# alibaba-damo-academy/Inferix

Hardware: AMD Instinct MI355X
Metric: latent_frames_per_sec (higher is better)
Workload: dtype bf16; 1 GPU; Self-Forcing 480p bf16 (Wan2.1-T2V-1.3B causal DiT, 30 layers), block_size=3, 21 latent frames = 7 blocks x (4 denoise + 1 context) generator forwards, KV prefix 4680..32760 keys in the KV manager's cache (identity page map; page-table form: `streaming_steady`); `value` counts the generator calls (SURVEY 8d), the per-block VAE decode of config 2 is measured beside it under --full (`per_block_decod; batch=1, parallelism=single, layers=30, pair_forwards=True, pair_mode=streams

## Files before the change

### include/inferix_hip.h

```cpp
#ifndef INFERIX_HIP_H
#define INFERIX_HIP_H

#include <stdint.h>

#ifdef __cplusplus
extern "C" {
#endif

#define IFX_OK 0
#define IFX_EINVAL (-1)
#define IFX_ELAUNCH (-2)
#define IFX_EUNSUP (-3)

typedef uint16_t ifx_bf16;

#define IFX_ABI_MINOR 7
int ifx_version(void);
const char* ifx_last_error(void);
const char* ifx_arch(void);
int ifx_set_option(const char* key, int32_t value);
int ifx_get_option(const char* key, int32_t* value);
int32_t ifx_device_error(int32_t clear);

typedef struct {
  ifx_bf16* k;
  ifx_bf16* v;
  const int32_t* page_table;
  int32_t page_size;
  int32_t num_slots;
  int32_t kv_heads;
  int32_t head_dim;
  int32_t seg_split;
  int32_t seg_delta;
} ifx_kv_view;

int ifx_attn_fwd_paged(const ifx_bf16* q, ifx_bf16* out, float* lse, const ifx_kv_view* kv,
                       int32_t q_rows, int32_t heads, int32_t kv_start, int32_t kv_len, float scale,
                       void* stream);

int32_t ifx_attn_split_plan(int32_t q_rows, int32_t heads, int32_t kv_start, int32_t kv_len,
                            int64_t* workspace_bytes);
int ifx_attn_fwd_paged_split(const ifx_bf16* q, ifx_bf16* out, float* lse, const ifx_kv_view* kv,
                             int32_t q_rows, int32_t heads, int32_t kv_start, int32_t kv_len, float scale,
                             int32_t num_splits, void* workspace, int64_t workspace_bytes, void* stream);

int ifx_attn_fwd_paged_ld(const ifx_bf16* q, int32_t ldq, ifx_bf16* out, int32_t ldo, float* lse, const ifx_kv_view* kv,
                          int32_t q_rows, int32_t heads, int32_t kv_start, int32_t kv_len, float scale, int32_t num_splits,
                          void* workspace, int64_t workspace_bytes, void* stream);

int ifx_attn_fwd_dedup(const ifx_bf16* q, ifx_bf16* out, const ifx_kv_view* kv, int32_t q_rows, int32_t heads, int32_t kv_len,
                       int32_t last_key_multiplicity, float scale, void* stream);

int ifx_attn_fwd_ranges(const ifx_bf16* q, int32_t ldq, ifx_bf16* out, int32_t ldo, const ifx_kv_view* kv, int32_t q_rows,
                        int32_t heads, int32_t n_ranges, const int32_t* q_ranges, const int32_t* k_ranges, float scale,
                        void* stream);

int ifx_attn_fwd_partial(const ifx_bf16* q, const ifx_kv_view* kv, int32_t q_rows, int32_t heads, int32_t kv_start,
                         int32_t kv_len, float scale, int32_t num_splits, void* workspace, int64_t workspace_bytes,
                         int32_t slot_base, int32_t slot_cap, int32_t* slots_used, void* stream);
int ifx_attn_merge_partials(const void* workspace, int32_t slot_cap, int32_t slots_used, ifx_bf16* out, float* lse,
                            int32_t q_rows, int32_t heads, void* stream);

int ifx_lse_merge(ifx_bf16* out_a, float* lse_a, const ifx_bf16* out_b, const float* lse_b,
                  int32_t rows, int32_t heads, void* stream);

typedef struct {
  const double* freqs;
  int32_t max_pos;
  int32_t start_frame;
  int32_t height, width;
  int32_t hw_offset;
  int32_t hw_local;
  float q_scale;
  int32_t flags;
} ifx_rope_grid;

int ifx_rmsnorm_rope_kv_append(const ifx_bf16* qkv, int32_t qkv_row_stride, ifx_bf16* q_out,
                               const ifx_bf16* wq, const ifx_bf16* wk, const ifx_rope_grid* rope,
                               const ifx_kv_view* kv, int32_t local_start, int32_t rows,
                               int32_t dim, float eps, void* stream);

int ifx_rmsnorm(const ifx_bf16* x, int32_t x_row_stride, ifx_bf16* y, int32_t y_row_stride,
                const ifx_bf16* w, int32_t rows, int32_t dim, float eps, void* stream);

enum { IFX_LN_PLAIN = 0, IFX_LN_AFFINE = 1, IFX_LN_MODULATE = 2 };
int ifx_layernorm(const ifx_bf16* x, ifx_bf16* y, int32_t rows, int32_t dim, float eps, int32_t mode,
                  const ifx_bf16* gamma, const ifx_bf16* beta, const ifx_bf16* mod,
                  int32_t mod_slots, int32_t shift_slot, int32_t scale_slot, int32_t rows_per_group,
                  void* stream);

enum { IFX_EPI_BIAS = 0, IFX_EPI_GELU_TANH = 1, IFX_EPI_RESIDUAL = 2, IFX_EPI_GATE_RES = 3, IFX_EPI_GELU_ERF = 4 };
typedef struct {
  int32_t epilogue;
  const ifx_bf16* residual;
  int32_t ld_res;
  const ifx_bf16* mod;
  int32_t mod_slots;
  int32_t gate_slot;
  int32_t rows_per_group;
  ifx_bf16* y2;
  int32_t ldy2;
  int32_t split_col;
} ifx_epilogue;
int ifx_gemm_bf16(const ifx_bf16* x, int32_t ldx, const ifx_bf16* w, const ifx_bf16* bias,
                  ifx_bf16* y, int32_t ldy, int32_t M, int32_t N, int32_t K,
                  const ifx_epilogue* epi, void* stream);

int64_t ifx_gemm_workspace_bytes(int32_t M, int32_t N, int32_t K);
int ifx_gemm_bf16_ws(const ifx_bf16* x, int32_t ldx, const ifx_bf16* w, const ifx_bf16* bias, ifx_bf16* y, int32_t ldy,
                     int32_t M, int32_t N, int32_t K, const ifx_epilogue* epi, void* workspace, int64_t workspace_bytes,
                     void* stream);

enum { IFX_Q_FP8_E4M3 = 0, IFX_Q_INT8 = 1 };
int ifx_quant_per_token(const ifx_bf16* x, int32_t ldx, void* q, int32_t ldq, float* scale, int32_t rows,
                        int32_t K, int32_t format, void* stream);
int ifx_gemm_q8(const void* xq, int32_t ldx, const float* x_scale, const void* wq, const float* w_scale,
                const ifx_bf16* bias, ifx_bf16* y, int32_t ldy, int32_t M, int32_t N, int32_t K, int32_t format,
                const ifx_epilogue* epi, void* stream);
int64_t ifx_gemm_q8_workspace_bytes(int32_t M, int32_t N, int32_t K);
int ifx_gemm_q8_ws(const void* xq, int32_t ldx, const float* x_scale, const void* wq, const float* w_scale, const ifx_bf16* bias,
                   ifx_bf16* y, int32_t ldy, int32_t M, int32_t N, int32_t K, int32_t format, const ifx_epilogue* epi,
                   void* workspace, int64_t workspace_bytes, void* stream);
int ifx_layernorm_quant(const ifx_bf16* x, void* q, int32_t ldq, float* scale, int32_t rows, int32_t dim, float eps,
                        int32_t mode, const ifx_bf16* gamma, const ifx_bf16* beta, const ifx_bf16* mod, int32_t mod_slots,
                        int32_t shift_slot, int32_t scale_slot, int32_t rows_per_group, int32_t format, void* stream);

int ifx_gemm_q8_quant_out(const void* xq, int32_t ldx, const float* x_scale, const void* wq, const float* w_scale,
                          const ifx_bf16* bias, void* yq, int32_t ldyq, int32_t M, int32_t N, int32_t K, int32_t format,
                          const ifx_epilogue* epi, const float* out_divisor, int32_t via_bf16, void* stream);
int ifx_layernorm_quant_static(const ifx_bf16* x, void* q, int32_t ldq, const float* divisors, int32_t n_out, int32_t rows,
                               int32_t dim, float eps, int32_t mode, const ifx_bf16* gamma, const ifx_bf16* beta,
                               int32_t via_bf16, void* stream);

int ifx_quant_static(const ifx_bf16* x, int32_t ldx, void* q, int32_t ldq, const float* divisor, int32_t divisor_len,
                     float* row_scale, int32_t rows, int32_t K, int32_t format, int32_t via_bf16, void* stream);
int ifx_quant_per_tensor(const ifx_bf16* x, int32_t ldx, void* q, int32_t ldq, float* row_scale, void* amax_workspace,
                         int32_t rows, int32_t K, int32_t format, void* stream);

int ifx_kv_roll(const ifx_kv_view* kv, int32_t sink_tokens, int32_t evicted, int32_t rolled,
                ifx_bf16* scratch, void* stream);

int ifx_kv_scatter_shards(const ifx_bf16* gathered, int32_t world, int32_t frames, int32_t hw_local,
                          int32_t frame_tokens, int32_t local_start, const ifx_kv_view* kv, void* stream);

#define IFX_MAX_PEERS 8
#define IFX_PEER_HANDLE_BYTES 64
typedef struct {
  int32_t count;
  ifx_bf16* k[IFX_MAX_PEERS];
  ifx_bf16* v[IFX_MAX_PEERS];
} ifx_peer_caches;
typedef struct {
  int32_t count;
  int32_t* flags[IFX_MAX_PEERS];
} ifx_peer_flags;
int ifx_peer_alloc(int64_t bytes, int32_t fine_grained, void** ptr);
int ifx_peer_free(void* ptr);
int ifx_peer_export(const void* ptr, uint8_t* handle, int64_t* offset);
int ifx_peer_open(const uint8_t* handle, void** ptr);
int ifx_peer_close(void* ptr);
int ifx_rmsnorm_rope_kv_push(const ifx_bf16* kv_rows, int32_t kv_row_stride, const ifx_bf16* wk, const ifx_rope_grid* rope,
                             const ifx_peer_caches* peers, const ifx_kv_view* geometry, int32_t local_start, int32_t frame_tokens,
                             int32_t slot_hw_local, int32_t slot_hw_offset, int32_t rows, int32_t dim, float eps, void* stream);
int ifx_peer_signal(const ifx_peer_flags* peers, int32_t index, int32_t value, void* stream);
int ifx_peer_wait(const int32_t* flags, int32_t count, int32_t value, int32_t timeout_ms, int32_t* status, void* stream);

typedef struct {
  const ifx_bf16* x;
  int64_t in_frame_stride;
  const int32_t* in_slots;
  int32_t hs, ws, cin, upsample;
  const ifx_bf16* w;
  const ifx_bf16* bias;
  int32_t kt, ks;
  ifx_bf16* y;
  int64_t out_frame_stride;
  const int32_t* out_slots;
  int32_t cout, t_out;
  const ifx_bf16* residual;
  const void* zero_page;
  int32_t in_planar;
} ifx_conv3d_desc;
int ifx_conv3d_cl(const ifx_conv3d_desc* desc, void* stream);

#define IFX_NORM_SILU 1
#define IFX_NORM_OUT_PLANAR 2
int ifx_rmsnorm_cl(const ifx_bf16* x, const ifx_bf16* gamma, ifx_bf16* y, int64_t out_frame_stride,
                   const int32_t* out_slots, int32_t frames, int32_t frame_pixels, int32_t channels,
                   int32_t flags, void* stream);

int ifx_softmax_rows(const ifx_bf16* scores, ifx_bf16* probs, int32_t rows, int32_t cols, int32_t ld, float scale,
                     void* stream);

int ifx_t5_attention(const ifx_bf16* q, int32_t ldq, const ifx_bf16* k, int32_t ldk, const ifx_bf16* v, int32_t ldv,
                     ifx_bf16* out, int32_t ldo, const ifx_bf16* rel_bias, const int32_t* seq_lens, int32_t batch,
                     int32_t seq_len_padded, int32_t heads, void* stream);

int ifx_t5_gated_gelu(const ifx_bf16* gate_fc1, ifx_bf16* h, int32_t rows, int32_t ffn, void* stream);

typedef struct {
  const ifx_bf16* in;
  int32_t ld_in, rows, layout, q_heads, kv_heads, head_dim;
  const float* rope;
  const float *qn_w, *qn_b, *kn_w, *kn_b;
  const ifx_bf16 *xn_w, *xn_b;
  float eps;
  int32_t layernorm_1p;
  ifx_bf16* q_out;
  int32_t ld_q;
  ifx_bf16* qx_out;
  int32_t ld_qx;
  ifx_bf16* k_out;
  ifx_bf16* v_out;
  int32_t ld_kv, kv_head_stride;
  int32_t row0, split, row1;
  float q_scale;
  int32_t rope_half;
  int32_t q_group;
  int64_t q_group_stride;
} ifx_magi_head_prep_desc;
int ifx_magi_head_prep(const ifx_magi_head_prep_desc* desc, void* stream);

int ifx_magi_gate_norm_residual(const ifx_bf16* x, int32_t ldx, const ifx_bf16* residual, int32_t ld_res,
                                const int32_t* condition_map, const ifx_bf16* gate, int32_t ld_gate, const float* norm_w,
                                const float* norm_b, int32_t layernorm_1p, ifx_bf16* y, int32_t ldy, int32_t rows, int32_t dim,
                                float eps, void* stream);

enum { IFX_ACT_SILU = 0, IFX_ACT_TANH = 1 };
int ifx_act_rows(const ifx_bf16* x, ifx_bf16* y, int64_t n, int32_t mode, void* stream);
int ifx_kv_split_rows(const ifx_bf16* kv, ifx_bf16* k_cache, ifx_bf16* v_cache, int32_t rows, int32_t heads, int32_t row0,
                      int32_t split, int32_t row1, void* stream);

#ifdef __cplusplus
}
#endif
#endif
```

### inferix_amd/_hip.py

```python
from __future__ import annotations

import ctypes as C
import os
from typing import Optional

import torch

_HERE = os.path.dirname(os.path.abspath(__file__))
LIB_PATH = os.environ.get("IFX_HIP_LIB", os.path.join(_HERE, "libinferix_hip.so"))

IFX_LN_PLAIN, IFX_LN_AFFINE, IFX_LN_MODULATE = 0, 1, 2
IFX_EPI_BIAS, IFX_EPI_GELU_TANH, IFX_EPI_RESIDUAL, IFX_EPI_GATE_RES, IFX_EPI_GELU_ERF = 0, 1, 2, 3, 4
IFX_ACT_SILU, IFX_ACT_TANH = 0, 1
IFX_Q_FP8_E4M3, IFX_Q_INT8 = 0, 1


class HipLibraryMissing(RuntimeError):
    pass


class HipKernelError(RuntimeError):
    pass


class KvView(C.Structure):
    _fields_ = [("k", C.c_void_p), ("v", C.c_void_p), ("page_table", C.c_void_p),
                ("page_size", C.c_int32), ("num_slots", C.c_int32), ("kv_heads", C.c_int32),
                ("head_dim", C.c_int32), ("seg_split", C.c_int32), ("seg_delta", C.c_int32)]


class RopeGrid(C.Structure):
    _fields_ = [("freqs", C.c_void_p), ("max_pos", C.c_int32), ("start_frame", C.c_int32),
                ("height", C.c_int32), ("width", C.c_int32), ("hw_offset", C.c_int32),
                ("hw_local", C.c_int32), ("q_scale", C.c_float), ("flags", C.c_int32)]


class Conv3dDesc(C.Structure):
    _fields_ = [("x", C.c_void_p), ("in_frame_stride", C.c_int64), ("in_slots", C.POINTER(C.c_int32)),
                ("hs", C.c_int32), ("ws", C.c_int32), ("cin", C.c_int32), ("upsample", C.c_int32),
                ("w", C.c_void_p), ("bias", C.c_void_p), ("kt", C.c_int32), ("ks", C.c_int32),
                ("y", C.c_void_p), ("out_frame_stride", C.c_int64), ("out_slots", C.POINTER(C.c_int32)),
                ("cout", C.c_int32), ("t_out", C.c_int32), ("residual", C.c_void_p), ("zero_page", C.c_void_p),
                ("in_planar", C.c_int32)]


class Epilogue(C.Structure):
    _fields_ = [("epilogue", C.c_int32), ("residual", C.c_void_p), ("ld_res", C.c_int32),
                ("mod", C.c_void_p), ("mod_slots", C.c_int32), ("gate_slot", C.c_int32),
                ("rows_per_group", C.c_int32), ("y2", C.c_void_p), ("ldy2", C.c_int32), ("split_col", C.c_int32)]


class MagiHeadPrepDesc(C.Structure):
    _fields_ = [("inp", C.c_void_p), ("ld_in", C.c_int32), ("rows", C.c_int32), ("layout", C.c_int32),
                ("q_heads", C.c_int32), ("kv_heads", C.c_int32), ("head_dim", C.c_int32), ("rope", C.c_void_p),
                ("qn_w", C.c_void_p), ("qn_b", C.c_void_p), ("kn_w", C.c_void_p), ("kn_b", C.c_void_p),
                ("xn_w", C.c_void_p), ("xn_b", C.c_void_p), ("eps", C.c_float), ("layernorm_1p", C.c_int32),
                ("q_out", C.c_void_p), ("ld_q", C.c_int32), ("qx_out", C.c_void_p), ("ld_qx", C.c_int32),
                ("k_out", C.c_void_p), ("v_out", C.c_void_p), ("ld_kv", C.c_int32), ("kv_head_stride", C.c_int32),
                ("row0", C.c_int32), ("split", C.c_int32), ("row1", C.c_int32), ("q_scale", C.c_float), ("rope_half", C.c_int32),
                ("q_group", C.c_int32), ("q_group_stride", C.c_int64)]


IFX_MAX_PEERS, IFX_PEER_HANDLE_BYTES = 8, 64


class PeerCaches(C.Structure):
    _fields_ = [("count", C.c_int32), ("k", C.c_void_p * IFX_MAX_PEERS), ("v", C.c_void_p * IFX_MAX_PEERS)]


class PeerFlags(C.Structure):
    _fields_ = [("count", C.c_int32), ("flags", C.c_void_p * IFX_MAX_PEERS)]


_vp, _i32, _f32 = C.c_void_p, C.c_int32, C.c_float
SIGNATURES = {
    "ifx_version": (C.c_int, []),
    "ifx_last_error": (C.c_char_p, []),
    "ifx_arch": (C.c_char_p, []),
    "ifx_set_option": (C.c_int, [C.c_char_p, _i32]),
    "ifx_get_option": (C.c_int, [C.c_char_p, C.POINTER(_i32)]),
    "ifx_device_error": (_i32, [_i32]),
    "ifx_attn_fwd_paged": (C.c_int, [_vp, _vp, _vp, C.POINTER(KvView), _i32, _i32, _i32, _i32, _f32, _vp]),
    "ifx_attn_split_plan": (_i32, [_i32, _i32, _i32, _i32, C.POINTER(C.c_int64)]),
    "ifx_attn_fwd_paged_split": (C.c_int, [_vp, _vp, _vp, C.POINTER(KvView), _i32, _i32, _i32, _i32, _f32, _i32, _vp,
                                           C.c_int64, _vp]),
    "ifx_conv3d_cl": (C.c_int, [C.POINTER(Conv3dDesc), _vp]),
    "ifx_rmsnorm_cl": (C.c_int, [_vp, _vp, _vp, C.c_int64, C.POINTER(_i32), _i32, _i32, _i32, _i32, _vp]),
    "ifx_softmax_rows": (C.c_int, [_vp, _vp, _i32, _i32, _i32, _f32, _vp]),
    "ifx_t5_attention": (C.c_int, [_vp, _i32, _vp, _i32, _vp, _i32, _vp, _i32, _vp, _vp, _i32, _i32, _i32, _vp]),
    "ifx_t5_gated_gelu": (C.c_int, [_vp, _vp, _i32, _i32, _vp]),
    "ifx_kv_scatter_shards": (C.c_int, [_vp, _i32, _i32, _i32, _i32, _i32, C.POINTER(KvView), _vp]),
    "ifx_peer_alloc": (C.c_int, [C.c_int64, _i32, C.POINTER(C.c_void_p)]),
    "ifx_peer_free": (C.c_int, [_vp]),
    "ifx_peer_export": (C.c_int, [_vp, C.c_char_p, C.POINTER(C.c_int64)]),
    "ifx_peer_open": (C.c_int, [C.c_char_p, C.POINTER(C.c_void_p)]),
    "ifx_peer_close": (C.c_int, [_vp]),
    "ifx_rmsnorm_rope_kv_push": (C.c_int, [_vp, _i32, _vp, C.POINTER(RopeGrid), C.POINTER(PeerCaches), C.POINTER(KvView), _i32, _i32,
                                           _i32, _i32, _i32, _i32, _f32, _vp]),
    "ifx_peer_signal": (C.c_int, [C.POINTER(PeerFlags), _i32, _i32, _vp]),
    "ifx_peer_wait": (C.c_int, [_vp, _i32, _i32, _i32, _vp, _vp]),
    "ifx_attn_fwd_partial": (C.c_int, [_vp, C.POINTER(KvView), _i32, _i32, _i32, _i32, _f32, _i32, _vp, C.c_int64, _i32,
                                       _i32, C.POINTER(_i32), _vp]),
    "ifx_attn_merge_partials": (C.c_int, [_vp, _i32, _i32, _vp, _vp, _i32, _i32, _vp]),
    "ifx_lse_merge": (C.c_int, [_vp, _vp, _vp, _vp, _i32, _i32, _vp]),
    "ifx_rmsnorm_rope_kv_append": (C.c_int, [_vp, _i32, _vp, _vp, _vp, C.POINTER(RopeGrid), C.POINTER(KvView),
                                             _i32, _i32, _i32, _f32, _vp]),
    "ifx_rmsnorm": (C.c_int, [_vp, _i32, _vp, _i32, _vp, _i32, _i32, _f32, _vp]),
    "ifx_layernorm": (C.c_int, [_vp, _vp, _i32, _i32, _f32, _i32, _vp, _vp, _vp, _i32, _i32, _i32, _i32, _vp]),
    "ifx_gemm_bf16": (C.c_int, [_vp, _i32, _vp, _vp, _vp, _i32, _i32, _i32, _i32, C.POINTER(Epilogue), _vp]),
    "ifx_kv_roll": (C.c_int, [C.POINTER(KvView), _i32, _i32, _i32, _vp, _vp]),
    "ifx_quant_per_token": (C.c_int, [_vp, _i32, _vp, _i32, _vp, _i32, _i32, _i32, _vp]),
    "ifx_layernorm_quant": (C.c_int, [_vp, _vp, _i32, _vp, _i32, _i32, _f32, _i32, _vp, _vp, _vp, _i32, _i32, _i32, _i32, _i32, _vp]),
    "ifx_gemm_q8": (C.c_int, [_vp, _i32, _vp, _vp, _vp, _vp, _vp, _i32, _i32, _i32, _i32, _i32, C.POINTER(Epilogue), _vp]),
    "ifx_gemm_q8_ws": (C.c_int, [_vp, _i32, _vp, _vp, _vp, _vp, _vp, _i32, _i32, _i32, _i32, _i32, C.POINTER(Epilogue), _vp, C.c_int64, _vp]),
    "ifx_gemm_q8_workspace_bytes": (C.c_int64, [_i32, _i32, _i32]),
    "ifx_attn_fwd_paged_ld": (C.c_int, [_vp, _i32, _vp, _i32, _vp, C.POINTER(KvView), _i32, _i32, _i32, _i32, _f32, _i32, _vp,
                                        C.c_int64, _vp]),
    "ifx_gemm_q8_quant_out": (C.c_int, [_vp, _i32, _vp, _vp, _vp, _vp, _vp, _i32, _i32, _i32, _i32, _i32, C.POINTER(Epilogue), _vp, _i32, _vp]),
    "ifx_layernorm_quant_static": (C.c_int, [_vp, _vp, _i32, _vp, _i32, _i32, _i32, _f32, _i32, _vp, _vp, _i32, _vp]),
    "ifx_quant_static": (C.c_int, [_vp, _i32, _vp, _i32, _vp, _i32, _vp, _i32, _i32, _i32, _i32, _vp]),
    "ifx_quant_per_tensor": (C.c_int, [_vp, _i32, _vp, _i32, _vp, _vp, _i32, _i32, _i32, _vp]),
    "ifx_magi_head_prep": (C.c_int, [C.POINTER(MagiHeadPrepDesc), _vp]),
    "ifx_magi_gate_norm_residual": (C.c_int, [_vp, _i32, _vp, _i32, _vp, _vp, _i32, _vp, _vp, _i32, _vp, _i32, _i32, _i32, _f32,
                                              _vp]),
    "ifx_act_rows": (C.c_int, [_vp, _vp, C.c_int64, _i32, _vp]),
    "ifx_kv_split_rows": (C.c_int, [_vp, _vp, _vp, _i32, _i32, _i32, _i32, _i32, _vp]),
    "ifx_attn_fwd_dedup": (C.c_int, [_vp, _vp, C.POINTER(KvView), _i32, _i32, _i32, _i32, _f32, _vp]),
    "ifx_attn_fwd_ranges": (C.c_int, [_vp, _i32, _vp, _i32, C.POINTER(KvView), _i32, _i32, _i32, C.POINTER(_i32), C.POINTER(_i32), _f32, _vp]),
    "ifx_gemm_workspace_bytes": (C.c_int64, [_i32, _i32, _i32]),
    "ifx_gemm_bf16_ws": (C.c_int, [_vp, _i32, _vp, _vp, _vp, _i32, _i32, _i32, _i32, C.POINTER(Epilogue), _vp, C.c_int64, _vp]),
}

_lib: Optional[C.CDLL] = None
ABI_MINOR = 7


def load() -> C.CDLL:
    global _lib
    if _lib is not None:
        return _lib
    if not os.path.exists(LIB_PATH):
        raise HipLibraryMissing(
            f"{LIB_PATH} not found: build it with `python -c 'import __graft_entry__ as g; g.build()'` "
            "(hipcc --offload-arch=gfx950).  inferix_amd has no CPU or eager fallback.")
    lib = C.CDLL(LIB_PATH)
    for name, (res, args) in SIGNATURES.items():
        fn = getattr(lib, name)
        fn.restype = res
        fn.argtypes = args
    got = (lib.ifx_version() >> 8) & 255
    if got != ABI_MINOR:
        raise HipLibraryMissing(f"{LIB_PATH} has ABI minor {got}, these bindings are for {ABI_MINOR} (include/inferix_hip.h "
                                "IFX_ABI_MINOR): rebuild with __graft_entry__.build()")
    _lib = lib
    return lib


def check(rc: int, what: str) -> None:
    if rc != 0:
        msg = load().ifx_last_error().decode("utf-8", "replace")
        raise HipKernelError(f"{what} failed (code {rc}): {msg}")


def version() -> str:
    v = load().ifx_version()
    return f"{v >> 16}.{(v >> 8) & 255}.{v & 255}"
```

### inferix_amd/csrc/ifx_attn.hip

```cpp
#include <stdlib.h>
#include <type_traits>

#include "ifx_common.h"

namespace ifx {

constexpr int QT = 128;
constexpr int KT = 64;
constexpr int HD = 128;

struct AttnArgs {
  const unsigned short* q;
  unsigned short* out;
  float* lse;
  const unsigned short* k;
  const unsigned short* v;
  KvAddr ka;
  int q_rows, heads, kv_start, kv_len, q_tiles, per_xcd, total;
  int ldq, ldo;
  float last_key_bias;
  int kv_heads, q_per_kv;
  float scale, scale_log2;
};

typedef __attribute__((address_space(3))) void* attn_lds_ptr_t;
typedef const __attribute__((address_space(1))) void* attn_gbl_ptr_t;

__device__ __forceinline__ void attn_dma16(const unsigned short* src, unsigned lds) {
  asm volatile("s_mov_b32 m0, %0\n\ts_nop 0\n\tglobal_load_lds_dwordx4 %1, off" : : "s"(lds), "v"(src) : "memory");
}

__device__ __forceinline__ float max3f(float a, float b, float c) {
  float r;
  asm("v_max3_f32 %0, %1, %2, %3" : "=v"(r) : "v"(a), "v"(b), "v"(c));
  return r;
}
__device__ __forceinline__ float half_swap_max(float x) {
  float a = x, b = x, r;
  asm volatile("s_nop 1\n\tv_permlane32_swap_b32 %0, %1\n\ts_nop 1\n\tv_max_f32 %2, %0, %1"
               : "+v"(a), "+v"(b), "=v"(r));
  return r;
}

template <bool PAGED, bool SHORT>
__global__ __launch_bounds__(256, 2) void attn_fwd_kernel(AttnArgs A) {
  __shared__ __attribute__((aligned(16))) unsigned char smem[65536];
  const int tid = threadIdx.x, lane = tid & 63;
  const int wave = __builtin_amdgcn_readfirstlane(tid >> 6);
  const int hi = lane >> 5, l31 = lane & 31;

  const int xcd = blockIdx.x & 7, slot_i = blockIdx.x >> 3;
  const int wi = xcd * A.per_xcd + slot_i;
  if (slot_i >= A.per_xcd || wi >= A.total) return;
  const int head = wi / A.q_tiles, qt = wi - head * A.q_tiles;
  const int kv_stride = A.kv_heads * HD;
  const int kvh = head / A.q_per_kv;

  const int qrow = qt * QT + wave * 32 + l31;
  const int qrow_c = min(qrow, A.q_rows - 1);
  bf16x8 qf[8];
  {
    const unsigned short* qp = A.q + (size_t)qrow_c * A.ldq + head * HD + hi * 8;
#pragma unroll
    for (int ks = 0; ks < 8; ++ks) qf[ks] = *reinterpret_cast<const bf16x8*>(qp + ks * 16);
  }
  __builtin_amdgcn_s_waitcnt(0x0F70);

  const int d_row = lane >> 4, d_pc = lane & 15;
  int k_src_c[4], v_src_c[4], d_rowi[4];
#pragma unroll
  for (int r = 0; r < 4; ++r) {
    const int row = (r * 4 + wave) * 4 + d_row;
    d_rowi[r] = row;
    k_src_c[r] = (d_pc ^ (row & 15)) * 8;
    v_src_c[r] = ((((d_pc >> 2) ^ (row & 3)) << 2) | (d_pc & 3)) * 8;
  }
  const unsigned short* kbase = A.k + kvh * HD;
  const unsigned short* vbase = A.v + kvh * HD;
  const int last_key = A.kv_len - 1;
  const unsigned lds0 = (unsigned)(unsigned long long)(attn_lds_ptr_t)smem + wave * 1024;
  auto issue = [&](int t, int buf, auto clamp_tag) {
    constexpr bool CLAMP = decltype(clamp_tag)::value;
    const unsigned kb = lds0 + buf * 32768;
#pragma unroll
    for (int r = 0; r < 4; ++r) {
      int key = A.kv_start + t * KT + d_rowi[r];
      if (CLAMP) key = min(key, last_key);
      const size_t off = (size_t)(PAGED ? A.ka.slot(key) : key) * kv_stride;
      attn_dma16(kbase + off + k_src_c[r], kb + r * 4096);
      attn_dma16(vbase + off + v_src_c[r], kb + 16384 + r * 4096);
    }
  };

  f32x16 o[4];
#pragma unroll
  for (int d = 0; d < 4; ++d)
#pragma unroll
    for (int r = 0; r < 16; ++r) o[d][r] = 0.f;
  float m_run = -INFINITY, l_run = 0.f;
  const float c2 = A.scale_log2;

  const int kswz = l31 & 15;
  const int vi = lane & 15, vg1 = (lane >> 4) & 1;
  const int v_rowq = vi >> 2;
  const int v_in = (vg1 << 5) | ((vi & 3) << 3);

  const int nkeys = A.kv_len - A.kv_start;
  const int NT = (nkeys + KT - 1) / KT;

  auto tile = [&](int t, int buf, auto ragged_tag) {
    constexpr bool RAGGED = decltype(ragged_tag)::value;
    const unsigned char* kb = smem + buf * 32768;
    const unsigned char* vb = kb + 16384;
    bf16x8 kA[4], kB[4], vA[4], vB[4];
    auto ldK = [&](bf16x8(&f)[4], int b, int kh) {
      const unsigned char* krow = kb + (32 * b + l31) * 256;
#pragma unroll
      for (int k4 = 0; k4 < 4; ++k4)
        f[k4] = *reinterpret_cast<const bf16x8*>(krow + (((2 * (4 * kh + k4) + hi) ^ kswz) << 4));
    };
    auto mmaK = [&](f32x16& acc, bf16x8(&f)[4], int kh) {
#pragma unroll
      for (int k4 = 0; k4 < 4; ++k4) acc = __builtin_amdgcn_mfma_f32_32x32x16_bf16(f[k4], qf[4 * kh + k4], acc, 0, 0, 0);
    };
    auto ldV = [&](bf16x8(&f)[4], int b, int s2) {
      const unsigned char* vr0 = vb + (32 * b + 16 * s2 + 4 * hi + v_rowq) * 256 + v_in;
      const unsigned char* vr1 = vr0 + 8 * 256;
#pragma unroll
      for (int d = 0; d < 4; ++d) {
        const int ch = (d ^ v_rowq) << 6;
        const bf16x4 t0 = __builtin_amdgcn_ds_read_tr16_b64_v4bf16((bf16x4 __attribute__((address_space(3)))*)(vr0 + ch));
        const bf16x4 t1 = __builtin_amdgcn_ds_read_tr16_b64_v4bf16((bf16x4 __attribute__((address_space(3)))*)(vr1 + ch));
        f[d] = __builtin_shufflevector(t0, t1, 0, 1, 2, 3, 4, 5, 6, 7);
      }
    };
    auto mmaV = [&](bf16x8(&f)[4], const bf16x8& p) {
#pragma unroll
      for (int d = 0; d < 4; ++d) o[d] = __builtin_amdgcn_mfma_f32_32x32x16_bf16(f[d], p, o[d], 0, 0, 0);
    };
    auto block_max = [&](f32x16& sb) -> float {
      float mx = __builtin_fmaxf(sb[0], sb[1]);
      mx = max3f(mx, sb[2], m_run);
#pragma unroll
      for (int r = 3; r < 15; r += 2) mx = max3f(mx, sb[r], sb[r + 1]);
      mx = max3f(mx, sb[15], mx);
      return half_swap_max(mx);
    };
    auto exp_block = [&](f32x16& sb, bf16x8(&pb)[2]) -> float {
      typedef float f32x2 __attribute__((ext_vector_type(2)));
      const float mc = m_run * c2;
      const f32x2 c2v = {c2, c2}, mcv = {mc, mc};
      float a0 = 0.f, a1 = 0.f;
#pragma unroll
      for (int i = 0; i < 8; ++i) {
        const f32x2 sv = {sb[2 * i], sb[2 * i + 1]};
        const f32x2 e = sv * c2v - mcv;
        const float p0 = __builtin_amdgcn_exp2f(e[0]), p1 = __builtin_amdgcn_exp2f(e[1]);
        a0 += p0;
        a1 += p1;
        pb[i >> 2][(2 * i) & 7] = static_cast<__bf16>(p0);
        pb[i >> 2][(2 * i + 1) & 7] = static_cast<__bf16>(p1);
      }
      return a0 + a1;
    };
    auto softmax_block = [&](f32x16& sb, int b, bf16x8(&pb)[2]) -> float {
      if (RAGGED) {
        const int kidx = t * KT + 32 * b + 4 * hi;
#pragma unroll
        for (int r = 0; r < 16; ++r) {
          const int kk = kidx + (r & 3) + 8 * (r >> 2);
          if (kk >= nkeys) sb[r] = -INFINITY;
          else if (kk == nkeys - 1) sb[r] += A.last_key_bias;
        }
      }
      if (t == 0 && b == 0) m_run = block_max(sb);
      float ps = exp_block(sb, pb);
      float alpha = 1.0f;
      if (__any(!(ps < 1048576.f))) {
        const float m_new = block_max(sb);
        alpha = __builtin_amdgcn_exp2f((m_run - m_new) * c2);
        m_run = m_new;
        ps = exp_block(sb, pb);
        l_run *= alpha;
      }
      l_run += ps;
      return alpha;
    };
    auto rescale_o = [&](float alpha) {
      asm volatile("" : "+v"(alpha));
      if (__any(alpha != 1.0f)) {
        asm volatile("s_nop 15\n\ts_nop 7" ::: "memory");
#pragma unroll
        for (int d = 0; d < 4; ++d)
#pragma unroll
          for (int r = 0; r < 16; ++r) asm volatile("v_mul_f32 %0, %0, %1" : "+v"(o[d][r]) : "v"(alpha));
        asm volatile("s_nop 3" ::: "memory");
      }
    };

    f32x16 s0, s1;
    bf16x8 p0[2], p1[2];
    ldK(kA, 0, 0);
    ldK(kB, 0, 1);
    __builtin_amdgcn_sched_barrier(0);
#pragma unroll
    for (int r = 0; r < 16; ++r) s0[r] = 0.f;
    __builtin_amdgcn_s_setprio(1);
    mmaK(s0, kA, 0);
    ldK(kA, 1, 0);
    __builtin_amdgcn_sched_barrier(0);
    mmaK(s0, kB, 1);
    ldK(kB, 1, 1);
    __builtin_amdgcn_sched_barrier(0);
#pragma unroll
    for (int r = 0; r < 16; ++r) s1[r] = 0.f;
    mmaK(s1, kA, 0);
    ldV(vA, 0, 0);
    mmaK(s1, kB, 1);
    ldV(vB, 0, 1);
    const float a0 = softmax_block(s0, 0, p0);
#pragma unroll
    for (int i = 0; i < 8; ++i) {
      __builtin_amdgcn_sched_group_barrier(0x008, 1, 0);
      __builtin_amdgcn_sched_group_barrier(0x100, 2, 0);
      __builtin_amdgcn_sched_group_barrier(0x002, 10, 0);
    }
    __builtin_amdgcn_sched_barrier(0);
    rescale_o(a0);
    mmaV(vA, p0[0]);
    ldV(vA, 1, 0);
    mmaV(vB, p0[1]);
    ldV(vB, 1, 1);
    const float a1 = softmax_block(s1, 1, p1);
#pragma unroll
    for (int i = 0; i < 8; ++i) {
      __builtin_amdgcn_sched_group_barrier(0x008, 1, 1);
      __builtin_amdgcn_sched_group_barrier(0x100, 2, 1);
      __builtin_amdgcn_sched_group_barrier(0x002, 10, 1);
    }
    __builtin_amdgcn_sched_barrier(0);
    rescale_o(a1);
    mmaV(vA, p1[0]);
    mmaV(vB, p1[1]);
    __builtin_amdgcn_s_setprio(0);
  };

  issue(0, 0, std::true_type{});
  asm volatile("s_waitcnt vmcnt(0)" ::: "memory");
  __builtin_amdgcn_s_barrier();
  for (int t = 0; t < NT - 1; ++t) {
    const int buf = t & 1;
    if (t + 2 < NT) issue(t + 1, buf ^ 1, std::false_type{});
    else issue(t + 1, buf ^ 1, std::true_type{});
    tile(t, buf, std::false_type{});
    asm volatile("s_waitcnt vmcnt(0) lgkmcnt(0)" ::: "memory");
    __builtin_amdgcn_s_barrier();
  }
  if ((nkeys & (KT - 1)) || A.last_key_bias != 0.f) tile(NT - 1, (NT - 1) & 1, std::true_type{});
  else tile(NT - 1, (NT - 1) & 1, std::false_type{});

  const float l_tot = l_run + __shfl_xor(l_run, 32, 64);
  const float inv = 1.0f / l_tot;
  if (qrow < A.q_rows) {
    unsigned short* op = A.out + (size_t)qrow * A.ldo + head * HD + 4 * hi;
#pragma unroll
    for (int d = 0; d < 4; ++d)
#pragma unroll
      for (int g = 0; g < 4; ++g) {
        u16x4 w;
#pragma unroll
        for (int e = 0; e < 4; ++e) w[e] = f2bf(o[d][4 * g + e] * inv);
        *reinterpret_cast<u16x4*>(op + 32 * d + 8 * g) = w;
      }
    if (A.lse != nullptr && hi == 0) A.lse[(size_t)head * A.q_rows + qrow] = m_run * A.scale + __logf(l_tot);
  }
}

__global__ __launch_bounds__(256) void lse_merge_kernel(unsigned short* __restrict__ oa, float* __restrict__ la,
                                                        const unsigned short* __restrict__ ob,
                                                        const float* __restrict__ lb, int rows, int heads) {
  const size_t total = (size_t)rows * heads * 16;
  for (size_t i = (size_t)blockIdx.x * blockDim.x + threadIdx.x; i < total; i += (size_t)gridDim.x * blockDim.x) {
    const int c = (int)(i & 15);
    const size_t rh = i >> 4;
    const int h = (int)(rh % heads);
    const size_t r = rh / heads;
    const float a = la[(size_t)h * rows + r], b = lb[(size_t)h * rows + r];
    const float sg = 1.0f / (1.0f + __expf(a - b));
    u16x8 ua = *reinterpret_cast<const u16x8*>(oa + rh * HD + c * 8);
    const u16x8 ub = *reinterpret_cast<const u16x8*>(ob + rh * HD + c * 8);
#pragma unroll
    for (int e = 0; e < 8; ++e) {
      const float x = bf2f(ua[e]), y = bf2f(ub[e]);
      ua[e] = f2bf(x - sg * (x - y));
    }
    *reinterpret_cast<u16x8*>(oa + rh * HD + c * 8) = ua;
    if (c == 0) {
      const float mxv = fmaxf(a, b);
      la[(size_t)h * rows + r] = mxv + __logf(__expf(a - mxv) + __expf(b - mxv));
    }
  }
}

int launch_attn_pp(const unsigned short* q, unsigned short* out, float* lse, const ifx_kv_view* kv, int q_rows,
                   int heads, int kv_start, int kv_len, float scale, int splits, void* workspace, int groups,
                   hipStream_t stream, int slot_base = 0, int slot_cap = 0, int* slots_used = nullptr, int ldq = 0, int ldo = 0,
                   int n_ranges = 0, const int* q_ranges = nullptr, const int* k_ranges = nullptr);
int launch_attn_merge(const float* workspace, int slot_cap, int slots_used, unsigned short* out, float* lse, int q_rows,
                      int heads, hipStream_t stream, int ldo = 0);
size_t attn_pp_workspace_bytes(int q_rows, int heads, int splits);
int attn_pp_split_heuristic(int q_rows, int heads, int nkeys, int qt, int slots);
static int attn_groups(int variant, int q_rows, int heads = 0) {
  if (variant == 3 || variant == 4 || variant == 2 || variant == 5 || variant == 6 || variant == 7) return variant;
  if (variant == 0 && q_rows > 0) {
    const int t256 = (q_rows + 255) / 256, t128 = (q_rows + 127) / 128;
    const float u256 = (float)q_rows / (256.f * t256), u128 = (float)q_rows / (128.f * t128);
    if (u128 > 1.1f * u256) return 6;
    if (heads > 0 && t256 * heads > 256) {
      const float c5 = (float)((t256 * heads + 255) / 256);
      const float c6 = (float)((t128 * heads + 511) / 512) / 0.953f;
      if (c6 < 0.95f * c5) return 6;
    }
  }
  return 7;
}
static int attn_qt(int groups) { return groups == 3 ? 384 : (groups == 6 ? 128 : 256); }
static int attn_slots(int groups) { return groups == 6 ? 512 : 256; }

}

using namespace ifx;

static int attn_dispatch(const ifx_bf16* q, ifx_bf16* out, float* lse, const ifx_kv_view* kv, int32_t q_rows,
                         int32_t heads, int32_t kv_start, int32_t kv_len, float scale, int32_t splits, void* workspace,
                         int64_t workspace_bytes, void* stream, int32_t ldq = 0, int32_t ldo = 0, int32_t last_key_multiplicity = 1) {
  IFX_REQUIRE(q && out && kv && kv->k && kv->v, "ifx_attn_fwd_paged: null argument");
  if (ldq <= 0) ldq = heads * HD;
  if (ldo <= 0) ldo = heads * HD;
  IFX_REQUIRE(ldq >= heads * HD && ldo >= heads * HD && ldq % 8 == 0 && ldo % 8 == 0,
              "ifx_attn_fwd_paged: row strides (%d, %d) must be >= heads * 128 and multiples of 8", ldq, ldo);
  IFX_REQUIRE(kv->head_dim == HD, "ifx_attn_fwd_paged: head_dim %d not built (128 only)", kv->head_dim);
  IFX_REQUIRE(heads > 0 && kv->kv_heads > 0 && heads % kv->kv_heads == 0,
              "ifx_attn_fwd_paged: heads %d is not a multiple of kv_heads %d", heads, kv->kv_heads);
  IFX_REQUIRE(q_rows >= 0 && kv_start >= 0 && kv_len > kv_start && kv_len <= kv->num_slots,
              "ifx_attn_fwd_paged: key range [%d, %d) out of range (capacity %d)", kv_start, kv_len, kv->num_slots);
  if (kv->page_table) IFX_REQUIRE(kv->page_size > 0, "ifx_attn_fwd_paged: page_size must be > 0");
  if (q_rows == 0) return IFX_OK;
  const int variant = attn_variant();
  if (last_key_multiplicity > 1) {
    IFX_REQUIRE(splits <= 1 && kv_len - kv_start <= 1024 && lse == nullptr,
                "ifx_attn_fwd_dedup: the multiplicity form is built for short key ranges (<= 1024 keys), unsplit, without LSE");
  }
  if (splits > 1) {
    IFX_REQUIRE(workspace && workspace_bytes >= (int64_t)attn_pp_workspace_bytes(q_rows, heads, splits),
                "ifx_attn_fwd_paged_split: workspace of %lld B too small for %d splits (need %lld B)",
                (long long)workspace_bytes, splits, (long long)attn_pp_workspace_bytes(q_rows, heads, splits));
    return launch_attn_pp(q, out, lse, kv, q_rows, heads, kv_start, kv_len, scale, splits, workspace, attn_groups(variant, q_rows, heads),
                          (hipStream_t)stream, 0, 0, nullptr, ldq, ldo);
  }
  if (last_key_multiplicity <= 1 && (variant >= 2 || (variant == 0 && q_rows >= 1024 && kv_len - kv_start > 1024)))
    return launch_attn_pp(q, out, lse, kv, q_rows, heads, kv_start, kv_len, scale, 1, nullptr, attn_groups(variant, q_rows, heads),
                          (hipStream_t)stream, 0, 0, nullptr, ldq, ldo);
  AttnArgs a;
  a.q = q;
  a.out = out;
  a.lse = lse;
  a.k = kv->k;
  a.v = kv->v;
  a.ka = KvAddr{kv->page_table, kv->page_size, kv->page_table ? 0 : kv->seg_split, kv->page_table ? 0 : kv->seg_delta};
  a.q_rows = q_rows;
  a.heads = heads;
  a.ldq = ldq;
  a.ldo = ldo;
  a.kv_start = kv_start;
  a.kv_len = kv_len;
  a.kv_heads = kv->kv_heads;
  a.q_per_kv = heads / kv->kv_heads;
  a.q_tiles = (q_rows + QT - 1) / QT;
  a.total = a.q_tiles * heads;
  a.per_xcd = (a.total + 7) / 8;
  a.scale = scale > 0.f ? scale : 0.08838834764831845f;
  a.scale_log2 = a.scale * 1.4426950408889634f;
  a.last_key_bias = last_key_multiplicity > 1 ? logf((float)last_key_multiplicity) / a.scale : 0.f;

  const dim3 grid(a.per_xcd * 8), block(256);
  const bool short_kv = kv_len - kv_start <= 1024;
  if (kv->page_table || kv->seg_split > 0) {
    if (short_kv) hipLaunchKernelGGL((attn_fwd_kernel<true, true>), grid, block, 0, (hipStream_t)stream, a);
    else hipLaunchKernelGGL((attn_fwd_kernel<true, false>), grid, block, 0, (hipStream_t)stream, a);
  } else {
    if (short_kv) hipLaunchKernelGGL((attn_fwd_kernel<false, true>), grid, block, 0, (hipStream_t)stream, a);
    else hipLaunchKernelGGL((attn_fwd_kernel<false, false>), grid, block, 0, (hipStream_t)stream, a);
  }
  return check_launch("ifx_attn_fwd_paged");
}

extern "C" int ifx_attn_fwd_paged(const ifx_bf16* q, ifx_bf16* out, float* lse, const ifx_kv_view* kv,
                                  int32_t q_rows, int32_t heads, int32_t kv_start, int32_t kv_len, float scale,
                                  void* stream) {
  return attn_dispatch(q, out, lse, kv, q_rows, heads, kv_start, kv_len, scale, 1, nullptr, 0, stream);
}

extern "C" int ifx_attn_fwd_paged_ld(const ifx_bf16* q, int32_t ldq, ifx_bf16* out, int32_t ldo, float* lse, const ifx_kv_view* kv,
                                     int32_t q_rows, int32_t heads, int32_t kv_start, int32_t kv_len, float scale,
                                     int32_t num_splits, void* workspace, int64_t workspace_bytes, void* stream) {
  IFX_REQUIRE(num_splits >= 1 && num_splits <= 64, "ifx_attn_fwd_paged_ld: num_splits %d outside [1, 64]", num_splits);
  IFX_REQUIRE(ldq > 0 && ldo > 0, "ifx_attn_fwd_paged_ld: row strides must be given");
  return attn_dispatch(q, out, lse, kv, q_rows, heads, kv_start, kv_len, scale, num_splits, workspace, workspace_bytes, stream,
                       ldq, ldo);
}

extern "C" int ifx_attn_fwd_dedup(const ifx_bf16* q, ifx_bf16* out, const ifx_kv_view* kv, int32_t q_rows, int32_t heads,
                                  int32_t kv_len, int32_t last_key_multiplicity, float scale, void* stream) {
  IFX_REQUIRE(last_key_multiplicity >= 1, "ifx_attn_fwd_dedup: multiplicity %d", last_key_multiplicity);
  return attn_dispatch(q, out, nullptr, kv, q_rows, heads, 0, kv_len, scale, 1, nullptr, 0, stream, 0, 0, last_key_multiplicity);
}

extern "C" int ifx_attn_fwd_ranges(const ifx_bf16* q, int32_t ldq, ifx_bf16* out, int32_t ldo, const ifx_kv_view* kv, int32_t q_rows,
                                   int32_t heads, int32_t n_ranges, const int32_t* q_ranges, const int32_t* k_ranges, float scale,
                                   void* stream) {
  IFX_REQUIRE(q && out && kv && kv->k && kv->v && q_ranges && k_ranges, "ifx_attn_fwd_ranges: null argument");
  IFX_REQUIRE(kv->head_dim == HD, "ifx_attn_fwd_ranges: head_dim %d not built (128 only)", kv->head_dim);
  IFX_REQUIRE(heads > 0 && kv->kv_heads > 0 && heads % kv->kv_heads == 0, "ifx_attn_fwd_ranges: heads %d / kv_heads %d", heads,
              kv->kv_heads);
  IFX_REQUIRE(n_ranges >= 1 && n_ranges <= 8, "ifx_attn_fwd_ranges: 1..8 ranges per launch (got %d)", n_ranges);
  if (ldq <= 0) ldq = heads * HD;
  if (ldo <= 0) ldo = heads * HD;
  IFX_REQUIRE(ldq >= heads * HD && ldo >= heads * HD && ldq % 8 == 0 && ldo % 8 == 0, "ifx_attn_fwd_ranges: row strides (%d, %d)", ldq, ldo);
  if (kv->page_table) IFX_REQUIRE(kv->page_size > 0, "ifx_attn_fwd_ranges: page_size must be > 0");
  int kmin = 0x7fffffff, kmax = 0, rows = 0;
  for (int i = 0; i < n_ranges; ++i) {
    const int q0 = q_ranges[2 * i], q1 = q_ranges[2 * i + 1], k0 = k_ranges[2 * i], k1 = k_ranges[2 * i + 1];
    IFX_REQUIRE(q0 >= 0 && q1 > q0 && q1 <= q_rows, "ifx_attn_fwd_ranges: query range %d = [%d, %d) outside [0, %d)", i, q0, q1, q_rows);
    IFX_REQUIRE(k0 >= 0 && k1 > k0 && k1 <= kv->num_slots, "ifx_attn_fwd_ranges: key range %d = [%d, %d) out of range (capacity %d)",
                i, k0, k1, kv->num_slots);
    kmin = k0 < kmin ? k0 : kmin;
    kmax = k1 > kmax ? k1 : kmax;
    rows += q1 - q0;
  }
  const int groups = attn_groups(attn_variant(), rows / n_ranges, heads * n_ranges);
  return launch_attn_pp(q, out, nullptr, kv, q_rows, heads, kmin, kmax, scale, 1, nullptr, groups == 5 || groups == 6 || groups == 7 ? groups : 7,
                        (hipStream_t)stream, 0, 0, nullptr, ldq, ldo, n_ranges, q_ranges, k_ranges);
}

extern "C" int32_t ifx_attn_split_plan(int32_t q_rows, int32_t heads, int32_t kv_start, int32_t kv_len,
                                       int64_t* workspace_bytes) {
  int splits = 1;
  if (q_rows > 0 && heads > 0 && kv_len > kv_start)
    splits = attn_pp_split_heuristic(q_rows, heads, kv_len - kv_start, attn_qt(attn_groups(attn_variant(), q_rows, heads)),
                                     attn_slots(attn_groups(attn_variant(), q_rows, heads)));
  if (workspace_bytes) *workspace_bytes = (int64_t)attn_pp_workspace_bytes(q_rows, heads, splits);
  return splits;
}

extern "C" int ifx_attn_fwd_paged_split(const ifx_bf16* q, ifx_bf16* out, float* lse, const ifx_kv_view* kv,
                                        int32_t q_rows, int32_t heads, int32_t kv_start, int32_t kv_len, float scale,
                                        int32_t num_splits, void* workspace, int64_t workspace_bytes, void* stream) {
  IFX_REQUIRE(num_splits >= 1 && num_splits <= 64, "ifx_attn_fwd_paged_split: num_splits %d outside [1, 64]", num_splits);
  return attn_dispatch(q, out, lse, kv, q_rows, heads, kv_start, kv_len, scale, num_splits, workspace, workspace_bytes,
                       stream);
}

extern "C" int ifx_attn_fwd_partial(const ifx_bf16* q, const ifx_kv_view* kv, int32_t q_rows, int32_t heads,
                                    int32_t kv_start, int32_t kv_len, float scale, int32_t num_splits, void* workspace,
                                    int64_t workspace_bytes, int32_t slot_base, int32_t slot_cap, int32_t* slots_used,
                                    void* stream) {
  IFX_REQUIRE(q && kv && kv->k && kv->v && workspace, "ifx_attn_fwd_partial: null argument");
  IFX_REQUIRE(kv->head_dim == HD, "ifx_attn_fwd_partial: head_dim %d not built (128 only)", kv->head_dim);
  IFX_REQUIRE(heads > 0 && kv->kv_heads > 0 && heads % kv->kv_heads == 0,
              "ifx_attn_fwd_partial: heads %d is not a multiple of kv_heads %d", heads, kv->kv_heads);
  IFX_REQUIRE(q_rows > 0 && kv_start >= 0 && kv_len > kv_start && kv_len <= kv->num_slots,
              "ifx_attn_fwd_partial: key range [%d, %d) out of range (capacity %d)", kv_start, kv_len, kv->num_slots);
  IFX_REQUIRE(num_splits >= 1 && slot_base >= 0 && slot_cap >= 1 && slot_cap <= 128,
              "ifx_attn_fwd_partial: bad split / slot arguments (%d splits, base %d, cap %d)", num_splits, slot_base, slot_cap);
  IFX_REQUIRE(workspace_bytes >= (int64_t)slot_cap * q_rows * heads * 129 * (int64_t)sizeof(float),
              "ifx_attn_fwd_partial: workspace of %lld B too small for %d slots", (long long)workspace_bytes, slot_cap);
  if (kv->page_table) IFX_REQUIRE(kv->page_size > 0, "ifx_attn_fwd_partial: page_size must be > 0");
  return launch_attn_pp(q, nullptr, nullptr, kv, q_rows, heads, kv_start, kv_len, scale, num_splits, workspace,
                        attn_groups(attn_variant(), q_rows, heads), (hipStream_t)stream, slot_base, slot_cap, slots_used);
}

extern "C" int ifx_attn_merge_partials(const void* workspace, int32_t slot_cap, int32_t slots_used, ifx_bf16* out,
                                       float* lse, int32_t q_rows, int32_t heads, void* stream) {
  IFX_REQUIRE(workspace && out && q_rows > 0 && heads > 0 && slots_used >= 1 && slots_used <= slot_cap,
              "ifx_attn_merge_partials: bad arguments (%d of %d slots)", slots_used, slot_cap);
  return launch_attn_merge((const float*)workspace, slot_cap, slots_used, out, lse, q_rows, heads, (hipStream_t)stream);
}

extern "C" int ifx_lse_merge(ifx_bf16* out_a, float* lse_a, const ifx_bf16* out_b, const float* lse_b,
                             int32_t rows, int32_t heads, void* stream) {
  IFX_REQUIRE(out_a && lse_a && out_b && lse_b && rows >= 0 && heads > 0, "ifx_lse_merge: bad arguments");
  if (rows == 0) return IFX_OK;
  const size_t total = (size_t)rows * heads * 16;
  const int blocks = (int)((total + 255) / 256 < 2048 ? (total + 255) / 256 : 2048);
  hipLaunchKernelGGL(lse_merge_kernel, dim3(blocks), dim3(256), 0, (hipStream_t)stream, out_a, lse_a, out_b,
                     lse_b, rows, heads);
  return check_launch("ifx_lse_merge");
}
```

### inferix_amd/csrc/ifx_core.hip

```cpp
#include <stdarg.h>
#include <stdlib.h>
#include <string.h>

#include "ifx_common.h"

namespace ifx {
static thread_local char g_err[512] = "";

void set_error(const char* fmt, ...) {
  va_list ap;
  va_start(ap, fmt);
  vsnprintf(g_err, sizeof(g_err), fmt, ap);
  va_end(ap);
}

static int g_gemm_variant = -1, g_gemm_pp_variant = -1, g_attn_variant = -1, g_conv_variant = -1, g_spin_timeout_ms = -1, g_spin_fault = 0;
static thread_local int g_gemm_small_split = -1;
static int opt_or_env(int& slot, const char* env, int dflt = 0) {
  if (slot < 0) {
    const char* e = getenv(env);
    slot = e ? atoi(e) : dflt;
  }
  return slot;
}
int gemm_variant() { return opt_or_env(g_gemm_variant, "IFX_GEMM_VARIANT"); }
int gemm_pp_variant() { return opt_or_env(g_gemm_pp_variant, "IFX_GEMM_PP_VARIANT"); }
int attn_variant() { return opt_or_env(g_attn_variant, "IFX_ATTN_VARIANT"); }
int conv_variant() { return opt_or_env(g_conv_variant, "IFX_CONV_VARIANT"); }
static unsigned* g_attn_dbg = nullptr;
static bool g_attn_dbg_on = false;
unsigned* attn_debug_counter() { return g_attn_dbg_on ? g_attn_dbg : nullptr; }
int gemm_small_split() { return opt_or_env(g_gemm_small_split, "IFX_GEMM_SMALL_SPLIT"); }

static unsigned* g_dev_err = nullptr;
unsigned* device_error_word() {
  if (g_dev_err == nullptr) {
    void* p = nullptr;
    if (hipHostMalloc(&p, 64, hipHostMallocMapped | hipHostMallocPortable) == hipSuccess && p != nullptr) {
      memset(p, 0, 64);
      g_dev_err = (unsigned*)p;
    }
  }
  return g_dev_err;
}
long long spin_timeout_ticks() { return (long long)max(1, opt_or_env(g_spin_timeout_ms, "IFX_SPIN_TIMEOUT_MS", 2000)) * 100000LL; }
int spin_fault() { return g_spin_fault; }
static thread_local char g_err_dev[640] = "";

int check_launch(const char* what) {
  hipError_t e = hipGetLastError();
  if (e != hipSuccess) {
    set_error("%s: launch failed: %s", what, hipGetErrorString(e));
    return IFX_ELAUNCH;
  }
  return IFX_OK;
}
}

extern "C" int ifx_version(void) { return (0 << 16) | (IFX_ABI_MINOR << 8) | 0; }
extern "C" int32_t ifx_device_error(int32_t clear) {
  unsigned* w = ifx::g_dev_err;
  if (w == nullptr) return 0;
  const unsigned v = __atomic_load_n(w, __ATOMIC_ACQUIRE);
  if (v != 0 && clear) __atomic_store_n(w, 0u, __ATOMIC_RELEASE);
  return (int32_t)v;
}
extern "C" const char* ifx_last_error(void) {
  const unsigned v = (unsigned)ifx_device_error(1);
  if (v == 0) return ifx::g_err;
  const unsigned kind = v >> 24, detail = v & 0xffffffu;
  snprintf(ifx::g_err_dev, sizeof(ifx::g_err_dev),
           "device: a kernel gave up a wait (%s, flag %u) after the spin budget — the producing workgroup was not resident or did not "
           "finish; the results of that launch are invalid%s%s",
           kind == 1 ? "split-K / stream-K consumer of ifx_gemm_bf16_ws / ifx_gemm_q8_ws" : "unknown waiter", detail,
           ifx::g_err[0] ? "; last host error: " : "", ifx::g_err);
  return ifx::g_err_dev;
}
extern "C" const char* ifx_arch(void) { return "gfx950"; }
extern "C" int ifx_set_option(const char* key, int32_t value) {
  if (key && !strcmp(key, "gemm_variant") && value >= 0 && value <= 29) { ifx::g_gemm_variant = value; return IFX_OK; }
  if (key && !strcmp(key, "gemm_small_split") && (value == 0 || value == 1)) { ifx::g_gemm_small_split = value; return IFX_OK; }
  if (key && !strcmp(key, "attn_variant") && value >= 0 && value <= 7) { ifx::g_attn_variant = value; return IFX_OK; }
  if (key && !strcmp(key, "conv_variant") && value >= 0 && value <= 1) { ifx::g_conv_variant = value; return IFX_OK; }
  if (key && !strcmp(key, "gemm_pp_variant") && value >= 0 && value <= 1) { ifx::g_gemm_pp_variant = value; return IFX_OK; }
  if (key && !strcmp(key, "attn_debug_counters") && (value == 0 || value == 1)) {
    if (value == 1) {
      if (ifx::g_attn_dbg == nullptr && hipMalloc((void**)&ifx::g_attn_dbg, 64) != hipSuccess) {
        ifx::g_attn_dbg = nullptr;
        ifx::set_error("ifx_set_option: attn_debug_counters: hipMalloc failed");
        return IFX_ELAUNCH;
      }
      (void)hipDeviceSynchronize();
      (void)hipMemset(ifx::g_attn_dbg, 0, 64);
    }
    ifx::g_attn_dbg_on = value == 1;
    return IFX_OK;
  }
  if (key && !strcmp(key, "spin_timeout_ms") && value >= 1 && value <= 600000) { ifx::g_spin_timeout_ms = value; return IFX_OK; }
  if (key && !strcmp(key, "spin_fault") && (value == 0 || value == 1)) { ifx::g_spin_fault = value; return IFX_OK; }
  ifx::set_error("ifx_set_option: unknown key or value out of range: %s = %d", key ? key : "(null)", (int)value);
  return IFX_EINVAL;
}
extern "C" int ifx_get_option(const char* key, int32_t* value) {
  if (key == nullptr || value == nullptr) { ifx::set_error("ifx_get_option: null argument"); return IFX_EINVAL; }
  if (!strcmp(key, "gemm_variant")) { *value = ifx::gemm_variant(); return IFX_OK; }
  if (!strcmp(key, "gemm_small_split")) { *value = ifx::gemm_small_split(); return IFX_OK; }
  if (!strcmp(key, "attn_variant")) { *value = ifx::attn_variant(); return IFX_OK; }
  if (!strcmp(key, "conv_variant")) { *value = ifx::conv_variant(); return IFX_OK; }
  if (!strcmp(key, "gemm_pp_variant")) { *value = ifx::gemm_pp_variant(); return IFX_OK; }
  if (!strcmp(key, "attn_debug_counters")) { *value = ifx::g_attn_dbg_on ? 1 : 0; return IFX_OK; }
  if (!strcmp(key, "attn_rescale_count")) {
    unsigned v = 0;
    if (ifx::g_attn_dbg != nullptr) {
      (void)hipDeviceSynchronize();
      (void)hipMemcpy(&v, ifx::g_attn_dbg, sizeof(v), hipMemcpyDeviceToHost);
    }
    *value = (int32_t)(v & 0x7fffffffu);
    return IFX_OK;
  }
  if (!strcmp(key, "spin_timeout_ms")) { *value = (int32_t)(ifx::spin_timeout_ticks() / 100000LL); return IFX_OK; }
  if (!strcmp(key, "spin_fault")) { *value = ifx::spin_fault(); return IFX_OK; }
  ifx::set_error("ifx_get_option: unknown key: %s", key);
  return IFX_EINVAL;
}
```

### inferix_amd/csrc/ifx_norm.hip

```cpp
#include "ifx_rows.h"

namespace ifx {

template <int NCH, int QUANT = 0>
__global__ __launch_bounds__(256) void layernorm_kernel(
    const unsigned short* __restrict__ x, unsigned short* __restrict__ y, int rows, int dim, float eps,
    int mode, const unsigned short* __restrict__ gamma, const unsigned short* __restrict__ beta,
    const unsigned short* __restrict__ mod, int mod_slots, int shift_slot, int scale_slot,
    int rows_per_group, unsigned char* __restrict__ q, int ldq, float* __restrict__ qscale, int n_out, int via_bf16) {
  const int lane = threadIdx.x & 63;
  const int r = blockIdx.x * 4 + (threadIdx.x >> 6);
  if (r >= rows) return;
  u16x8 xr[NCH], pa[NCH], pb[NCH];
  load_chunks<NCH>(xr, x + (size_t)r * dim, dim, lane);
  {
    const unsigned short* pa_p = nullptr;
    const unsigned short* pb_p = nullptr;
    if (mode == IFX_LN_MODULATE) {
      const size_t g0 = (size_t)(r / rows_per_group) * mod_slots;
      pa_p = mod + (g0 + scale_slot) * dim;
      pb_p = mod + (g0 + shift_slot) * dim;
    } else if (mode == IFX_LN_AFFINE) {
      pa_p = gamma;
      pb_p = beta;
    }
    if (pa_p != nullptr) {
      load_chunks<NCH>(pa, pa_p, dim, lane);
      load_chunks<NCH>(pb, pb_p, dim, lane);
    } else {
#pragma unroll
      for (int c = 0; c < NCH; ++c) {
        pa[c] = u16x8{0, 0, 0, 0, 0, 0, 0, 0};
        pb[c] = u16x8{0, 0, 0, 0, 0, 0, 0, 0};
      }
    }
  }
  Row<NCH> row;
  row.from(xr, dim, lane);
  float mean, rstd;
  ln_stats(row, dim, eps, lane, mean, rstd);

  u16x8 qrow[QUANT != 0 ? NCH : 1];
  if (QUANT != 0) {
#pragma unroll
    for (int c = 0; c < NCH; ++c) qrow[c] = u16x8{0, 0, 0, 0, 0, 0, 0, 0};
  }
#pragma unroll
  for (int c = 0; c < NCH; ++c) {
    const int col = c * 512 + lane * 8;
    if (col >= dim) continue;
    u16x8 o;
    if (mode == IFX_LN_MODULATE) {
      const u16x8 sc = pa[c], sh = pb[c];
#pragma unroll
      for (int i = 0; i < 8; ++i) {
        float t = rbf((row.v[c][i] - mean) * rstd);
        float s1 = rbf(1.0f + bf2f(sc[i]));
        t = rbf(t * s1);
        o[i] = f2bf(t + bf2f(sh[i]));
      }
    } else if (mode == IFX_LN_AFFINE) {
      const u16x8 g = pa[c], b = pb[c];
#pragma unroll
      for (int i = 0; i < 8; ++i)
        o[i] = f2bf((row.v[c][i] - mean) * rstd * bf2f(g[i]) + bf2f(b[i]));
    } else {
#pragma unroll
      for (int i = 0; i < 8; ++i) o[i] = f2bf((row.v[c][i] - mean) * rstd);
    }
    if (QUANT == 0) *reinterpret_cast<u16x8*>(y + (size_t)r * dim + col) = o;
    else qrow[c] = o;
  }
  if constexpr (QUANT == 3) {
    const float* divs = qscale;
    for (int j = 0; j < n_out; ++j) {
#pragma unroll
      for (int c = 0; c < NCH; ++c) {
        const int col = c * 512 + lane * 8;
        if (col >= dim) continue;
        const f32x4 d0 = *reinterpret_cast<const f32x4*>(divs + (size_t)j * dim + col);
        const f32x4 d1 = *reinterpret_cast<const f32x4*>(divs + (size_t)j * dim + col + 4);
        float v[8];
#pragma unroll
        for (int i = 0; i < 8; ++i) v[i] = bf2f(qrow[c][i]);
        *reinterpret_cast<u32x2*>(q + (size_t)r * ldq + (size_t)j * dim + col) = div_clamp8<true>(v, d0, d1, via_bf16);
      }
    }
  } else if constexpr (QUANT != 0) {
    quant_row_dynamic<QUANT == 1, NCH>(qrow, q + (size_t)r * ldq, qscale + r, dim, lane);
  }
}

template <int NCH>
__global__ __launch_bounds__(256) void rmsnorm_kernel(const unsigned short* __restrict__ x, int ldx,
                                                      unsigned short* __restrict__ y, int ldy,
                                                      const unsigned short* __restrict__ w, int rows,
                                                      int dim, float eps) {
  const int lane = threadIdx.x & 63;
  const int r = blockIdx.x * 4 + (threadIdx.x >> 6);
  if (r >= rows) return;
  u16x8 xr[NCH], wv[NCH];
  load_chunks<NCH>(xr, x + (size_t)r * ldx, dim, lane);
  load_chunks<NCH>(wv, w, dim, lane);
  Row<NCH> row;
  row.from(xr, dim, lane);
  const float rs = 1.0f / sqrtf(wave_sum(row.sumsq()) / (float)dim + eps);
#pragma unroll
  for (int c = 0; c < NCH; ++c) {
    const int col = c * 512 + lane * 8;
    u16x8 o;
#pragma unroll
    for (int i = 0; i < 8; ++i) o[i] = f2bf(rbf(row.v[c][i] * rs) * bf2f(wv[c][i]));
    if (col < dim) *reinterpret_cast<u16x8*>(y + (size_t)r * ldy + col) = o;
  }
}

template <int NCH>
__global__ __launch_bounds__(256) void rmsnorm_rope_append_kernel(
    const unsigned short* __restrict__ qkv, int ld, unsigned short* __restrict__ q_out,
    const unsigned short* __restrict__ wq, const unsigned short* __restrict__ wk, RopeArgs ra, int has_rope,
    unsigned short* __restrict__ kc, unsigned short* __restrict__ vc, KvAddr ka, int local_start, int rows,
    int dim, int head_dim, float eps) {
  const int lane = threadIdx.x & 63;
  const int r = blockIdx.x * 4 + (threadIdx.x >> 6);
  if (r >= rows) return;
  const unsigned short* base = qkv + (size_t)r * ld;

  size_t slot_off = 0;
  if (kc != nullptr) slot_off = (size_t)ka.slot(local_start + r) * dim;
  const RopeToken tk(ra, has_rope, r, head_dim, lane);

  const bool has_kv = kc != nullptr;
  const bool copy_v = vc != nullptr;
  u16x8 qraw[NCH], kraw[NCH], vraw[NCH], wqv[NCH], wkv[NCH];
  load_chunks<NCH>(qraw, base, dim, lane);
  load_chunks<NCH>(wqv, wq, dim, lane);
  if (has_kv) {
    load_chunks<NCH>(kraw, base + dim, dim, lane);
    if (copy_v) load_chunks<NCH>(vraw, base + 2 * dim, dim, lane);
    load_chunks<NCH>(wkv, wk, dim, lane);
  }
  if (has_kv && copy_v) {
#pragma unroll
    for (int c = 0; c < NCH; ++c) {
      const int col = c * 512 + lane * 8;
      if (col < dim) *reinterpret_cast<u16x8*>(vc + slot_off + col) = vraw[c];
    }
  }
  Row<NCH> row;
  rmsnorm_rope_row<NCH>(row, qraw, wqv, tk, ra, has_rope, ra.q_scale, dim, head_dim, eps, lane,
                        [&](int, int col, const u16x8& o) { *reinterpret_cast<u16x8*>(q_out + (size_t)r * dim + col) = o; });
  if (!has_kv) return;
  rmsnorm_rope_row<NCH>(row, kraw, wkv, tk, ra, has_rope, 1.0f, dim, head_dim, eps, lane,
                        [&](int, int col, const u16x8& o) { *reinterpret_cast<u16x8*>(kc + slot_off + col) = o; });
}

__global__ __launch_bounds__(256) void kv_copy_rows_kernel(const unsigned short* __restrict__ src,
                                                           unsigned short* __restrict__ dst, KvAddr ka,
                                                           int src_tok0, int dst_tok0, int ntok, int row_elems,
                                                           int src_is_paged, int dst_is_paged) {
  const int chunks = row_elems / 8;
  const size_t total = (size_t)ntok * chunks;
  for (size_t i = (size_t)blockIdx.x * blockDim.x + threadIdx.x; i < total; i += (size_t)gridDim.x * blockDim.x) {
    const int t = (int)(i / chunks), c = (int)(i - (size_t)t * chunks);
    const size_t s = (size_t)(src_is_paged ? ka.slot(src_tok0 + t) : (src_tok0 + t)) * row_elems + c * 8;
    const size_t d = (size_t)(dst_is_paged ? ka.slot(dst_tok0 + t) : (dst_tok0 + t)) * row_elems + c * 8;
    *reinterpret_cast<u16x8*>(dst + d) = *reinterpret_cast<const u16x8*>(src + s);
  }
}

__global__ __launch_bounds__(256) void kv_scatter_shards_kernel(const unsigned short* __restrict__ gathered,
                                                                unsigned short* __restrict__ kc,
                                                                unsigned short* __restrict__ vc, KvAddr ka, int world,
                                                                int frames, int hw_local, int frame_tokens,
                                                                int local_start, int row_elems) {
  const int n_local = frames * hw_local;
  const int chunks = row_elems / 8;
  const size_t total = (size_t)world * n_local * chunks;
  for (size_t i = (size_t)blockIdx.x * blockDim.x + threadIdx.x; i < total; i += (size_t)gridDim.x * blockDim.x) {
    const int row = (int)(i / chunks), c = (int)(i - (size_t)row * chunks);
    const int r = row / n_local, j = row - r * n_local;
    const int f = j / hw_local, w = j - f * hw_local;
    const int tok = local_start + f * frame_tokens + r * hw_local + w;
    const size_t d = (size_t)ka.slot(tok) * row_elems + c * 8;
    const unsigned short* ks = gathered + ((size_t)(2 * r) * n_local + j) * row_elems + c * 8;
    *reinterpret_cast<u16x8*>(kc + d) = *reinterpret_cast<const u16x8*>(ks);
    *reinterpret_cast<u16x8*>(vc + d) = *reinterpret_cast<const u16x8*>(ks + (size_t)n_local * row_elems);
  }
}

template <typename F>
static int dispatch_norm(int dim, F&& f) {
  return dispatch_nch<1, 2, 3, 4, 6, 8, 10>(dim, "row kernels support dim <= 5120 (got %d)", f);
}

}

using namespace ifx;

extern "C" int ifx_layernorm(const ifx_bf16* x, ifx_bf16* y, int32_t rows, int32_t dim, float eps, int32_t mode,
                             const ifx_bf16* gamma, const ifx_bf16* beta, const ifx_bf16* mod, int32_t mod_slots,
                             int32_t shift_slot, int32_t scale_slot, int32_t rows_per_group, void* stream) {
  IFX_REQUIRE(x && y && rows >= 0 && dim > 0 && dim % 8 == 0, "ifx_layernorm: bad x/y/rows/dim(%d)", dim);
  if (const int rc = check_ln_mode("ifx_layernorm", mode, gamma, beta, mod, mod_slots, shift_slot, scale_slot, rows_per_group))
    return rc;
  if (rows == 0) return IFX_OK;
  return dispatch_norm(dim, [&](auto nch) {
    return launch_rows("ifx_layernorm", layernorm_kernel<decltype(nch)::value, 0>, rows, stream, x, y, rows, dim, eps, mode, gamma, beta,
                       mod, mod_slots, shift_slot, scale_slot, rows_per_group > 0 ? rows_per_group : 1, (unsigned char*)nullptr, 0,
                       (float*)nullptr, 0, 0);
  });
}

extern "C" int ifx_layernorm_quant(const ifx_bf16* x, void* q, int32_t ldq, float* scale, int32_t rows, int32_t dim, float eps,
                                   int32_t mode, const ifx_bf16* gamma, const ifx_bf16* beta, const ifx_bf16* mod,
                                   int32_t mod_slots, int32_t shift_slot, int32_t scale_slot, int32_t rows_per_group,
                                   int32_t format, void* stream) {
  IFX_REQUIRE(x && q && scale && rows >= 0 && dim > 0 && dim % 8 == 0 && ldq >= dim && ldq % 8 == 0,
              "ifx_layernorm_quant: bad x/q/scale/rows/dim(%d)/ldq(%d)", dim, ldq);
  IFX_REQUIRE(format == IFX_Q_FP8_E4M3 || format == IFX_Q_INT8, "ifx_layernorm_quant: unknown format %d", format);
  if (const int rc = check_ln_mode("ifx_layernorm_quant", mode, gamma, beta, mod, mod_slots, shift_slot, scale_slot, rows_per_group))
    return rc;
  if (rows == 0) return IFX_OK;
  return dispatch_norm(dim, [&](auto nch) {
    return dispatch_q8_format(format, [&](auto fp8) {
      return launch_rows("ifx_layernorm_quant", layernorm_kernel<decltype(nch)::value, decltype(fp8)::value ? 1 : 2>, rows, stream, x,
                         (unsigned short*)nullptr, rows, dim, eps, mode, gamma, beta, mod, mod_slots, shift_slot, scale_slot,
                         rows_per_group > 0 ? rows_per_group : 1, (unsigned char*)q, ldq, scale, 0, 0);
    });
  });
}

extern "C" int ifx_layernorm_quant_static(const ifx_bf16* x, void* q, int32_t ldq, const float* divisors, int32_t n_out, int32_t rows,
                                          int32_t dim, float eps, int32_t mode, const ifx_bf16* gamma, const ifx_bf16* beta,
                                          int32_t via_bf16, void* stream) {
  IFX_REQUIRE(x && q && divisors && rows >= 0 && dim > 0 && dim % 8 == 0 && n_out >= 1 && n_out <= 8 && ldq >= n_out * dim && ldq % 8 == 0,
              "ifx_layernorm_quant_static: bad x/q/divisors/rows/dim(%d)/n_out(%d)/ldq(%d)", dim, n_out, ldq);
  IFX_REQUIRE(mode == IFX_LN_PLAIN || mode == IFX_LN_AFFINE, "ifx_layernorm_quant_static: mode %d (plain or affine)", mode);
  if (mode == IFX_LN_AFFINE) IFX_REQUIRE(gamma && beta, "ifx_layernorm_quant_static: affine mode needs gamma/beta");
  if (rows == 0) return IFX_OK;
  return dispatch_norm(dim, [&](auto nch) {
    return launch_rows("ifx_layernorm_quant_static", layernorm_kernel<decltype(nch)::value, 3>, rows, stream, x, (unsigned short*)nullptr,
                       rows, dim, eps, mode, gamma, beta, (const unsigned short*)nullptr, 0, 0, 0, 1, (unsigned char*)q, ldq,
                       const_cast<float*>(divisors), n_out, via_bf16);
  });
}

extern "C" int ifx_rmsnorm(const ifx_bf16* x, int32_t ldx, ifx_bf16* y, int32_t ldy, const ifx_bf16* w,
                           int32_t rows, int32_t dim, float eps, void* stream) {
  IFX_REQUIRE(x && y && w && rows >= 0 && dim > 0 && dim % 8 == 0 && ldx % 8 == 0 && ldy % 8 == 0,
              "ifx_rmsnorm: bad arguments (dim %d)", dim);
  IFX_REQUIRE(ldx >= dim && ldy >= dim, "ifx_rmsnorm: row strides ldx (%d) and ldy (%d) must be >= dim (%d)", ldx, ldy, dim);
  if (rows == 0) return IFX_OK;
  return dispatch_norm(dim, [&](auto nch) {
    return launch_rows("ifx_rmsnorm", rmsnorm_kernel<decltype(nch)::value>, rows, stream, x, ldx, y, ldy, w, rows, dim, eps);
  });
}

extern "C" int ifx_rmsnorm_rope_kv_append(const ifx_bf16* qkv, int32_t ld, ifx_bf16* q_out, const ifx_bf16* wq,
                                          const ifx_bf16* wk, const ifx_rope_grid* rope, const ifx_kv_view* kv,
                                          int32_t local_start, int32_t rows, int32_t dim, float eps,
                                          void* stream) {
  IFX_REQUIRE(qkv && q_out && wq && rows >= 0 && dim > 0 && dim % 8 == 0 && ld % 8 == 0,
              "ifx_rmsnorm_rope_kv_append: bad arguments");
  int head_dim = 128;
  KvAddr ka{nullptr, 1};
  unsigned short *kc = nullptr, *vc = nullptr;
  if (kv) {
    IFX_REQUIRE(wk && kv->k && kv->v && kv->kv_heads * kv->head_dim == dim,
                "ifx_rmsnorm_rope_kv_append: kv view (heads %d x head_dim %d) does not match dim %d",
                kv->kv_heads, kv->head_dim, dim);
    IFX_REQUIRE(local_start >= 0 && local_start + rows <= kv->num_slots,
                "ifx_rmsnorm_rope_kv_append: append [%d, %d) exceeds cache capacity %d", local_start,
                local_start + rows, kv->num_slots);
    if (const int rc = check_writer_view("ifx_rmsnorm_rope_kv_append", kv)) return rc;
    head_dim = kv->head_dim;
    kc = kv->k;
    vc = kv->v;
    ka = KvAddr{kv->page_table, kv->page_size};
  }
  RopeArgs ra{};
  if (const int rc = resolve_rope("ifx_rmsnorm_rope_kv_append", rope, head_dim, dim, rows, &ra)) return rc;
  if (rope) {
    IFX_REQUIRE(rope->q_scale >= 0.f && rope->q_scale == rope->q_scale, "ifx_rmsnorm_rope_kv_append: q_scale must be >= 0 (0 = 1)");
    ra.q_scale = rope->q_scale > 0.f ? rope->q_scale : 1.0f;
    if (rope->flags & 1) {
      IFX_REQUIRE(kv != nullptr, "ifx_rmsnorm_rope_kv_append: flags bit 0 (V in place) needs a cache view");
      vc = nullptr;
    }
  }
  {
    const int cols = kc == nullptr ? 1 : (vc == nullptr ? 2 : 3);
    IFX_REQUIRE(ld >= cols * dim, "ifx_rmsnorm_rope_kv_append: qkv_row_stride (ld %d) must cover the %d x dim (%d) columns read", ld, cols,
                dim);
  }
  if (rows == 0) return IFX_OK;
  return dispatch_norm(dim, [&](auto nch) {
    return launch_rows("ifx_rmsnorm_rope_kv_append", rmsnorm_rope_append_kernel<decltype(nch)::value>, rows, stream, qkv, ld, q_out, wq,
                       wk, ra, rope ? 1 : 0, kc, vc, ka, local_start, rows, dim, head_dim, eps);
  });
}

struct PeerDest {
  unsigned short* k[IFX_MAX_PEERS];
  unsigned short* v[IFX_MAX_PEERS];
  int n;
};

template <int NCH>
__global__ __launch_bounds__(256) void rmsnorm_rope_kv_push_kernel(
    const unsigned short* __restrict__ kv, int ld, const unsigned short* __restrict__ wk, RopeArgs ra, int has_rope, PeerDest pd,
    KvAddr ka, int local_start, int frame_tokens, int slot_hw_local, int slot_hw_offset, int rows, int dim, int head_dim, float eps) {
  const int lane = threadIdx.x & 63;
  const int r = blockIdx.x * 4 + (threadIdx.x >> 6);
  if (r >= rows) return;
  const unsigned short* base = kv + (size_t)r * ld;
  const int sf = r / slot_hw_local;
  const size_t slot_off = (size_t)ka.slot(local_start + sf * frame_tokens + slot_hw_offset + (r - sf * slot_hw_local)) * dim;
  const RopeToken tk(ra, has_rope, r, head_dim, lane);
  u16x8 kraw[NCH], vraw[NCH], wkv[NCH];
  load_chunks<NCH>(kraw, base, dim, lane);
  load_chunks<NCH>(vraw, base + dim, dim, lane);
  load_chunks<NCH>(wkv, wk, dim, lane);
  Row<NCH> row;
  rmsnorm_rope_row<NCH>(row, kraw, wkv, tk, ra, has_rope, 1.0f, dim, head_dim, eps, lane, [&](int c, int col, const u16x8& o) {
    for (int p = 0; p < pd.n; ++p) {
      *reinterpret_cast<u16x8*>(pd.k[p] + slot_off + col) = o;
      *reinterpret_cast<u16x8*>(pd.v[p] + slot_off + col) = vraw[c];
    }
  });
}

extern "C" int ifx_rmsnorm_rope_kv_push(const ifx_bf16* kv_rows, int32_t ld, const ifx_bf16* wk, const ifx_rope_grid* rope,
                                        const ifx_peer_caches* peers, const ifx_kv_view* geometry, int32_t local_start,
                                        int32_t frame_tokens, int32_t slot_hw_local, int32_t slot_hw_offset, int32_t rows, int32_t dim,
                                        float eps, void* stream) {
  IFX_REQUIRE(kv_rows && wk && peers && geometry && rows >= 0 && dim > 0 && dim % 8 == 0 && ld % 8 == 0 && ld >= 2 * dim,
              "ifx_rmsnorm_rope_kv_push: bad arguments");
  IFX_REQUIRE(peers->count >= 1 && peers->count <= IFX_MAX_PEERS, "ifx_rmsnorm_rope_kv_push: %d destinations (1..%d)", peers->count,
              IFX_MAX_PEERS);
  IFX_REQUIRE(geometry->kv_heads * geometry->head_dim == dim, "ifx_rmsnorm_rope_kv_push: cache rows (heads %d x head_dim %d) != dim %d",
              geometry->kv_heads, geometry->head_dim, dim);
  IFX_REQUIRE(slot_hw_local > 0 && frame_tokens >= slot_hw_local && slot_hw_offset >= 0 && slot_hw_offset + slot_hw_local <= frame_tokens,
              "ifx_rmsnorm_rope_kv_push: bad shard geometry (frame %d tokens, shard [%d, %d))", frame_tokens, slot_hw_offset,
              slot_hw_offset + slot_hw_local);
  if (rows == 0) return IFX_OK;
  const int last_f = (rows - 1) / slot_hw_local;
  const int last_token = local_start + last_f * frame_tokens + slot_hw_offset + (rows - 1 - last_f * slot_hw_local);
  IFX_REQUIRE(local_start >= 0 && last_token < geometry->num_slots, "ifx_rmsnorm_rope_kv_push: token %d exceeds the cache capacity %d",
              last_token, geometry->num_slots);
  if (geometry->page_table) IFX_REQUIRE(geometry->page_size > 0, "ifx_rmsnorm_rope_kv_push: page_size must be > 0");
  PeerDest pd{};
  pd.n = peers->count;
  for (int p = 0; p < pd.n; ++p) {
    IFX_REQUIRE(peers->k[p] && peers->v[p], "ifx_rmsnorm_rope_kv_push: destination %d is null", p);
    pd.k[p] = peers->k[p];
    pd.v[p] = peers->v[p];
  }
  const int head_dim = geometry->head_dim;
  RopeArgs ra{};
  if (const int rc = resolve_rope("ifx_rmsnorm_rope_kv_push", rope, head_dim, dim, rows, &ra)) return rc;
  const KvAddr ka{geometry->page_table, geometry->page_size, geometry->page_table ? 0 : geometry->seg_split,
                  geometry->page_table ? 0 : geometry->seg_delta};
  return dispatch_norm(dim, [&](auto nch) {
    return launch_rows("ifx_rmsnorm_rope_kv_push", rmsnorm_rope_kv_push_kernel<decltype(nch)::value>, rows, stream, kv_rows, ld, wk, ra,
                       rope ? 1 : 0, pd, ka, local_start, frame_tokens, slot_hw_local, slot_hw_offset, rows, dim, head_dim, eps);
  });
}

extern "C" int ifx_kv_roll(const ifx_kv_view* kv, int32_t sink_tokens, int32_t evicted, int32_t rolled,
                           ifx_bf16* scratch, void* stream) {
  IFX_REQUIRE(kv && kv->k && kv->v && scratch, "ifx_kv_roll: null argument");
  IFX_REQUIRE(sink_tokens >= 0 && evicted >= 0 && rolled >= 0 &&
                  sink_tokens + evicted + rolled <= kv->num_slots,
              "ifx_kv_roll: span out of range");
  if (const int rc = check_writer_view("ifx_kv_roll", kv)) return rc;
  if (rolled == 0 || evicted == 0) return IFX_OK;
  const int row_elems = kv->kv_heads * kv->head_dim;
  KvAddr ka{kv->page_table, kv->page_size};
  const int blocks = 1024;
  for (int which = 0; which < 2; ++which) {
    unsigned short* c = which == 0 ? kv->k : kv->v;
    hipLaunchKernelGGL(kv_copy_rows_kernel, dim3(blocks), dim3(256), 0, (hipStream_t)stream, c, scratch, ka,
                       sink_tokens + evicted, 0, rolled, row_elems, 1, 0);
    hipLaunchKernelGGL(kv_copy_rows_kernel, dim3(blocks), dim3(256), 0, (hipStream_t)stream, scratch, c, ka, 0,
                       sink_tokens, rolled, row_elems, 0, 1);
  }
  return check_launch("ifx_kv_roll");
}

extern "C" int ifx_kv_scatter_shards(const ifx_bf16* gathered, int32_t world, int32_t frames, int32_t hw_local,
                                     int32_t frame_tokens, int32_t local_start, const ifx_kv_view* kv, void* stream) {
  IFX_REQUIRE(gathered && kv && kv->k && kv->v, "ifx_kv_scatter_shards: null argument");
  IFX_REQUIRE(world > 0 && frames > 0 && hw_local > 0 && world * hw_local <= frame_tokens && local_start >= 0,
              "ifx_kv_scatter_shards: bad shard geometry (world %d, frames %d, hw_local %d, frame_tokens %d)", world,
              frames, hw_local, frame_tokens);
  IFX_REQUIRE(local_start + (frames - 1) * frame_tokens + world * hw_local <= kv->num_slots,
              "ifx_kv_scatter_shards: tokens [%d, %d) exceed the cache capacity %d", local_start,
              local_start + (frames - 1) * frame_tokens + world * hw_local, kv->num_slots);
  if (const int rc = check_writer_view("ifx_kv_scatter_shards", kv)) return rc;
  const int row_elems = kv->kv_heads * kv->head_dim;
  IFX_REQUIRE(row_elems % 8 == 0, "ifx_kv_scatter_shards: row of %d elements is not 16-byte granular", row_elems);
  const size_t total = (size_t)world * frames * hw_local * (row_elems / 8);
  const int blocks = (int)((total + 255) / 256 < 4096 ? (total + 255) / 256 : 4096);
  hipLaunchKernelGGL(kv_scatter_shards_kernel, dim3(blocks), dim3(256), 0, (hipStream_t)stream, gathered, kv->k, kv->v,
                     KvAddr{kv->page_table, kv->page_size}, world, frames, hw_local, frame_tokens, local_start, row_elems);
  return check_launch("ifx_kv_scatter_shards");
}
```

### inferix_amd/csrc/ifx_rows.h

```cpp
#pragma once
#include <type_traits>

#include "ifx_common.h"

namespace ifx {

template <int NCH>
__device__ __forceinline__ void load_chunks(u16x8 (&u)[NCH], const unsigned short* p, int dim, int lane) {
#pragma unroll
  for (int c = 0; c < NCH; ++c) {
    const int col = c * 512 + lane * 8;
    u[c] = *reinterpret_cast<const u16x8*>(p + (col < dim ? col : 0));
  }
}

template <int NCH>
struct Row {
  float v[NCH][8];
  __device__ __forceinline__ void from(const u16x8 (&u)[NCH], int dim, int lane) {
#pragma unroll
    for (int c = 0; c < NCH; ++c) {
      const bool ok = c * 512 + lane * 8 < dim;
#pragma unroll
      for (int i = 0; i < 8; ++i) v[c][i] = ok ? bf2f(u[c][i]) : 0.f;
    }
  }
  __device__ __forceinline__ float sum() const {
    float s = 0.f;
#pragma unroll
    for (int c = 0; c < NCH; ++c)
#pragma unroll
      for (int i = 0; i < 8; ++i) s += v[c][i];
    return s;
  }
  __device__ __forceinline__ float sumsq() const {
    float s = 0.f;
#pragma unroll
    for (int c = 0; c < NCH; ++c)
#pragma unroll
      for (int i = 0; i < 8; ++i) s += v[c][i] * v[c][i];
    return s;
  }
};

template <int NCH>
__device__ __forceinline__ void ln_stats(const Row<NCH>& row, int dim, float eps, int lane, float& mean, float& rstd) {
  const float inv_n = 1.0f / (float)dim;
  mean = wave_sum(row.sum()) * inv_n;
  float ss = 0.f;
#pragma unroll
  for (int c = 0; c < NCH; ++c) {
    if (c * 512 + lane * 8 < dim) {
#pragma unroll
      for (int i = 0; i < 8; ++i) {
        const float d = row.v[c][i] - mean;
        ss += d * d;
      }
    }
  }
  rstd = 1.0f / sqrtf(wave_sum(ss) * inv_n + eps);
}

template <bool FP8>
__device__ __forceinline__ u32x2 pack8(const float (&v)[8]) {
  if (FP8) {
    unsigned w0 = 0, w1 = 0;
    w0 = __builtin_amdgcn_cvt_pk_fp8_f32(v[0], v[1], w0, false);
    w0 = __builtin_amdgcn_cvt_pk_fp8_f32(v[2], v[3], w0, true);
    w1 = __builtin_amdgcn_cvt_pk_fp8_f32(v[4], v[5], w1, false);
    w1 = __builtin_amdgcn_cvt_pk_fp8_f32(v[6], v[7], w1, true);
    return u32x2{w0, w1};
  }
  unsigned w[2] = {0, 0};
#pragma unroll
  for (int i = 0; i < 8; ++i) w[i >> 2] |= ((unsigned)(int)rintf(v[i]) & 0xffu) << (8 * (i & 3));
  return u32x2{w[0], w[1]};
}

template <bool FP8, int NCH>
__device__ __forceinline__ void quant_row_dynamic(const u16x8 (&u)[NCH], unsigned char* qr, float* scale, int dim, int lane) {
  constexpr float QMAX = FP8 ? 448.0f : 127.0f;
  float amax = 0.f;
#pragma unroll
  for (int c = 0; c < NCH; ++c)
#pragma unroll
    for (int i = 0; i < 8; ++i) amax = fmaxf(amax, fabsf(bf2f(u[c][i])));
  amax = wave_max(amax);
  const float s = amax > 0.f ? amax / QMAX : 1.0f;
  if (lane == 0) *scale = s;
  const RowDivisor rdiv(s);
  auto emit = [&](auto fastc) {
#pragma unroll
    for (int c = 0; c < NCH; ++c) {
      const int col = c * 512 + lane * 8;
      float v[8];
#pragma unroll
      for (int i = 0; i < 8; ++i) v[i] = fminf(fmaxf(rdiv.template div<decltype(fastc)::value>(bf2f(u[c][i])), -QMAX), QMAX);
      const u32x2 pk = pack8<FP8>(v);
      if (col < dim) *reinterpret_cast<u32x2*>(qr + col) = pk;
    }
  };
  if (rdiv.fast()) emit(std::true_type{});
  else emit(std::false_type{});
}

template <bool FP8>
__device__ __forceinline__ u32x2 div_clamp8(const float (&x)[8], const f32x4 d0, const f32x4 d1, int via_bf16) {
  constexpr float QMAX = FP8 ? 448.0f : 127.0f;
  float v[8];
#pragma unroll
  for (int i = 0; i < 8; ++i) {
    const float t = fminf(fmaxf(x[i] / (i < 4 ? d0[i] : d1[i - 4]), -QMAX), QMAX);
    v[i] = via_bf16 ? rbf(t) : t;
  }
  return pack8<FP8>(v);
}

struct RopeArgs {
  const double* freqs;
  int max_pos, start_frame, height, width, hw_offset, hw_local;
  float q_scale = 1.0f;
};

__device__ __forceinline__ void rope4(float (&t)[8], int jp0, const RopeArgs& ra, int half, int n_t,
                                      int n_h, int pos_t, int pos_h, int pos_w) {
#pragma unroll
  for (int p = 0; p < 4; ++p) {
    const int j = jp0 + p;
    const int pos = (j < n_t) ? pos_t : ((j < n_t + n_h) ? pos_h : pos_w);
    const double2 cs = *reinterpret_cast<const double2*>(ra.freqs + ((size_t)pos * half + j) * 2);
    const double a = (double)t[2 * p], b = (double)t[2 * p + 1];
    const double re = __dmul_rn(a, cs.x) - __dmul_rn(b, cs.y);
    const double im = __dmul_rn(a, cs.y) + __dmul_rn(b, cs.x);
    t[2 * p] = (float)re;
    t[2 * p + 1] = (float)im;
  }
}

__device__ __forceinline__ void rope4_cs(float (&t)[8], const double2 (&cs)[4]) {
#pragma unroll
  for (int p = 0; p < 4; ++p) {
    const double a = (double)t[2 * p], b = (double)t[2 * p + 1];
    const double re = __dmul_rn(a, cs[p].x) - __dmul_rn(b, cs[p].y);
    const double im = __dmul_rn(a, cs[p].y) + __dmul_rn(b, cs[p].x);
    t[2 * p] = (float)re;
    t[2 * p + 1] = (float)im;
  }
}

struct RopeToken {
  int pos_t = 0, pos_h = 0, pos_w = 0;
  int half, n_t, n_h;
  bool shared_cs;
  double2 cs4[4];
  __device__ __forceinline__ RopeToken(const RopeArgs& ra, int has_rope, int r, int head_dim, int lane)
      : half(head_dim >> 1), n_t(half - 2 * (half / 3)), n_h(half / 3), shared_cs(has_rope && (512 % head_dim) == 0) {
    if (has_rope) {
      const int f = r / ra.hw_local;
      const int p = ra.hw_offset + (r - f * ra.hw_local);
      pos_t = ra.start_frame + f;
      pos_h = p / ra.width;
      pos_w = p - pos_h * ra.width;
    }
    if (shared_cs) {
      const int jp0 = ((lane * 8) % head_dim) >> 1;
#pragma unroll
      for (int p = 0; p < 4; ++p) {
        const int j = jp0 + p;
        const int pos = (j < n_t) ? pos_t : ((j < n_t + n_h) ? pos_h : pos_w);
        cs4[p] = *reinterpret_cast<const double2*>(ra.freqs + ((size_t)pos * half + j) * 2);
      }
    }
  }
};

template <int NCH, typename Put>
__device__ __forceinline__ void rmsnorm_rope_row(Row<NCH>& row, const u16x8 (&raw)[NCH], const u16x8 (&wv)[NCH], const RopeToken& tk,
                                                 const RopeArgs& ra, int has_rope, float out_scale, int dim, int head_dim, float eps,
                                                 int lane, Put&& put) {
  row.from(raw, dim, lane);
  const float rs = 1.0f / sqrtf(wave_sum(row.sumsq()) / (float)dim + eps);
#pragma unroll
  for (int c = 0; c < NCH; ++c) {
    const int col = c * 512 + lane * 8;
    float t[8];
#pragma unroll
    for (int i = 0; i < 8; ++i) t[i] = rbf(rbf(row.v[c][i] * rs) * bf2f(wv[c][i]));
    if (tk.shared_cs) rope4_cs(t, tk.cs4);
    else if (has_rope && col < dim) rope4(t, (col % head_dim) >> 1, ra, tk.half, tk.n_t, tk.n_h, tk.pos_t, tk.pos_h, tk.pos_w);
    u16x8 o;
#pragma unroll
    for (int i = 0; i < 8; ++i) o[i] = f2bf(t[i] * out_scale);
    if (col < dim) put(c, col, o);
  }
}

template <int N, int... WIDER, typename F>
static int dispatch_nch(int dim, const char* too_wide, F&& f) {
  if (N == 0 || (dim + 511) / 512 <= N) return f(std::integral_constant<int, N>{});
  if constexpr (sizeof...(WIDER) > 0) return dispatch_nch<WIDER...>(dim, too_wide, f);
  set_error(too_wide, dim);
  return IFX_EUNSUP;
}

template <typename K, typename... A>
static int launch_rows(const char* who, K kernel, int rows, void* stream, A... args) {
  hipLaunchKernelGGL(kernel, dim3((rows + 3) / 4), dim3(256), 0, (hipStream_t)stream, args...);
  return check_launch(who);
}

template <typename F>
static int dispatch_q8_format(int format, F&& f) {
  return format == IFX_Q_FP8_E4M3 ? f(std::true_type{}) : f(std::false_type{});
}

static int check_ln_mode(const char* who, int mode, const void* gamma, const void* beta, const void* mod, int mod_slots,
                         int shift_slot, int scale_slot, int rows_per_group) {
  IFX_REQUIRE(mode >= IFX_LN_PLAIN && mode <= IFX_LN_MODULATE, "%s: bad mode %d", who, mode);
  if (mode == IFX_LN_AFFINE) IFX_REQUIRE(gamma && beta, "%s: affine mode needs gamma/beta", who);
  if (mode == IFX_LN_MODULATE)
    IFX_REQUIRE(mod && rows_per_group > 0 && mod_slots > 0 && shift_slot >= 0 && shift_slot < mod_slots &&
                    scale_slot >= 0 && scale_slot < mod_slots,
                "%s: modulate mode needs mod/slots/rows_per_group", who);
  return IFX_OK;
}

static int resolve_rope(const char* who, const ifx_rope_grid* rope, int head_dim, int dim, int rows, RopeArgs* ra) {
  if (rope == nullptr) return IFX_OK;
  IFX_REQUIRE(rope->freqs && rope->hw_local > 0 && rope->width > 0 && rope->height > 0, "%s: bad rope grid", who);
  IFX_REQUIRE(head_dim % 16 == 0 && dim % head_dim == 0, "%s: head_dim %d", who, head_dim);
  IFX_REQUIRE(rope->hw_offset >= 0 && (long long)rope->hw_offset + rope->hw_local <= (long long)rope->height * rope->width,
              "%s: rope hw_offset %d + hw_local %d outside the %d x %d grid", who, rope->hw_offset, rope->hw_local, rope->height,
              rope->width);
  const int frames = (rows + rope->hw_local - 1) / rope->hw_local;
  IFX_REQUIRE(rope->start_frame + frames <= rope->max_pos && rope->height <= rope->max_pos && rope->width <= rope->max_pos,
              "%s: positions exceed rope table (%d)", who, rope->max_pos);
  *ra = RopeArgs{rope->freqs, rope->max_pos, rope->start_frame, rope->height, rope->width, rope->hw_offset, rope->hw_local};
  return IFX_OK;
}

static int check_writer_view(const char* who, const ifx_kv_view* kv) {
  if (kv->page_table) IFX_REQUIRE(kv->page_size > 0, "%s: page_size must be > 0", who);
  else IFX_REQUIRE(kv->seg_split <= 0, "%s: kv view with a two-segment map (seg_split %d) and no page table: the map is for readers",
                   who, kv->seg_split);
  return IFX_OK;
}

}
```

### inferix_amd/hip_ops.py

```python
from __future__ import annotations

import ctypes as C
import threading
from dataclasses import dataclass
from typing import Sequence, Optional, Tuple

import torch

from . import _hip

BF16 = torch.bfloat16
F32 = torch.float32


class KernelTimer:

    def __init__(self, names=("attn_self",)):
        self.names = set(names)
        self.records = []

    def wants(self, name: str) -> bool:
        return name in self.names

    def summary(self):
        torch.cuda.synchronize()
        out = {}
        for name, s, e, fl, by in self.records:
            d = out.setdefault(name, dict(launches=0, ms=0.0, flops=0.0, bytes=0.0))
            d["launches"] += 1
            d["ms"] += s.elapsed_time(e)
            d["flops"] += fl
            d["bytes"] += by
        return out


_timer: Optional[KernelTimer] = None


def set_kernel_timer(t: Optional[KernelTimer]) -> None:
    global _timer
    _timer = t


class _Timing:
    def __init__(self, name, flops, nbytes):
        self.name, self.flops, self.nbytes = name, flops, nbytes

    def __enter__(self):
        self.s = torch.cuda.Event(enable_timing=True)
        self.e = torch.cuda.Event(enable_timing=True)
        self.s.record()

    def __exit__(self, *a):
        self.e.record()
        _timer.records.append((self.name, self.s, self.e, self.flops, self.nbytes))


class _NotTimed:
    __slots__ = ()

    def __enter__(self):
        return None

    def __exit__(self, *a):
        return False


_NOT_TIMED = _NotTimed()


def _timed(name, flops=0.0, nbytes=0.0):
    if _timer is None or name not in _timer.names:
        return _NOT_TIMED
    return _Timing(name, flops, nbytes)


_raw_stream = torch._C._cuda_getCurrentRawStream
_cur_device = torch._C._cuda_getDevice


def _stream() -> int:
    return _raw_stream(_cur_device())


def _dev(t: torch.Tensor, name: str, dtype=BF16) -> int:
    if not t.is_cuda:
        raise _hip.HipKernelError(f"{name}: tensor is on {t.device}; inferix_amd ops run on the GPU only")
    if t.dtype != dtype:
        raise TypeError(f"{name}: expected {dtype}, got {t.dtype}")
    if t.dim() and t.stride(-1) != 1:
        raise ValueError(f"{name}: innermost dimension must be contiguous")
    return t.data_ptr()


def _rows2d(t: torch.Tensor, name: str) -> Tuple[int, int, int]:
    if t.dim() == 1:
        return 1, t.shape[0], t.shape[0]
    if t.dim() > 2:
        if t.is_contiguous():
            t = t.flatten(0, -2)
        else:
            try:
                t = t.view(-1, t.shape[-1])
            except RuntimeError as e:
                raise ValueError(f"{name}: tensor of shape {tuple(t.shape)} / strides {t.stride()} is not a matrix of "
                                 "uniformly strided rows; make it contiguous first") from e
    return t.shape[0], t.shape[1], t.stride(0)


@dataclass
class KvCacheView:
    k: torch.Tensor
    v: torch.Tensor
    page_table: Optional[torch.Tensor] = None
    page_size: int = 1
    seg_split: int = 0
    seg_delta: int = 0

    def struct(self) -> _hip.KvView:
        key = (self.k.data_ptr(), self.v.data_ptr(), None if self.page_table is None else self.page_table.data_ptr(), self.page_size,
               self.seg_split, self.seg_delta)
        memo = self.__dict__.get("_memo")
        if memo is not None and memo[0] == key:
            return memo[1]
        assert self.k.shape == self.v.shape and self.k.dim() == 3 and self.k.is_contiguous() and self.v.is_contiguous()
        pt = 0
        if self.page_table is not None:
            pt = _dev(self.page_table, "page_table", torch.int32)
        assert not (self.seg_split and self.page_table is not None), "a view has a page table or a two-segment map, not both"
        st = _hip.KvView(_dev(self.k, "kv.k"), _dev(self.v, "kv.v"), pt, int(self.page_size),
                         self.k.shape[0], self.k.shape[1], self.k.shape[2], int(self.seg_split), int(self.seg_delta))
        self.__dict__["_memo"] = (key, st)
        return st

    @staticmethod
    def from_manager_tensor(t: torch.Tensor, page_table=None, page_size=1) -> "KvCacheView":
        assert t.dim() == 5 and t.shape[0] == 2 and t.is_contiguous()
        return KvCacheView(t[0].flatten(0, 1), t[1].flatten(0, 1), page_table, page_size)


@dataclass
class RopeGridSpec:
    freqs: torch.Tensor
    start_frame: int
    height: int
    width: int
    hw_offset: int = 0
    hw_local: Optional[int] = None
    q_scale: float = 0.0

    def struct(self) -> _hip.RopeGrid:
        hl = self.hw_local if self.hw_local is not None else self.height * self.width
        return _hip.RopeGrid(_dev(self.freqs, "rope.freqs", torch.float64), self.freqs.shape[0],
                             int(self.start_frame), int(self.height), int(self.width), int(self.hw_offset), int(hl),
                             float(self.q_scale))


def attn_q_prescale(head_dim: int) -> Tuple[float, float]:
    return (head_dim ** -0.5) * 1.4426950408889634, 0.6931471805599453


def _ln_mode(rows: int, dim: int, gamma, beta, mod, shift_slot: int, scale_slot: int, rows_per_group: Optional[int]):
    if mod is not None:
        assert mod.dim() == 3 and mod.shape[-1] == dim and mod.is_contiguous() and rows_per_group
        assert rows <= mod.shape[0] * rows_per_group
        return _hip.IFX_LN_MODULATE, (None, None, _dev(mod, "mod"), mod.shape[1], shift_slot, scale_slot, rows_per_group)
    if gamma is not None:
        return _hip.IFX_LN_AFFINE, (_dev(gamma, "gamma"), _dev(beta, "beta"), None, 0, 0, 0, 1)
    return _hip.IFX_LN_PLAIN, (None, None, None, 0, 0, 0, 1)


def layernorm(x: torch.Tensor, eps: float, *, gamma=None, beta=None, mod=None, shift_slot=0, scale_slot=1,
              rows_per_group: Optional[int] = None, out: Optional[torch.Tensor] = None) -> torch.Tensor:
    lib = _hip.load()
    rows, dim, ld = _rows2d(x, "x")
    assert ld == dim, "x rows must be dense"
    out = torch.empty_like(x) if out is None else out
    mode, args = _ln_mode(rows, dim, gamma, beta, mod, shift_slot, scale_slot, rows_per_group)
    with _timed("layernorm", 0.0, 4.0 * rows * dim):
        _hip.check(lib.ifx_layernorm(_dev(x, "x"), _dev(out, "out"), rows, dim, eps, mode, *args, _stream()),
                   "ifx_layernorm")
    return out


def layernorm_quant(x: torch.Tensor, eps: float, fmt: int, *, gamma=None, beta=None, mod=None, shift_slot=0, scale_slot=1,
                    rows_per_group: Optional[int] = None, q: Optional[torch.Tensor] = None,
                    scale: Optional[torch.Tensor] = None) -> Tuple[torch.Tensor, torch.Tensor]:
    lib = _hip.load()
    rows, dim, ld = _rows2d(x, "x")
    assert ld == dim, "x rows must be dense"
    q = torch.empty(rows, dim, dtype=torch.uint8, device=x.device) if q is None else q
    scale = torch.empty(rows, dtype=torch.float32, device=x.device) if scale is None else scale
    mode, args = _ln_mode(rows, dim, gamma, beta, mod, shift_slot, scale_slot, rows_per_group)
    with _timed("layernorm", 0.0, 3.0 * rows * dim):
        _hip.check(lib.ifx_layernorm_quant(_dev(x, "x"), _dev(q, "q", torch.uint8), q.stride(0), _dev(scale, "scale", torch.float32),
                                           rows, dim, eps, mode, *args, int(fmt), _stream()), "ifx_layernorm_quant")
    return q, scale


def rmsnorm(x: torch.Tensor, w: torch.Tensor, eps: float, out: Optional[torch.Tensor] = None) -> torch.Tensor:
    lib = _hip.load()
    rows, dim, ldx = _rows2d(x, "x")
    out = torch.empty(x.shape, dtype=x.dtype, device=x.device) if out is None else out
    _, _, ldy = _rows2d(out, "out")
    _hip.check(lib.ifx_rmsnorm(_dev(x, "x"), ldx, _dev(out, "out"), ldy, _dev(w, "w"), rows, dim, eps, _stream()),
               "ifx_rmsnorm")
    return out


def rmsnorm_rope_kv_append(qkv: torch.Tensor, wq: torch.Tensor, wk: Optional[torch.Tensor], eps: float,
                           rope: Optional[RopeGridSpec], kv: Optional[KvCacheView], local_start: int,
                           dim: int, q_out: Optional[torch.Tensor] = None, v_in_place: bool = False) -> torch.Tensor:
    lib = _hip.load()
    rows, _, ld = _rows2d(qkv, "qkv")
    q_out = torch.empty(rows, dim, dtype=BF16, device=qkv.device) if q_out is None else q_out
    rs = rope.struct() if rope is not None else None
    if v_in_place:
        assert rs is not None and kv is not None, "v_in_place needs a rope grid (it carries the flag) and a cache view"
        rs.flags = 1
    ks = kv.struct() if kv is not None else None
    nb = 2.0 * rows * dim * ((4 if v_in_place else 6) if kv is not None else 2)
    with _timed("rmsnorm_rope_append", 0.0, nb):
        _hip.check(lib.ifx_rmsnorm_rope_kv_append(
            _dev(qkv, "qkv"), ld, _dev(q_out, "q_out"), _dev(wq, "wq"), _dev(wk, "wk") if wk is not None else None,
            C.byref(rs) if rs is not None else None, C.byref(ks) if ks is not None else None,
            int(local_start), rows, dim, eps, _stream()), "ifx_rmsnorm_rope_kv_append")
    return q_out


_OPTIONS: dict = {}


def get_option(key: str) -> int:
    v = C.c_int32(0)
    _hip.check(_hip.load().ifx_get_option(key.encode(), C.byref(v)), "ifx_get_option")
    _OPTIONS[key] = int(v.value)
    if key == "gemm_small_split":
        _TLS.small_split = int(v.value)
    return int(v.value)


_TLS = threading.local()


def _small_split() -> int:
    v = getattr(_TLS, "small_split", None)
    return get_option("gemm_small_split") if v is None else v


def device_error(clear: bool = True) -> int:
    return int(_hip.load().ifx_device_error(1 if clear else 0))


def check_device(what: str = "", sync: bool = False) -> None:
    if sync and torch.cuda.is_available():
        torch.cuda.current_stream().synchronize()
    if device_error(clear=False):
        _GEMM_WS.clear()
        msg = _hip.load().ifx_last_error().decode("utf-8", "replace")
        raise _hip.HipKernelError(f"{what + ': ' if what else ''}{msg}")


def set_option(key: str, value: int) -> None:
    _hip.check(_hip.load().ifx_set_option(key.encode(), int(value)), "ifx_set_option")
    _OPTIONS[key] = int(value)
    if key == "gemm_small_split":
        _TLS.small_split = int(value)
    if key == "attn_variant":
        _SPLIT_PLAN.clear()
    if key == "gemm_variant":
        _GEMM_WS_NEED.clear()


class option_scope:

    def __init__(self, key: str, value: int):
        self.key, self.value, self.prev = key, int(value), 0

    def __enter__(self):
        self.prev = get_option(self.key)
        if self.prev != self.value:
            set_option(self.key, self.value)
        return self

    def __exit__(self, *exc):
        if self.prev != self.value:
            set_option(self.key, self.prev)
        return False


_ATTN_WS: dict = {}
_SPLIT_PLAN: dict = {}


def _split_plan(rows: int, heads: int, kv_start: int, kv_len: int) -> Tuple[int, int]:
    key = (rows, heads, kv_len - kv_start)
    plan = _SPLIT_PLAN.get(key)
    if plan is None:
        need = C.c_int64(0)
        plan = (int(_hip.load().ifx_attn_split_plan(rows, heads, int(kv_start), int(kv_len), C.byref(need))), int(need.value))
        _SPLIT_PLAN[key] = plan
    return plan


def _attn_workspace(dev: torch.device, nbytes: int) -> torch.Tensor:
    key = (dev.index, _stream())
    ws = _ATTN_WS.get(key)
    if ws is None or ws.numel() * 4 < nbytes:
        ws = torch.empty((nbytes + 3) // 4, dtype=torch.float32, device=dev)
        _ATTN_WS[key] = ws
    return ws


def attention(q: torch.Tensor, kv: KvCacheView, kv_len: int, scale: float = 0.0,
              out: Optional[torch.Tensor] = None, return_lse: bool = False, tag: str = "attn", kv_start: int = 0,
              splits: Optional[int] = None):
    lib = _hip.load()
    assert q.dim() == 3 and q.is_contiguous()
    rows, heads, hd = q.shape
    out = torch.empty_like(q) if out is None else out
    lse = torch.empty(heads, rows, dtype=torch.float32, device=q.device) if return_lse else None
    ks = kv.struct()
    d = heads * hd
    nk = kv_len - kv_start
    if splits is None:
        splits, ws_bytes = _split_plan(rows, heads, kv_start, kv_len)
    else:
        ws_bytes = splits * rows * heads * (hd + 1) * 4 if splits > 1 else 0
    lse_p = _dev(lse, "lse", torch.float32) if lse is not None else None
    with _timed(tag, 4.0 * rows * nk * d, 2.0 * (2 * rows * d + 2 * nk * d)):
        if splits > 1:
            ws = _attn_workspace(q.device, ws_bytes)
            _hip.check(lib.ifx_attn_fwd_paged_split(_dev(q, "q"), _dev(out, "out"), lse_p, C.byref(ks), rows, heads,
                                                    int(kv_start), int(kv_len), float(scale), int(splits),
                                                    ws.data_ptr(), ws.numel() * 4, _stream()),
                       "ifx_attn_fwd_paged_split")
        else:
            _hip.check(lib.ifx_attn_fwd_paged(_dev(q, "q"), _dev(out, "out"), lse_p, C.byref(ks), rows, heads,
                                              int(kv_start), int(kv_len), float(scale), _stream()),
                       "ifx_attn_fwd_paged")
    return (out, lse) if return_lse else out


def attention_split_plan(rows: int, heads: int, nkeys: int) -> int:
    return _split_plan(rows, heads, 0, nkeys)[0]


def attention_partial(q: torch.Tensor, kv: KvCacheView, kv_len: int, kv_start: int, splits: int, workspace: torch.Tensor,
                      slot_base: int, slot_cap: int, scale: float = 0.0, tag: str = "attn") -> int:
    rows, heads, hd = q.shape
    ks = kv.struct()
    used = C.c_int32(0)
    nk = kv_len - kv_start
    with _timed(tag, 4.0 * rows * nk * heads * hd, 2.0 * (2 * rows * heads * hd + 2 * nk * heads * hd)):
        _hip.check(_hip.load().ifx_attn_fwd_partial(_dev(q, "q"), C.byref(ks), rows, heads, int(kv_start), int(kv_len),
                                                    float(scale), int(splits), workspace.data_ptr(), workspace.numel() * 4,
                                                    int(slot_base), int(slot_cap), C.byref(used), _stream()),
                   "ifx_attn_fwd_partial")
    return int(used.value)


def attention_merge(workspace: torch.Tensor, slot_cap: int, slots_used: int, out: torch.Tensor,
                    lse: Optional[torch.Tensor] = None) -> None:
    rows, heads, _ = out.shape
    _hip.check(_hip.load().ifx_attn_merge_partials(workspace.data_ptr(), int(slot_cap), int(slots_used), _dev(out, "out"),
                                                   _dev(lse, "lse", torch.float32) if lse is not None else None, rows, heads,
                                                   _stream()), "ifx_attn_merge_partials")


def attention_workspace(q: torch.Tensor, slot_cap: int) -> torch.Tensor:
    rows, heads, hd = q.shape
    return _attn_workspace(q.device, slot_cap * rows * heads * (hd + 1) * 4)


def kv_scatter_shards(gathered: torch.Tensor, world: int, frames: int, hw_local: int, frame_tokens: int,
                      local_start: int, kv: KvCacheView) -> None:
    assert gathered.is_contiguous() and gathered.numel() == world * 2 * frames * hw_local * kv.k.shape[-2] * kv.k.shape[-1]
    ks = kv.struct()
    with _timed("kv_scatter", 0.0, 2.0 * gathered.numel() * 2):
        _hip.check(_hip.load().ifx_kv_scatter_shards(_dev(gathered, "gathered"), world, frames, hw_local, frame_tokens,
                                                     int(local_start), C.byref(ks), _stream()), "ifx_kv_scatter_shards")


class PeerBuffer:

    def __init__(self, nbytes: int, fine_grained: bool = False):
        p = C.c_void_p()
        _hip.check(_hip.load().ifx_peer_alloc(int(nbytes), 1 if fine_grained else 0, C.byref(p)), "ifx_peer_alloc")
        self.ptr, self.nbytes = int(p.value), int(nbytes)

    def free(self) -> None:
        if self.ptr:
            _hip.check(_hip.load().ifx_peer_free(self.ptr), "ifx_peer_free")
            self.ptr = 0

    def tensor(self, dtype: torch.dtype, shape) -> torch.Tensor:
        typestr = {torch.int32: "<i4", torch.bfloat16: "<u2", torch.uint8: "|u1", torch.float32: "<f4"}[dtype]
        holder = type("_Cai", (), {"__cuda_array_interface__": {"shape": tuple(shape), "typestr": typestr, "data": (self.ptr, False),
                                                                 "version": 2}, "_keep": self})()
        t = torch.as_tensor(holder, device="cuda")
        return t.view(torch.bfloat16) if dtype == torch.bfloat16 else t


def peer_export(ptr: int) -> Tuple[bytes, int]:
    h = C.create_string_buffer(_hip.IFX_PEER_HANDLE_BYTES)
    off = C.c_int64()
    _hip.check(_hip.load().ifx_peer_export(int(ptr), h, C.byref(off)), "ifx_peer_export")
    return h.raw, int(off.value)


def peer_open(handle: bytes) -> int:
    p = C.c_void_p()
    _hip.check(_hip.load().ifx_peer_open(C.create_string_buffer(handle, _hip.IFX_PEER_HANDLE_BYTES), C.byref(p)), "ifx_peer_open")
    return int(p.value)


def peer_close(ptr: int) -> None:
    _hip.check(_hip.load().ifx_peer_close(int(ptr)), "ifx_peer_close")


def rmsnorm_rope_kv_push(kv_rows: torch.Tensor, wk: torch.Tensor, eps: float, rope: Optional[RopeGridSpec], dest_k: Sequence[int],
                         dest_v: Sequence[int], geometry: KvCacheView, local_start: int, frame_tokens: int, slot_hw_local: int,
                         slot_hw_offset: int, dim: int) -> None:
    rows, cols, ld = _rows2d(kv_rows, "kv_rows")
    assert cols >= 2 * dim and len(dest_k) == len(dest_v) and 1 <= len(dest_k) <= _hip.IFX_MAX_PEERS
    pc = _hip.PeerCaches()
    pc.count = len(dest_k)
    for i, (a, b) in enumerate(zip(dest_k, dest_v)):
        pc.k[i], pc.v[i] = int(a), int(b)
    rs = rope.struct() if rope is not None else None
    gs = geometry.struct()
    with _timed("kv_push", 0.0, 2.0 * rows * dim * 2 * (1 + len(dest_k))):
        _hip.check(_hip.load().ifx_rmsnorm_rope_kv_push(
            _dev(kv_rows, "kv_rows"), ld, _dev(wk, "wk"), C.byref(rs) if rs is not None else None, C.byref(pc), C.byref(gs),
            int(local_start), int(frame_tokens), int(slot_hw_local), int(slot_hw_offset), rows, dim, eps, _stream()),
            "ifx_rmsnorm_rope_kv_push")


def peer_signal(flag_blocks: Sequence[int], index: int, value: int) -> None:
    pf = _hip.PeerFlags()
    pf.count = len(flag_blocks)
    for i, a in enumerate(flag_blocks):
        pf.flags[i] = int(a)
    _hip.check(_hip.load().ifx_peer_signal(C.byref(pf), int(index), int(value), _stream()), "ifx_peer_signal")


def peer_wait(flags_ptr: int, count: int, value: int, timeout_ms: int, status: Optional[torch.Tensor]) -> None:
    _hip.check(_hip.load().ifx_peer_wait(int(flags_ptr), int(count), int(value), int(timeout_ms),
                                         _dev(status, "status", torch.int32) if status is not None else None, _stream()), "ifx_peer_wait")


def lse_merge(out_a: torch.Tensor, lse_a: torch.Tensor, out_b: torch.Tensor, lse_b: torch.Tensor) -> None:
    lib = _hip.load()
    rows, heads, _ = out_a.shape
    _hip.check(lib.ifx_lse_merge(_dev(out_a, "out_a"), _dev(lse_a, "lse_a", torch.float32), _dev(out_b, "out_b"),
                                 _dev(lse_b, "lse_b", torch.float32), rows, heads, _stream()), "ifx_lse_merge")


def _epilogue(epilogue: int, M: int, N: int, residual: Optional[torch.Tensor] = None, mod: Optional[torch.Tensor] = None,
              gate_slot: int = 0, rows_per_group: int = 1) -> _hip.Epilogue:
    epi = _hip.Epilogue(epilogue, None, 0, None, 1, 0, 1)
    if residual is not None:
        _, _, ldr = _rows2d(residual, "residual")
        epi.residual, epi.ld_res = _dev(residual, "residual"), ldr
    if mod is not None:
        assert mod.dim() == 3 and mod.shape[-1] == N and mod.is_contiguous()
        assert rows_per_group > 0 and M <= mod.shape[0] * rows_per_group, "mod table does not cover every output row"
        epi.mod, epi.mod_slots, epi.gate_slot, epi.rows_per_group = _dev(mod, "mod"), mod.shape[1], gate_slot, rows_per_group
    return epi


def linear(x: torch.Tensor, w: torch.Tensor, bias: Optional[torch.Tensor], *, epilogue: int = _hip.IFX_EPI_BIAS,
           residual: Optional[torch.Tensor] = None, mod: Optional[torch.Tensor] = None, gate_slot: int = 0,
           rows_per_group: int = 1, out: Optional[torch.Tensor] = None, out2: Optional[torch.Tensor] = None,
           split_col: int = 0) -> torch.Tensor:
    lib = _hip.load()
    M, K, ldx = _rows2d(x, "x")
    N = w.shape[0]
    assert w.shape[1] == K and w.is_contiguous()
    if out is None:
        out = torch.empty(*x.shape[:-1], N, dtype=BF16, device=x.device)
    _, _, ldy = _rows2d(out, "out")
    epi = _epilogue(epilogue, M, N, residual, mod, gate_slot, rows_per_group)
    if out2 is not None:
        r2, c2, ld2 = _rows2d(out2, "out2")
        assert r2 == M and c2 == N - split_col and 0 < split_col < N, (out2.shape, M, N, split_col)
        epi.y2, epi.ldy2, epi.split_col = _dev(out2, "out2"), ld2, int(split_col)
    wkey = (M, N, K, _small_split())
    need = _GEMM_WS_NEED.get(wkey) if out2 is None else 0
    if need is None:
        need = _GEMM_WS_NEED[wkey] = int(lib.ifx_gemm_workspace_bytes(M, N, K))
    with _timed("gemm", 2.0 * M * N * K, 2.0 * (M * K + N * K + M * N * (2 if residual is not None else 1))):
        if need:
            ws = _gemm_workspace(x.device, need)
            _hip.check(lib.ifx_gemm_bf16_ws(_dev(x, "x"), ldx, _dev(w, "w"), _dev(bias, "bias") if bias is not None else None,
                                            _dev(out, "out"), ldy, M, N, K, C.byref(epi), ws.data_ptr(), ws.numel(), _stream()),
                       "ifx_gemm_bf16_ws")
        else:
            _hip.check(lib.ifx_gemm_bf16(_dev(x, "x"), ldx, _dev(w, "w"), _dev(bias, "bias") if bias is not None else None,
                                         _dev(out, "out"), ldy, M, N, K, C.byref(epi), _stream()), "ifx_gemm_bf16")
    return out


_GEMM_WS_NEED: dict = {}
_GEMM_WS: dict = {}


def _gemm_workspace(dev: torch.device, nbytes: int) -> torch.Tensor:
    key = (dev.index, _stream())
    ws = _GEMM_WS.get(key)
    if ws is None or ws.numel() < nbytes:
        ws = torch.zeros(nbytes, dtype=torch.uint8, device=dev)
        _GEMM_WS[key] = ws
    return ws


def quant_per_token(x: torch.Tensor, fmt: int, q: Optional[torch.Tensor] = None,
                    scale: Optional[torch.Tensor] = None) -> Tuple[torch.Tensor, torch.Tensor]:
    lib = _hip.load()
    rows, K, ldx = _rows2d(x, "x")
    q = torch.empty(rows, K, dtype=torch.uint8, device=x.device) if q is None else q
    scale = torch.empty(rows, dtype=torch.float32, device=x.device) if scale is None else scale
    with _timed("quant_per_token", 0.0, 3.0 * rows * K):
        _hip.check(lib.ifx_quant_per_token(_dev(x, "x"), ldx, _dev(q, "q", torch.uint8), q.stride(0),
                                           _dev(scale, "scale", torch.float32), rows, K, fmt, _stream()),
                   "ifx_quant_per_token")
    return q, scale


def linear_q8(xq: torch.Tensor, x_scale: torch.Tensor, wq: torch.Tensor, w_scale: torch.Tensor,
              bias: Optional[torch.Tensor], fmt: int, *, epilogue: int = _hip.IFX_EPI_BIAS,
              residual: Optional[torch.Tensor] = None, mod: Optional[torch.Tensor] = None, gate_slot: int = 0,
              rows_per_group: int = 1, out: Optional[torch.Tensor] = None) -> torch.Tensor:
    lib = _hip.load()
    M, K = xq.shape
    N = wq.shape[0]
    assert wq.shape[1] == K and wq.is_contiguous() and xq.stride(1) == 1
    out = torch.empty(M, N, dtype=BF16, device=xq.device) if out is None else out
    _, _, ldy = _rows2d(out, "out")
    epi = _epilogue(epilogue, M, N, residual, mod, gate_slot, rows_per_group)
    wkey = ("q8", M, N, K, _small_split())
    need = _GEMM_WS_NEED.get(wkey)
    if need is None:
        need = _GEMM_WS_NEED[wkey] = int(lib.ifx_gemm_q8_workspace_bytes(M, N, K))
    with _timed("gemm_q8", 2.0 * M * N * K, 1.0 * (M * K + N * K) + 2.0 * M * N):
        if need:
            ws = _gemm_workspace(xq.device, need)
            _hip.check(lib.ifx_gemm_q8_ws(_dev(xq, "xq", torch.uint8), xq.stride(0), _dev(x_scale, "x_scale", torch.float32),
                                          _dev(wq, "wq", torch.uint8), _dev(w_scale, "w_scale", torch.float32),
                                          _dev(bias, "bias") if bias is not None else None, _dev(out, "out"), ldy, M, N, K,
                                          fmt, C.byref(epi), ws.data_ptr(), ws.numel(), _stream()), "ifx_gemm_q8_ws")
        else:
            _hip.check(lib.ifx_gemm_q8(_dev(xq, "xq", torch.uint8), xq.stride(0), _dev(x_scale, "x_scale", torch.float32),
                                       _dev(wq, "wq", torch.uint8), _dev(w_scale, "w_scale", torch.float32),
                                       _dev(bias, "bias") if bias is not None else None, _dev(out, "out"), ldy, M, N, K,
                                       fmt, C.byref(epi), _stream()), "ifx_gemm_q8")
    return out


def linear_q8_quant_out(xq: torch.Tensor, x_scale: torch.Tensor, wq: torch.Tensor, w_scale: torch.Tensor, fmt: int, out_divisor: torch.Tensor,
                        *, epilogue: int = _hip.IFX_EPI_GELU_ERF, via_bf16: bool = True, out: Optional[torch.Tensor] = None) -> torch.Tensor:
    M, K = xq.shape
    N = wq.shape[0]
    assert wq.shape[1] == K and wq.is_contiguous() and xq.stride(1) == 1 and out_divisor.numel() == N
    out = torch.empty(M, N, dtype=torch.uint8, device=xq.device) if out is None else out
    epi = _epilogue(epilogue, M, N)
    with _timed("gemm_q8", 2.0 * M * N * K, 1.0 * (M * K + N * K) + 1.0 * M * N):
        _hip.check(_hip.load().ifx_gemm_q8_quant_out(_dev(xq, "xq", torch.uint8), xq.stride(0), _dev(x_scale, "x_scale", F32),
                                                     _dev(wq, "wq", torch.uint8), _dev(w_scale, "w_scale", F32), None,
                                                     _dev(out, "out", torch.uint8), out.stride(0), M, N, K, int(fmt), C.byref(epi),
                                                     _dev(out_divisor, "out_divisor", F32), 1 if via_bf16 else 0, _stream()),
                   "ifx_gemm_q8_quant_out")
    return out


def layernorm_quant_static(x: torch.Tensor, eps: float, divisors: torch.Tensor, gamma: Optional[torch.Tensor] = None,
                           beta: Optional[torch.Tensor] = None, via_bf16: bool = True) -> torch.Tensor:
    rows, dim, ldx = _rows2d(x, "x")
    assert ldx == dim, "layernorm_quant_static: dense rows"
    n_out = divisors.shape[0]
    assert divisors.shape == (n_out, dim) and divisors.is_contiguous()
    q = torch.empty(rows, n_out, dim, dtype=torch.uint8, device=x.device)
    mode = _hip.IFX_LN_AFFINE if gamma is not None else _hip.IFX_LN_PLAIN
    with _timed("layernorm", 0.0, (2.0 + n_out) * rows * dim):
        _hip.check(_hip.load().ifx_layernorm_quant_static(_dev(x, "x"), _dev(q, "q", torch.uint8), n_out * dim, _dev(divisors, "divisors", F32),
                                                          n_out, rows, dim, float(eps), mode, _dev(gamma, "gamma") if gamma is not None else None,
                                                          _dev(beta, "beta") if beta is not None else None, 1 if via_bf16 else 0, _stream()),
                   "ifx_layernorm_quant_static")
    return q


def kv_roll(kv: KvCacheView, sink_tokens: int, evicted: int, rolled: int, scratch: torch.Tensor) -> None:
    lib = _hip.load()
    ks = kv.struct()
    assert scratch.numel() >= rolled * kv.k.shape[1] * kv.k.shape[2]
    _hip.check(lib.ifx_kv_roll(C.byref(ks), sink_tokens, evicted, rolled, _dev(scratch, "scratch"), _stream()),
               "ifx_kv_roll")


_ZERO_PAGE = {}


def _zero_page(dev: torch.device) -> torch.Tensor:
    z = _ZERO_PAGE.get(dev)
    if z is None:
        z = _ZERO_PAGE[dev] = torch.zeros(256, dtype=torch.uint8, device=dev)
    return z


def _slots(v) -> "C.Array":
    return (C.c_int32 * len(v))(*[int(i) for i in v])


def to_planar(x: torch.Tensor) -> torch.Tensor:
    t, h, w, c = x.shape
    return x.view(t, h, w, c // 32, 32).permute(0, 3, 1, 2, 4).contiguous()


def conv3d_cl(x: torch.Tensor, in_slots, w: torch.Tensor, bias: Optional[torch.Tensor], *, kt: int, ks: int,
              y: torch.Tensor, out_slots, upsample: bool = False, residual: Optional[torch.Tensor] = None) -> torch.Tensor:
    t_out = len(out_slots)
    assert len(in_slots) == t_out + kt - 1, (len(in_slots), t_out, kt)
    in_planar = x.dim() == 5
    if in_planar:
        _, planes, hs, ws, c32 = x.shape
        assert c32 == 32
        cin = planes * 32
    else:
        _, hs, ws, cin = x.shape
    taps, cc, cout, c32 = w.shape
    assert taps == kt * ks * ks and c32 == 32 and cc * 32 == cin and x.is_contiguous() and y.is_contiguous() and w.is_contiguous()
    ho, wo = (hs * 2, ws * 2) if upsample else (hs, ws)
    assert tuple(y.shape[1:]) == (ho, wo, cout), (tuple(y.shape), ho, wo, cout)
    assert max(out_slots) < y.shape[0] and max(in_slots) < x.shape[0]
    if residual is not None:
        assert residual.is_contiguous() and tuple(residual.shape) == (t_out, ho, wo, cout)
    ins, outs = _slots(in_slots), _slots(out_slots)
    d = _hip.Conv3dDesc(_dev(x, "x"), hs * ws * cin, ins, hs, ws, cin, 1 if upsample else 0, _dev(w, "w"),
                        _dev(bias, "bias") if bias is not None else None, kt, ks, _dev(y, "y"), ho * wo * cout, outs, cout,
                        t_out, _dev(residual, "residual") if residual is not None else None,
                        _zero_page(x.device).data_ptr(), 1 if in_planar else 0)
    flops = 2.0 * t_out * ho * wo * cout * cin * taps
    with _timed("conv3d", flops, 0.0):
        _hip.check(_hip.load().ifx_conv3d_cl(C.byref(d), _stream()), "ifx_conv3d_cl")
    return y


def rmsnorm_cl(x: torch.Tensor, gamma: torch.Tensor, y: torch.Tensor, out_slots, silu: bool) -> torch.Tensor:
    frames, h, w_, c = x.shape
    out_planar = y.dim() == 5
    assert x.is_contiguous() and y.is_contiguous() and len(out_slots) == frames
    assert tuple(y.shape[1:]) == ((c // 32, h, w_, 32) if out_planar else (h, w_, c)), (tuple(y.shape), tuple(x.shape))
    assert gamma.numel() == c and max(out_slots) < y.shape[0]
    with _timed("rmsnorm_cl", 0.0, 4.0 * x.numel()):
        _hip.check(_hip.load().ifx_rmsnorm_cl(_dev(x, "x"), _dev(gamma, "gamma"), _dev(y, "y"), h * w_ * c, _slots(out_slots),
                                              frames, h * w_, c, (1 if silu else 0) | (2 if out_planar else 0), _stream()), "ifx_rmsnorm_cl")
    return y


def softmax_rows(scores: torch.Tensor, scale: float, out: Optional[torch.Tensor] = None) -> torch.Tensor:
    rows, cols = scores.shape
    ld = scores.stride(0)
    out = torch.empty_like(scores) if out is None else out
    assert scores.stride(1) == 1 and out.stride() == scores.stride()
    _hip.check(_hip.load().ifx_softmax_rows(_dev(scores, "scores"), _dev(out, "probs"), rows, cols, ld, float(scale),
                                            _stream()), "ifx_softmax_rows")
    return out


def t5_attention(q: torch.Tensor, k: torch.Tensor, v: torch.Tensor, rel_bias: torch.Tensor, seq_lens: torch.Tensor,
                 batch: int, heads: int, out: Optional[torch.Tensor] = None) -> torch.Tensor:
    rows = q.shape[0]
    L = rows // batch
    assert rows == batch * L and q.shape[1] == heads * 64 and k.shape == q.shape and v.shape == q.shape
    assert tuple(rel_bias.shape) == (heads, 2 * L - 1) and rel_bias.is_contiguous()
    assert seq_lens.dtype == torch.int32 and seq_lens.is_cuda and seq_lens.numel() == batch
    out = torch.empty(rows, heads * 64, dtype=BF16, device=q.device) if out is None else out
    with _timed("attn_t5", 4.0 * batch * heads * L * L * 64, 0.0):
        _hip.check(_hip.load().ifx_t5_attention(_dev(q, "q"), q.stride(0), _dev(k, "k"), k.stride(0), _dev(v, "v"), v.stride(0),
                                                _dev(out, "out"), out.stride(0), _dev(rel_bias, "rel_bias"),
                                                seq_lens.data_ptr(), batch, L, heads, _stream()), "ifx_t5_attention")
    return out


def t5_gated_gelu(gate_fc1: torch.Tensor, out: Optional[torch.Tensor] = None) -> torch.Tensor:
    rows, two_ffn = gate_fc1.shape
    ffn = two_ffn // 2
    assert gate_fc1.is_contiguous()
    out = torch.empty(rows, ffn, dtype=BF16, device=gate_fc1.device) if out is None else out
    _hip.check(_hip.load().ifx_t5_gated_gelu(_dev(gate_fc1, "gate_fc1"), _dev(out, "h"), rows, ffn, _stream()),
               "ifx_t5_gated_gelu")
    return out


def attention_ld(q: torch.Tensor, kv: KvCacheView, kv_len: int, out: torch.Tensor, heads: int, kv_start: int = 0,
                 scale: float = 0.0, tag: str = "attn") -> torch.Tensor:
    lib = _hip.load()
    rows = q.shape[0]
    assert q.dim() == 2 and out.dim() == 2 and out.shape[0] == rows and q.stride(1) == 1 and out.stride(1) == 1
    assert q.shape[1] >= heads * 128 and out.shape[1] >= heads * 128
    ks = kv.struct()
    nk = kv_len - kv_start
    splits, ws_bytes = _split_plan(rows, heads, kv_start, kv_len)
    ws = _attn_workspace(q.device, ws_bytes) if splits > 1 else None
    d = heads * 128
    with _timed(tag, 4.0 * rows * nk * d, 2.0 * (2 * rows * d + 2 * nk * kv.k.shape[1] * 128)):
        _hip.check(lib.ifx_attn_fwd_paged_ld(_dev(q, "q"), q.stride(0), _dev(out, "out"), out.stride(0), None, C.byref(ks), rows,
                                             heads, int(kv_start), int(kv_len), float(scale), int(splits),
                                             ws.data_ptr() if ws is not None else None,
                                             ws.numel() * 4 if ws is not None else 0, _stream()), "ifx_attn_fwd_paged_ld")
    return out


def magi_head_prep(mixed: torch.Tensor, *, layout: int, q_heads: int, kv_heads: int, eps: float, layernorm_1p: bool,
                   k_out: torch.Tensor, v_out: torch.Tensor, kv_head_stride: int, ld_kv: int, row0: int = 0,
                   split: Optional[int] = None, row1: int = 0, rope: Optional[torch.Tensor] = None, qn=None, kn=None, xn=None,
                   q_out: Optional[torch.Tensor] = None, qx_out: Optional[torch.Tensor] = None, q_scale: float = 0.0,
                   q_group: int = 0) -> None:
    rows = mixed.shape[0]
    assert mixed.dim() == 2 and mixed.stride(1) == 1
    d = _hip.MagiHeadPrepDesc()
    d.inp, d.ld_in, d.rows, d.layout = _dev(mixed, "mixed"), mixed.stride(0), rows, layout
    d.q_heads, d.kv_heads, d.head_dim = q_heads, kv_heads, 128
    d.eps, d.layernorm_1p = float(eps), 1 if layernorm_1p else 0
    if layout == 0:
        assert rope is not None and rope.is_contiguous() and rope.dim() == 2 and rope.shape[0] == rows
        assert rope.shape[1] % 16 == 0 and rope.shape[1] <= 128, "rope rows are (sin | cos) of at most 64 pairs, a multiple of 8 each"
        d.rope = _dev(rope, "rope", F32)
        d.rope_half = rope.shape[1] // 2
        d.qn_w, d.qn_b = _dev(qn[0], "q_layernorm.weight", F32), _dev(qn[1], "q_layernorm.bias", F32)
        d.kn_w, d.kn_b = _dev(kn[0], "k_layernorm.weight", F32), _dev(kn[1], "k_layernorm.bias", F32)
        if q_group > 0:
            assert q_out.dim() == 3 and q_out.is_contiguous() and q_out.shape == (q_heads // q_group, rows, q_group * 128), q_out.shape
            d.q_out, d.ld_q, d.q_group, d.q_group_stride = _dev(q_out, "q_out"), q_group * 128, int(q_group), rows * q_group * 128
        else:
            d.q_out, d.ld_q = _dev(q_out, "q_out"), q_out.stride(0)
            assert q_out.shape[0] >= rows
        d.qx_out, d.ld_qx = _dev(qx_out, "qx_out"), qx_out.stride(0)
        assert qx_out.shape[0] >= rows
    d.xn_w, d.xn_b = _dev(xn[0], "layernorm_xattn.weight"), _dev(xn[1], "layernorm_xattn.bias")
    d.k_out, d.v_out, d.ld_kv, d.kv_head_stride = _dev(k_out, "k_out"), _dev(v_out, "v_out"), int(ld_kv), int(kv_head_stride)
    d.row0, d.split, d.row1 = int(row0), int(rows if split is None else split), int(row1)
    d.q_scale = float(q_scale)
    n_heads = (2 * q_heads + 2 * kv_heads) if layout == 0 else 2 * kv_heads
    with _timed("magi_head_prep", 0.0, 4.0 * rows * n_heads * 128):
        _hip.check(_hip.load().ifx_magi_head_prep(C.byref(d), _stream()), "ifx_magi_head_prep")


def kv_split_rows(kv: torch.Tensor, k_cache: torch.Tensor, v_cache: torch.Tensor, row0: int, split: int, row1: int) -> None:
    n, heads, hd2 = kv.shape
    assert hd2 == 256 and kv.is_contiguous() and k_cache.is_contiguous() and v_cache.is_contiguous()
    assert k_cache.shape[1:] == (heads, 128) and v_cache.shape == k_cache.shape
    assert 0 <= split <= n and row0 + split <= k_cache.shape[0] and row1 + (n - split) <= k_cache.shape[0]
    _hip.check(_hip.load().ifx_kv_split_rows(_dev(kv, "kv"), _dev(k_cache, "k_cache"), _dev(v_cache, "v_cache"), n, heads, int(row0),
                                             int(split), int(row1), _stream()), "ifx_kv_split_rows")


def magi_gate_norm_residual(x: torch.Tensor, residual: torch.Tensor, condition_map: torch.Tensor, gate: torch.Tensor,
                            norm_w: torch.Tensor, norm_b: torch.Tensor, eps: float, layernorm_1p: bool,
                            out: Optional[torch.Tensor] = None) -> torch.Tensor:
    rows, dim, ldx = _rows2d(x, "x")
    _, _, ldr = _rows2d(residual, "residual")
    out = torch.empty(rows, dim, dtype=BF16, device=x.device) if out is None else out
    _, _, ldy = _rows2d(out, "out")
    assert gate.dim() == 2 and gate.shape[1] == dim and gate.stride(1) == 1
    assert condition_map.dtype == torch.int32 and condition_map.is_cuda and condition_map.numel() == rows and condition_map.is_contiguous()
    with _timed("magi_gate_norm", 0.0, 6.0 * rows * dim):
        _hip.check(_hip.load().ifx_magi_gate_norm_residual(
            _dev(x, "x"), ldx, _dev(residual, "residual"), ldr, condition_map.data_ptr(), _dev(gate, "gate"), gate.stride(0),
            _dev(norm_w, "norm_w", F32), _dev(norm_b, "norm_b", F32), 1 if layernorm_1p else 0, _dev(out, "out"), ldy, rows, dim,
            float(eps), _stream()), "ifx_magi_gate_norm_residual")
    return out


def act_rows(x: torch.Tensor, mode: int, out: Optional[torch.Tensor] = None) -> torch.Tensor:
    assert x.is_contiguous()
    out = torch.empty_like(x) if out is None else out
    _hip.check(_hip.load().ifx_act_rows(_dev(x, "x"), _dev(out, "out"), x.numel(), int(mode), _stream()), "ifx_act_rows")
    return out


def quant_static(x: torch.Tensor, divisor: torch.Tensor, fmt: int, via_bf16: bool, q: Optional[torch.Tensor] = None,
                 row_scale: Optional[torch.Tensor] = None) -> torch.Tensor:
    rows, K, ldx = _rows2d(x, "x")
    q = torch.empty(rows, K, dtype=torch.uint8, device=x.device) if q is None else q
    divisor = divisor.reshape(-1)
    with _timed("quant_static", 0.0, 3.0 * rows * K):
        _hip.check(_hip.load().ifx_quant_static(_dev(x, "x"), ldx, _dev(q, "q", torch.uint8), q.stride(0), _dev(divisor, "divisor", F32),
                                                divisor.numel(), _dev(row_scale, "row_scale", F32) if row_scale is not None else None,
                                                rows, K, int(fmt), 1 if via_bf16 else 0, _stream()), "ifx_quant_static")
    return q


_AMAX_WS: dict = {}


def quant_per_tensor(x: torch.Tensor, fmt: int, q: Optional[torch.Tensor] = None,
                     scale: Optional[torch.Tensor] = None) -> Tuple[torch.Tensor, torch.Tensor]:
    rows, K, ldx = _rows2d(x, "x")
    q = torch.empty(rows, K, dtype=torch.uint8, device=x.device) if q is None else q
    scale = torch.empty(rows, dtype=F32, device=x.device) if scale is None else scale
    key = (x.device.index, _stream())
    ws = _AMAX_WS.get(key)
    if ws is None:
        ws = _AMAX_WS[key] = torch.zeros(1, dtype=torch.int32, device=x.device)
    _hip.check(_hip.load().ifx_quant_per_tensor(_dev(x, "x"), ldx, _dev(q, "q", torch.uint8), q.stride(0), _dev(scale, "scale", F32),
                                                ws.data_ptr(), rows, K, int(fmt), _stream()), "ifx_quant_per_tensor")
    return q, scale


def attention_ranges(q: torch.Tensor, kv: KvCacheView, q_ranges, k_ranges, out: torch.Tensor, heads: int, scale: float = 0.0,
                     tag: str = "attn") -> torch.Tensor:
    n = len(q_ranges)
    assert 1 <= n <= 8 and len(k_ranges) == n and q.dim() == 2 and out.dim() == 2 and q.stride(1) == 1 and out.stride(1) == 1
    rows = q.shape[0]
    qa = (C.c_int32 * (2 * n))(*[int(v) for r in q_ranges for v in r])
    ka = (C.c_int32 * (2 * n))(*[int(v) for r in k_ranges for v in r])
    ks = kv.struct()
    d = heads * 128
    flops = sum(4.0 * (qe - qs) * (ke - kb) * d for (qs, qe), (kb, ke) in zip(q_ranges, k_ranges))
    with _timed(tag, flops, 0.0):
        _hip.check(_hip.load().ifx_attn_fwd_ranges(_dev(q, "q"), q.stride(0), _dev(out, "out"), out.stride(0), C.byref(ks), rows, heads,
                                                   n, qa, ka, float(scale), _stream()), "ifx_attn_fwd_ranges")
    return out


def attention_dedup(q: torch.Tensor, kv: KvCacheView, kv_len: int, last_key_multiplicity: int, out: Optional[torch.Tensor] = None,
                    scale: float = 0.0, tag: str = "attn") -> torch.Tensor:
    assert q.dim() == 3 and q.is_contiguous()
    rows, heads, hd = q.shape
    out = torch.empty_like(q) if out is None else out
    ks = kv.struct()
    nk = kv_len - 1 + last_key_multiplicity
    with _timed(tag, 4.0 * rows * nk * heads * hd, 0.0):
        _hip.check(_hip.load().ifx_attn_fwd_dedup(_dev(q, "q"), _dev(out, "out"), C.byref(ks), rows, heads, int(kv_len),
                                                  int(last_key_multiplicity), float(scale), _stream()), "ifx_attn_fwd_dedup")
    return out
```

### inferix_amd/wan/causal_model.py

```python
from __future__ import annotations

import math
import os
from dataclasses import dataclass
from typing import Dict, List, Optional, Sequence, Tuple

import torch
import torch.nn.functional as F

from .. import _hip, hip_ops as ops
from ..kvcache_manager import KVCacheManager, KVCacheRequest
from ..kvcache_manager.model import SelfForcingKVCacheManagerFactory
from . import components as C

BF16 = torch.bfloat16


class ParallelConfig:

    def __init__(self, ulysses_size=1, ring_size=1, local_rank=0, rank=0, world_size=1,
                 ring_strategy="pass-kv", attn_backend=None):
        from ..attention import collect_supported_attn
        ulysses_size, ring_size, world_size = int(ulysses_size), int(ring_size), int(world_size)
        if ulysses_size < 1 or ring_size < 1:
            raise ValueError(f"ulysses_size={ulysses_size} / ring_size={ring_size}: degrees must be >= 1")
        if ulysses_size * ring_size not in (1, world_size):
            raise ValueError(f"ulysses_size={ulysses_size} x ring_size={ring_size} != world_size={world_size}: the sequence-parallel "
                             "degree is ulysses_size * ring_size and must equal the number of ranks")
        self.ulysses_size, self.ring_size = ulysses_size, ring_size
        self.local_rank, self.rank, self.world_size = local_rank, rank, world_size
        self.ring_strategy = ring_strategy
        supported = collect_supported_attn()
        if attn_backend is None:
            attn_backend = "HipPagedFA"
        if attn_backend not in supported:
            raise ValueError(f"Specified attention backend '{attn_backend}' is not available. "
                             f"Available backends: {list(supported)}")
        self.attn_backend = attn_backend


@dataclass
class KVIndexStep:
    local_start: int
    local_end: int
    global_end: int
    evicted: int
    rolled: int
    sink_tokens: int


def kv_index_update(global_end: int, local_end: int, current_start: int, num_new: int, cache_size: int,
                    local_attn_size: int, sink_tokens: int) -> KVIndexStep:
    current_end = current_start + num_new
    evicted = rolled = 0
    if local_attn_size != -1 and current_end > global_end and num_new + local_end > cache_size:
        evicted = num_new + local_end - cache_size
        rolled = local_end - evicted - sink_tokens
    new_local_end = local_end + current_end - global_end - evicted
    return KVIndexStep(new_local_end - num_new, new_local_end, current_end, evicted, rolled, sink_tokens)


class _Block:

    def __init__(self, layer_idx: int, num_heads: int, head_dim: int, enable_kv_offload: bool):
        self.layer_idx = layer_idx
        self.kv_cache_manager = SelfForcingKVCacheManagerFactory.create_manager(
            layer_idx, num_heads, head_dim, enable_kv_offload=enable_kv_offload)
        self.w: Dict[str, torch.Tensor] = {}
        self.cross_meta = {"is_init": False}

    @property
    def is_cross_attn_init(self) -> bool:
        return self.cross_meta["is_init"]

    @is_cross_attn_init.setter
    def is_cross_attn_init(self, v: bool) -> None:
        self.cross_meta["is_init"] = bool(v)


class HipCausalWanModel(torch.nn.Module):
    def __init__(self, model_type="t2v", patch_size=(1, 2, 2), text_len=512, in_dim=16, dim=2048, ffn_dim=8192,
                 freq_dim=256, text_dim=4096, out_dim=16, num_heads=16, num_layers=32, local_attn_size=-1,
                 sink_size=0, qk_norm=True, cross_attn_norm=True, eps=1e-6, enable_kv_offload=False,
                 parallel_config: Optional[ParallelConfig] = None, device="cuda"):
        super().__init__()
        if model_type != "t2v":
            raise NotImplementedError("HipCausalWanModel: only the t2v cross-attention path is built")
        if not (qk_norm and cross_attn_norm):
            raise NotImplementedError("HipCausalWanModel: qk_norm and cross_attn_norm are always on (Wan2.1 config)")
        if dim % num_heads or dim // num_heads != 128:
            raise NotImplementedError("HipCausalWanModel: kernels are built for head_dim 128")
        _hip.load()
        self.model_type, self.patch_size, self.text_len = model_type, tuple(patch_size), text_len
        self.in_dim, self.dim, self.ffn_dim, self.freq_dim = in_dim, dim, ffn_dim, freq_dim
        self.text_dim, self.out_dim, self.num_heads, self.num_layers = text_dim, out_dim, num_heads, num_layers
        self.head_dim = dim // num_heads
        self.local_attn_size, self.sink_size, self.eps = local_attn_size, sink_size, eps
        self.qk_norm, self.cross_attn_norm = qk_norm, cross_attn_norm
        self.enable_kv_offload = enable_kv_offload
        self.parallel_config = parallel_config if parallel_config is not None else ParallelConfig()
        pc = self.parallel_config
        u, r = int(getattr(pc, "ulysses_size", 1)), int(getattr(pc, "ring_size", 1))
        if u * r not in (1, int(getattr(pc, "world_size", 1))):
            raise ValueError(f"CausalWanModel: ulysses_size={u} x ring_size={r} must equal world_size={getattr(pc, 'world_size', 1)} "
                             "(both degrees map onto the one sequence-parallel exchange; see ParallelConfig)")
        self.num_frame_per_block = 1
        self.independent_first_frame = False
        self.device_ = torch.device(device)
        self.blocks: List[_Block] = [_Block(i, num_heads, self.head_dim, enable_kv_offload) for i in range(num_layers)]
        self.g: Dict[str, torch.Tensor] = {}
        self.mod_all: Optional[torch.Tensor] = None
        self.freqs = C.rope_table(self.head_dim).to(self.device_)
        self._scratch: Dict[Tuple, torch.Tensor] = {}
        self.cross_dedup = True
        self._cross_dedup: Dict[str, Tuple[int, int]] = {}
        self._roll_scratch: Optional[torch.Tensor] = None
        self.v_direct = os.environ.get("IFX_V_DIRECT", "1") != "0"
        self._temb_cache: Dict[Tuple, Tuple] = {}
        self.index_trace: Optional[list] = None
        self._chain = 0
        self._pair_stream: Optional[torch.cuda.Stream] = None
        self.cp = None
        self.q_prescale = self.head_dim == 128

    def parameters(self, recurse: bool = True):
        for t in self.g.values():
            yield t
        for b in self.blocks:
            for t in b.w.values():
                if isinstance(t, torch.Tensor):
                    yield t

    def state_dict_keys(self) -> List[str]:
        keys = ["patch_embedding.weight", "patch_embedding.bias"]
        for n in ("text_embedding.0", "text_embedding.2", "time_embedding.0", "time_embedding.2", "time_projection.1"):
            keys += [n + ".weight", n + ".bias"]
        for i in range(self.num_layers):
            p = f"blocks.{i}."
            keys += [p + "modulation", p + "norm3.weight", p + "norm3.bias"]
            for a in ("self_attn", "cross_attn"):
                for n in ("q", "k", "v", "o"):
                    keys += [p + f"{a}.{n}.weight", p + f"{a}.{n}.bias"]
                keys += [p + f"{a}.norm_q.weight", p + f"{a}.norm_k.weight"]
            keys += [p + "ffn.0.weight", p + "ffn.0.bias", p + "ffn.2.weight", p + "ffn.2.bias"]
        keys += ["head.modulation", "head.head.weight", "head.head.bias"]
        return keys

    def load_state_dict(self, sd: Dict[str, torch.Tensor], strict: bool = True, assign: bool = False):
        missing = [k for k in self.state_dict_keys() if k not in sd]
        if missing and strict:
            raise KeyError(f"missing keys in state_dict: {missing[:5]}{'...' if len(missing) > 5 else ''}")
        dev = self.device_

        def t(name):
            return sd[name].detach().to(device=dev, dtype=BF16).contiguous()

        g = self.g
        g["patch_w"] = t("patch_embedding.weight").flatten(1).contiguous()
        g["patch_b"] = t("patch_embedding.bias")
        for short, n in (("text0", "text_embedding.0"), ("text2", "text_embedding.2"), ("time0", "time_embedding.0"),
                         ("time2", "time_embedding.2"), ("tproj", "time_projection.1"), ("head", "head.head")):
            g[short + "_w"], g[short + "_b"] = t(n + ".weight"), t(n + ".bias")
        g["head_mod"] = t("head.modulation")
        mods = []
        for i, blk in enumerate(self.blocks):
            p = f"blocks.{i}."
            w = blk.w
            w["qkv_w"] = torch.cat([t(p + f"self_attn.{n}.weight") for n in "qkv"], dim=0).contiguous()
            w["qkv_b"] = torch.cat([t(p + f"self_attn.{n}.bias") for n in "qkv"], dim=0).contiguous()
            w["nq"], w["nk"] = t(p + "self_attn.norm_q.weight"), t(p + "self_attn.norm_k.weight")
            w["o_w"], w["o_b"] = t(p + "self_attn.o.weight"), t(p + "self_attn.o.bias")
            w["n3_w"], w["n3_b"] = t(p + "norm3.weight"), t(p + "norm3.bias")
            for n in "qkvo":
                w[f"c{n}_w"], w[f"c{n}_b"] = t(p + f"cross_attn.{n}.weight"), t(p + f"cross_attn.{n}.bias")
            w["cnq"], w["cnk"] = t(p + "cross_attn.norm_q.weight"), t(p + "cross_attn.norm_k.weight")
            w["f0_w"], w["f0_b"] = t(p + "ffn.0.weight"), t(p + "ffn.0.bias")
            w["f2_w"], w["f2_b"] = t(p + "ffn.2.weight"), t(p + "ffn.2.bias")
            mods.append(t(p + "modulation"))
        self.mod_all = torch.stack(mods, dim=0).contiguous()
        self._temb_cache.clear()
        return self

    def _buf(self, name: str, *shape) -> torch.Tensor:
        key = (self._chain, name, shape)
        b = self._scratch.get(key)
        if b is None:
            b = torch.empty(*shape, dtype=BF16, device=self.device_)
            self._scratch[key] = b
        return b

    @staticmethod
    def _meta_int(v) -> int:
        return int(v.item()) if isinstance(v, torch.Tensor) else int(v)

    @staticmethod
    def _meta_set(meta: dict, key: str, value: int) -> None:
        cur = meta.get(key)
        if isinstance(cur, torch.Tensor):
            cur.fill_(value)
        else:
            meta[key] = value

    def _kv_view(self, mgr: KVCacheManager, req: KVCacheRequest, name: str) -> ops.KvCacheView:
        t = mgr.get_raw(req, name)
        pt = mgr.page_table(req, name) if hasattr(mgr, "page_table") else None
        caches = getattr(mgr, "request_to_kv_caches", {}).get(getattr(req, "request_id", None))
        store = getattr(caches, "views", None)
        key = (t.data_ptr(), None if pt is None else (pt.device.data_ptr(), pt.page_size))
        if store is not None:
            hit = store.get(name)
            if hit is not None and hit[0] == key:
                return hit[1]
        if not t.is_cuda:
            raise _hip.HipKernelError(
                f"KV cache '{name}' lives on {t.device}: the HIP path reads pages in place from HBM "
                "(create the model with enable_kv_offload=False)")
        if pt is not None:
            v = ops.KvCacheView.from_manager_tensor(t, pt.device, pt.page_size)
        else:
            v = ops.KvCacheView.from_manager_tensor(t)
        if store is not None:
            store[name] = (key, v)
        return v

    def _evict(self, mgr, req, name: str, view: ops.KvCacheView, step: KVIndexStep) -> None:
        pt = mgr.page_table(req, name) if hasattr(mgr, "page_table") else None
        if pt is not None and step.sink_tokens % pt.page_size == 0 and step.evicted % pt.page_size == 0 \
                and step.rolled % pt.page_size == 0:
            mgr.rotate_pages(req, name, step.sink_tokens // pt.page_size, step.evicted // pt.page_size,
                             step.rolled // pt.page_size)
            return
        need = step.rolled * self.dim
        if self._chain:
            ops.kv_roll(view, step.sink_tokens, step.evicted, step.rolled, self._buf("roll", need))
            return
        if self._roll_scratch is None or self._roll_scratch.numel() < need:
            self._roll_scratch = torch.empty(need, dtype=BF16, device=self.device_)
        ops.kv_roll(view, step.sink_tokens, step.evicted, step.rolled, self._roll_scratch)

    def _q8_scratch(self, rows: int, cols: int, device):
        c = self._chain
        xq = self._scratch.get((c, "xq", rows, cols))
        if xq is None:
            xq = torch.empty(rows, cols, dtype=torch.uint8, device=device)
            self._scratch[(c, "xq", rows, cols)] = xq
            self._scratch[(c, "xs", rows)] = torch.empty(rows, dtype=torch.float32, device=device)
        return xq, self._scratch[(c, "xs", rows)]

    def _lin(self, w: Dict[str, torch.Tensor], key: str, x: torch.Tensor, **kw) -> torch.Tensor:
        if key + "_q" in w:
            fmt = w[key + "_fmt"]
            xq, xs = self._q8_scratch(x.shape[0], x.shape[1], x.device)
            if w.get(key + "_act") == "per_tensor":
                ops.quant_per_tensor(x, fmt, q=xq, scale=xs)
            else:
                ops.quant_per_token(x, fmt, q=xq, scale=xs)
            return ops.linear_q8(xq, xs, w[key + "_q"], w[key + "_s"], w[key + "_b"], fmt, **kw)
        return ops.linear(x, w[key + "_w"], w[key + "_b"], **kw)

    def _norm_lin(self, w: Dict[str, torch.Tensor], key: str, x: torch.Tensor, h: torch.Tensor, norm_kw: dict, **kw) -> torch.Tensor:
        if key + "_q" in w:
            fmt = w[key + "_fmt"]
            xq, xs = self._q8_scratch(x.shape[0], x.shape[1], x.device)
            if w.get(key + "_act") == "per_tensor":
                ops.layernorm(x, self.eps, out=h, **norm_kw)
                ops.quant_per_tensor(h, fmt, q=xq, scale=xs)
            else:
                ops.layernorm_quant(x, self.eps, fmt, q=xq, scale=xs, **norm_kw)
            return ops.linear_q8(xq, xs, w[key + "_q"], w[key + "_s"], w[key + "_b"], fmt, **kw)
        ops.layernorm(x, self.eps, out=h, **norm_kw)
        return ops.linear(h, w[key + "_w"], w[key + "_b"], **kw)

    def _run_block(self, l: int, xact: torch.Tensor, El: torch.Tensor, st: dict, meta: dict, cmeta: dict,
                   kv_cache_manager, kv_cache_requests) -> None:
        blk = self.blocks[l]
        w = blk.w
        d, H, hd = self.dim, self.num_heads, self.head_dim
        B, N, rows_per_group, rope = st["B"], st["N"], st["rows_per_group"], st["rope"]
        sink_tokens, current_start, ctx = st["sink_tokens"], st["current_start"], st["ctx"]
        h = self._buf("h", B * N, d)
        qkv = self._buf("qkv", B * N, 3 * d)
        qb = self._buf("q", B * N, d)
        ab = self._buf("a", B * N, d)
        ub = self._buf("u", B * N, self.ffn_dim)
        explicit0 = st.get("explicit_slots")
        samples = st.get("samples")
        if samples is None:
            samples = [dict(req=req, rope=rope, current_start=current_start, explicit=explicit0, ctx_index=b)
                       for b, req in enumerate(kv_cache_requests)]
        lockstep = bool(st.get("lockstep"))
        explicit_any = any(smp["explicit"] is not None for smp in samples)
        if not explicit_any:
            g_end, l_end = self._meta_int(meta["global_end_index"]), self._meta_int(meta["local_end_index"])
        else:
            g_end = l_end = 0
        steps_done: List[KVIndexStep] = []

        def index_state(smp=None):
            if lockstep and smp is not None and smp.get("fwd", 0) > 0:
                prev = [stp for stp, s0 in zip(steps_done, samples) if s0.get("fwd", 0) == smp["fwd"] - 1]
                if prev:
                    return prev[-1].global_end, prev[-1].local_end
            return g_end, l_end
        step = None
        kv_first = self.cp is not None and self.cp.kv_first and "qkv_q" not in w
        if kv_first:
            ops.layernorm(xact, self.eps, out=h, mod=El, shift_slot=0, scale_slot=1, rows_per_group=rows_per_group)
            kvp = self._buf("kvp", B * N, 2 * d)
            ops.linear(h, w["qkv_w"][d:], w["qkv_b"][d:], out=kvp)
            name = blk.kv_cache_manager.self_name
            pending = []
            for b, smp in enumerate(samples):
                ge, le = index_state(smp)
                pst = self.cp.begin(self, l, self._kv_view(kv_cache_manager, smp["req"], name), kvp[b * N:(b + 1) * N], w, smp["rope"],
                                    smp["current_start"], ge, le, sink_tokens, kv_cache_manager, smp["req"], name)
                pending.append(pst)
                steps_done.append(pst["step"])
            qraw = self._buf("qraw", B * N, d)
            ops.linear(h, w["qkv_w"][:d], w["qkv_b"][:d], out=qraw)
            for b, pst in enumerate(pending):
                ops.rmsnorm_rope_kv_append(qraw[b * N:(b + 1) * N], w["nq"], None, self.eps, samples[b]["rope"], None, 0, d,
                                           q_out=qb[b * N:(b + 1) * N])
                step = self.cp.finish(self, pst, qb[b * N:(b + 1) * N], ab[b * N:(b + 1) * N])
        planned: List[Tuple[KVIndexStep, ops.KvCacheView]] = []
        v_direct = None

        def plan(smp):
            name = blk.kv_cache_manager.self_name
            view = self._kv_view(kv_cache_manager, smp["req"], name)
            ge, le = index_state(smp)
            if smp["explicit"] is not None:
                step = KVIndexStep(smp["explicit"][0], smp["explicit"][1], smp["explicit"][1], 0, 0, 0)
            else:
                step = kv_index_update(ge, le, smp["current_start"], N, view.k.shape[0], self.local_attn_size, sink_tokens)
            if step.local_start < 0 or step.local_end > view.k.shape[0]:
                raise _hip.HipKernelError(f"KV cache overflow: slots [{step.local_start}, {step.local_end}) of "
                                          f"{view.k.shape[0]} (layer {l})")
            if step.evicted:
                self._evict(kv_cache_manager, smp["req"], name, view, step)
                view = self._kv_view(kv_cache_manager, smp["req"], name)
            steps_done.append(step)
            return step, view
        if not kv_first and self.cp is None and not lockstep:
            planned = [plan(smp) for smp in samples]
            step0, view0 = planned[0]
            if (self.v_direct and len(samples) == 1 and B * N >= 2048 and "qkv_q" not in w and view0.page_table is None
                    and not view0.seg_split and d % 256 == 0 and ops.get_option("gemm_variant") in (0, 22, 23, 24, 25)):
                v_direct = view0.v.view(view0.v.shape[0], d)[step0.local_start:step0.local_start + N]
        if not kv_first:
            extra = dict(out2=v_direct, split_col=2 * d) if v_direct is not None else {}
            self._norm_lin(w, "qkv", xact, h, dict(mod=El, shift_slot=0, scale_slot=1, rows_per_group=rows_per_group), out=qkv, **extra)
        for b, smp in enumerate(() if kv_first else samples):
            req, rope_b = smp["req"], smp["rope"]
            name = blk.kv_cache_manager.self_name
            if self.cp is not None:
                view = self._kv_view(kv_cache_manager, req, name)
                ge, le = index_state(smp)
                step = self.cp.self_attention(self, l, b, view, qkv[b * N:(b + 1) * N], qb[b * N:(b + 1) * N],
                                              ab[b * N:(b + 1) * N], w, rope_b, smp["current_start"], ge, le,
                                              sink_tokens, kv_cache_manager, req, name)
                steps_done.append(step)
                continue
            step, view = planned[b] if planned else plan(smp)
            ops.rmsnorm_rope_kv_append(qkv[b * N:(b + 1) * N], w["nq"], w["nk"], self.eps, rope_b, view,
                                       step.local_start, d, q_out=qb[b * N:(b + 1) * N], v_in_place=v_direct is not None)
            ops.attention(qb[b * N:(b + 1) * N].view(N, H, hd), view, step.local_end, scale=st.get("attn_scale", 0.0),
                          out=ab[b * N:(b + 1) * N].view(N, H, hd), tag="attn_self")
        if not explicit_any:
            self._meta_set(meta, "global_end_index", step.global_end)
            self._meta_set(meta, "local_end_index", step.local_end)
        if self.index_trace is not None and l == 0:
            for smp, stp in zip(samples, steps_done if steps_done else [step] * len(samples)):
                if smp["ctx_index"] == 0:
                    self.index_trace.append((int(smp["current_start"]), int(stp.global_end), int(stp.local_end)))
        self._lin(w, "o", ab, epilogue=_hip.IFX_EPI_GATE_RES, residual=xact, mod=El, gate_slot=2,
                  rows_per_group=rows_per_group, out=xact)
        self._norm_lin(w, "cq", xact, h, dict(gamma=w["n3_w"], beta=w["n3_b"]), out=qb)
        ops.rmsnorm(qb, w["cnq"], self.eps, out=qb)
        b = 0
        while b < len(samples):
            req = samples[b]["req"]
            nb = 1
            while b + nb < len(samples) and samples[b + nb]["req"] is req:
                nb += 1
            cview = self._kv_view(kv_cache_manager, req, blk.kv_cache_manager.cross_name)
            if not cmeta["is_init"]:
                ci = samples[b]["ctx_index"]
                cb = ctx[ci * self.text_len:(ci + 1) * self.text_len]
                kx = self._lin(w, "ck", cb)
                ops.rmsnorm(kx, w["cnk"], self.eps, out=cview.k.view(self.text_len, d))
                self._lin(w, "cv", cb, out=cview.v.view(self.text_len, d))
            nkeys, mult = self._cross_dedup.get(req.request_id, (self.text_len, 1)) if self.cross_dedup else (self.text_len, 1)
            qv, av = qb[b * N:(b + nb) * N].view(nb * N, H, hd), ab[b * N:(b + nb) * N].view(nb * N, H, hd)
            if mult > 1:
                ops.attention_dedup(qv, cview, nkeys, mult, out=av, tag="attn_cross")
            else:
                ops.attention(qv, cview, self.text_len, out=av, tag="attn_cross")
            b += nb
        cmeta["is_init"] = True
        self._lin(w, "co", ab, epilogue=_hip.IFX_EPI_RESIDUAL, residual=xact, out=xact)
        self._norm_lin(w, "f0", xact, h, dict(mod=El, shift_slot=3, scale_slot=4, rows_per_group=rows_per_group),
                       epilogue=_hip.IFX_EPI_GELU_TANH, out=ub)
        self._lin(w, "f2", ub, epilogue=_hip.IFX_EPI_GATE_RES, residual=xact, mod=El, gate_slot=5,
                  rows_per_group=rows_per_group, out=xact)


    @torch.no_grad()
    def forward(self, x, t, context, seq_len=None, clip_fea=None, y=None, kv_cache_meta=None,
                crossattn_cache_meta=None, current_start: int = 0, cache_start=None,
                kv_cache_manager: Optional[KVCacheManager] = None,
                kv_cache_requests: Optional[Sequence[KVCacheRequest]] = None,
                kv_start: Optional[int] = None, kv_end: Optional[int] = None,
                current_end: Optional[int] = None) -> torch.Tensor:
        fw = self._prologue(x, t, context, kv_cache_meta, crossattn_cache_meta, current_start, kv_cache_manager, kv_cache_requests,
                            kv_start, kv_end)
        with self._small_split_scope():
            for l in range(self.num_layers):
                self._run_block(l, fw["xact"], fw["E"][l], fw["st"], fw["kv_meta"][l], fw["cross_meta"][l], kv_cache_manager,
                                kv_cache_requests)
        return self._epilogue(fw)

    def _small_split_scope(self):
        import contextlib
        return ops.option_scope("gemm_small_split", 1) if getattr(self.cp, "gemm_small_split", False) else contextlib.nullcontext()

    @torch.no_grad()
    def forward_pair(self, first: dict, second: dict):
        if self._pair_mode() == "lockstep":
            return self._forward_pair_lockstep(first, second)
        dev = self.device_
        main = torch.cuda.current_stream(dev)
        if self._pair_stream is None:
            self._pair_stream = torch.cuda.Stream(device=dev)
        side = self._pair_stream
        side.wait_stream(main)
        kvm, reqs = first["kv_cache_manager"], first["kv_cache_requests"]
        assert second["kv_cache_manager"] is kvm, "forward_pair: both forwards must address the same cache"

        def pro(kw):
            return self._prologue(kw["x"], kw["t"], kw["context"], kw.get("kv_cache_meta"), kw.get("crossattn_cache_meta"),
                                  kw.get("current_start", 0), kw["kv_cache_manager"], kw["kv_cache_requests"], kw.get("kv_start"),
                                  kw.get("kv_end"))
        try:
            fa = pro(first)
            self._chain = 1
            with torch.cuda.stream(side):
                fb = pro(second)
            with self._small_split_scope():
                for l in range(self.num_layers):
                    self._chain = 0
                    self._run_block(l, fa["xact"], fa["E"][l], fa["st"], fa["kv_meta"][l], fa["cross_meta"][l], kvm, reqs)
                    ev = torch.cuda.Event()
                    ev.record(main)
                    self._chain = 1
                    with torch.cuda.stream(side):
                        side.wait_event(ev)
                        self._run_block(l, fb["xact"], fb["E"][l], fb["st"], fb["kv_meta"][l], fb["cross_meta"][l], kvm,
                                        second["kv_cache_requests"])
            self._chain = 0
            ya = self._epilogue(fa)
            self._chain = 1
            with torch.cuda.stream(side):
                yb = self._epilogue(fb)
        finally:
            self._chain = 0
        main.wait_stream(side)
        yb.record_stream(main)
        return ya, yb

    def _pair_mode(self) -> str:
        import os
        m = getattr(self, "pair_mode", None) or os.environ.get("IFX_PAIR_MODE", "")
        return m if m in ("streams", "lockstep") else "streams"

    def _forward_pair_lockstep(self, first: dict, second: dict):
        kvm, reqs = first["kv_cache_manager"], list(first["kv_cache_requests"])
        assert second["kv_cache_manager"] is kvm and list(second["kv_cache_requests"]) == reqs, \
            "forward_pair: both forwards must address the same requests"
        d = self.dim

        def pro(kw, out):
            return self._prologue(kw["x"], kw["t"], kw["context"], kw.get("kv_cache_meta"), kw.get("crossattn_cache_meta"),
                                  kw.get("current_start", 0), kvm, reqs, kw.get("kv_start"), kw.get("kv_end"), xact_out=out)
        lat = first["x"] if isinstance(first["x"], torch.Tensor) else torch.stack(list(first["x"]))
        B = lat.shape[0]
        pt_, ph, pw = self.patch_size
        rows = B * (lat.shape[2] // pt_) * (lat.shape[3] // ph) * (lat.shape[4] // pw) // self.parallel_config.world_size
        x2 = self._buf("x2", 2 * rows, d)
        fa = pro(first, x2[:rows])
        self._chain = 1
        try:
            fb = pro(second, x2[rows:])
        finally:
            self._chain = 0
        if fa["N"] != fb["N"] or fa["rows_per_group"] != fb["rows_per_group"] or fa["grid"] != fb["grid"]:
            raise ValueError("forward_pair (lockstep): the two forwards must have the same latent geometry and timestep layout")
        N = fa["N"]
        E2 = torch.cat([fa["E"], fb["E"]], dim=1).contiguous()
        eh2 = torch.cat([fa["eh"], fb["eh"]], dim=0).contiguous()
        sa, sb = fa["st"], fb["st"]
        samples = [dict(req=r, rope=s_["rope"], current_start=s_["current_start"], explicit=s_.get("explicit_slots"), ctx_index=b, fwd=f)
                   for f, s_ in enumerate((sa, sb)) for b, r in enumerate(reqs)]
        st = dict(sa, B=2 * B, samples=samples, lockstep=True, ctx=sa["ctx"] if sa["ctx"] is not None else sb["ctx"])
        if sa["ctx"] is None and sb["ctx"] is not None or any(not m["is_init"] for m in fa["cross_meta"]):
            raise RuntimeError("forward_pair: the cross-attention cache must be initialised before two forwards are paired")
        with self._small_split_scope():
            for l in range(self.num_layers):
                self._run_block(l, x2, E2[l], st, fa["kv_meta"][l], fa["cross_meta"][l], kvm, reqs)
        h2 = self._buf("h", 2 * B * N, d)
        ops.layernorm(x2, self.eps, mod=eh2, shift_slot=0, scale_slot=1, rows_per_group=fa["rows_per_group"], out=h2)
        yv = self._lin(self.g, "head", h2)
        if self.cp is not None:
            yv = self.cp.gather_head(yv, 2 * B, fa["F_"])
        y = C.unpatchify(yv, 2 * B, fa["grid"], self.patch_size, self.out_dim)
        return y[:B], y[B:]

    def _prologue(self, x, t, context, kv_cache_meta, crossattn_cache_meta, current_start, kv_cache_manager, kv_cache_requests,
                  kv_start=None, kv_end=None, xact_out: Optional[torch.Tensor] = None) -> dict:
        explicit = None
        if kv_start is not None and kv_end is not None:
            explicit = (int(kv_start), int(kv_end))
            kv_cache_meta = [dict() for _ in range(self.num_layers)]
            crossattn_cache_meta = [b.cross_meta for b in self.blocks]
        if kv_cache_meta is None:
            raise NotImplementedError("HipCausalWanModel implements the KV-cached inference path only")
        assert kv_cache_manager is not None and kv_cache_requests is not None
        if self.mod_all is None:
            raise RuntimeError("HipCausalWanModel: weights not loaded (call load_state_dict first)")
        dev, d, L = self.device_, self.dim, self.num_layers
        lat = torch.stack(list(x)) if not isinstance(x, torch.Tensor) else x
        lat = lat.to(device=dev, dtype=BF16)
        B, _, nf, hh, ww = lat.shape
        pt_, ph, pw = self.patch_size
        grid = (nf // pt_, hh // ph, ww // pw)
        F_, fs = grid[0], grid[1] * grid[2]
        cp_ws = self.parallel_config.world_size
        cp_rank = self.parallel_config.rank
        if fs % cp_ws != 0:
            raise ValueError(f"sequence parallelism splits every frame's {fs} tokens over {cp_ws} ranks: not divisible")
        hw_local = fs // cp_ws
        fs_l = hw_local
        N = F_ * fs_l
        assert len(kv_cache_requests) == B

        patches = C.patchify(lat, self.patch_size)
        if cp_ws > 1:
            patches = patches.view(B * F_, fs, -1)[:, cp_rank * hw_local:(cp_rank + 1) * hw_local].reshape(B * N, -1)
        xact = ops.linear(patches.contiguous(), self.g["patch_w"], self.g["patch_b"],
                          out=self._buf("x", B * N, d) if xact_out is None else xact_out)
        Ft = t.shape[1]
        rows_per_group = (F_ // Ft) * fs_l
        from ..schedulers import carry_tag, const_tag
        t_in = t
        t = carry_tag(t_in, t.to(dev))
        tc = const_tag(t)
        tkey = None if tc is None else (tc, tuple(t.shape), t.dtype, self.g["time0_w"].data_ptr(), self.g.get("time0_fmt"))
        hit = self._temb_cache.get(tkey) if tkey is not None else None
        stream_now = ops._stream()
        if hit is not None:
            E, eh = hit[1], hit[2]
            if hit[3] != stream_now:
                cur = torch.cuda.current_stream(dev)
                if hit[0] is not None:
                    cur.wait_event(hit[0])
                E.record_stream(cur)
                eh.record_stream(cur)
        else:
            emb = C.sinusoidal_embedding_1d(self.freq_dim, t.flatten()).to(BF16)
            e = self._lin(self.g, "time2", F.silu(self._lin(self.g, "time0", emb.contiguous())))
            e0 = self._lin(self.g, "tproj", F.silu(e)).unflatten(1, (6, d))
            E = (self.mod_all + e0.unsqueeze(0)).contiguous()
            eh = (self.g["head_mod"] + e.unsqueeze(1)).contiguous()
            if tkey is not None:
                if len(self._temb_cache) >= 16:
                    self._temb_cache.pop(next(iter(self._temb_cache)))
                ready = torch.cuda.Event() if t.is_cuda else None
                if ready is not None:
                    ready.record(torch.cuda.current_stream(dev))
                self._temb_cache[tkey] = (ready, E, eh, stream_now)

        need_ctx = any(not m["is_init"] for m in crossattn_cache_meta)
        ctx = None
        if need_ctx:
            if isinstance(context, torch.Tensor):
                context = list(context)
            padded = torch.stack([torch.cat([u.to(dev, BF16), torch.zeros(self.text_len - u.size(0), u.size(1),
                                                                       device=dev, dtype=BF16)]) for u in context])
            if self.cross_dedup:
                same = (padded == padded[:, -1:]).all(-1)
                idx = torch.arange(self.text_len, device=dev).expand(B, -1)
                first = (torch.where(same, -1, idx).amax(1) + 1).tolist()
                live = getattr(kv_cache_manager, "request_to_kv_caches", None)
                if live is not None:
                    for rid in [r for r in self._cross_dedup if r not in live]:
                        del self._cross_dedup[rid]
                for b, req in enumerate(kv_cache_requests or []):
                    j0 = min(int(first[b]), self.text_len - 1)
                    self._cross_dedup[req.request_id] = (j0 + 1, self.text_len - j0)
            c0 = self._lin(self.g, "text0", padded.view(B * self.text_len, -1), epilogue=_hip.IFX_EPI_GELU_TANH)
            ctx = self._lin(self.g, "text2", c0)

        h = self._buf("h", B * N, d)
        start_frame = current_start // fs
        q_scale, attn_scale = ops.attn_q_prescale(self.head_dim) if self.q_prescale else (0.0, 0.0)
        self._attn_scale = attn_scale
        rope = ops.RopeGridSpec(self.freqs, start_frame, grid[1], grid[2], cp_rank * hw_local, hw_local, q_scale)
        sink_tokens = self.sink_size * fs

        st = dict(B=B, N=N, F_=F_, fs=fs, rows_per_group=rows_per_group, rope=rope, sink_tokens=sink_tokens,
                  current_start=current_start, ctx=ctx, explicit_slots=explicit, attn_scale=attn_scale)
        return dict(xact=xact, E=E, eh=eh, h=h, st=st, kv_meta=kv_cache_meta, cross_meta=crossattn_cache_meta, grid=grid, B=B, F_=F_,
                    rows_per_group=rows_per_group, N=N, requests=list(kv_cache_requests))

    def _epilogue(self, fw: dict) -> torch.Tensor:
        ops.layernorm(fw["xact"], self.eps, mod=fw["eh"], shift_slot=0, scale_slot=1, rows_per_group=fw["rows_per_group"], out=fw["h"])
        yv = self._lin(self.g, "head", fw["h"])
        if self.cp is not None:
            yv = self.cp.gather_head(yv, fw["B"], fw["F_"])
        return C.unpatchify(yv, fw["B"], fw["grid"], self.patch_size, self.out_dim)
```

Measured before the change: 22.44 frames/s.

## Fuse cross-attention query RMSNorm into a grouped-head cross-attention kernel

```diff
diff --git a/include/inferix_hip.h b/include/inferix_hip.h
--- a/include/inferix_hip.h
+++ b/include/inferix_hip.h
@@ -50,6 +50,10 @@
 
 int ifx_attn_fwd_dedup(const ifx_bf16* q, ifx_bf16* out, const ifx_kv_view* kv, int32_t q_rows, int32_t heads, int32_t kv_len,
                        int32_t last_key_multiplicity, float scale, void* stream);
+
+int ifx_cross_attn_rms(const ifx_bf16* q, int32_t ldq, ifx_bf16* out, int32_t ldo, const ifx_bf16* w, const ifx_kv_view* kv,
+                       int32_t q_rows, int32_t heads, int32_t kv_len, int32_t last_key_multiplicity, float eps, float scale,
+                       void* stream);
 
 int ifx_attn_fwd_ranges(const ifx_bf16* q, int32_t ldq, ifx_bf16* out, int32_t ldo, const ifx_kv_view* kv, int32_t q_rows,
                         int32_t heads, int32_t n_ranges, const int32_t* q_ranges, const int32_t* k_ranges, float scale,
diff --git a/inferix_amd/_hip.py b/inferix_amd/_hip.py
--- a/inferix_amd/_hip.py
+++ b/inferix_amd/_hip.py
@@ -126,6 +126,7 @@
     "ifx_act_rows": (C.c_int, [_vp, _vp, C.c_int64, _i32, _vp]),
     "ifx_kv_split_rows": (C.c_int, [_vp, _vp, _vp, _i32, _i32, _i32, _i32, _i32, _vp]),
     "ifx_attn_fwd_dedup": (C.c_int, [_vp, _vp, C.POINTER(KvView), _i32, _i32, _i32, _i32, _f32, _vp]),
+    "ifx_cross_attn_rms": (C.c_int, [_vp, _i32, _vp, _i32, _vp, C.POINTER(KvView), _i32, _i32, _i32, _i32, _f32, _f32, _vp]),
     "ifx_attn_fwd_ranges": (C.c_int, [_vp, _i32, _vp, _i32, C.POINTER(KvView), _i32, _i32, _i32, C.POINTER(_i32), C.POINTER(_i32), _f32, _vp]),
     "ifx_gemm_workspace_bytes": (C.c_int64, [_i32, _i32, _i32]),
     "ifx_gemm_bf16_ws": (C.c_int, [_vp, _i32, _vp, _vp, _vp, _i32, _i32, _i32, _i32, C.POINTER(Epilogue), _vp, C.c_int64, _vp]),
diff --git a/inferix_amd/csrc/ifx_attn.hip b/inferix_amd/csrc/ifx_attn.hip
--- a/inferix_amd/csrc/ifx_attn.hip
+++ b/inferix_amd/csrc/ifx_attn.hip
@@ -1,13 +1,9 @@
 #include <stdlib.h>
 #include <type_traits>
 
-#include "ifx_common.h"
+#include "ifx_attn_tile.h"
 
 namespace ifx {
-
-constexpr int QT = 128;
-constexpr int KT = 64;
-constexpr int HD = 128;
 
 struct AttnArgs {
   const unsigned short* q;
@@ -23,25 +19,6 @@
   float scale, scale_log2;
 };
 
-typedef __attribute__((address_space(3))) void* attn_lds_ptr_t;
-typedef const __attribute__((address_space(1))) void* attn_gbl_ptr_t;
-
-__device__ __forceinline__ void attn_dma16(const unsigned short* src, unsigned lds) {
-  asm volatile("s_mov_b32 m0, %0\n\ts_nop 0\n\tglobal_load_lds_dwordx4 %1, off" : : "s"(lds), "v"(src) : "memory");
-}
-
-__device__ __forceinline__ float max3f(float a, float b, float c) {
-  float r;
-  asm("v_max3_f32 %0, %1, %2, %3" : "=v"(r) : "v"(a), "v"(b), "v"(c));
-  return r;
-}
-__device__ __forceinline__ float half_swap_max(float x) {
-  float a = x, b = x, r;
-  asm volatile("s_nop 1\n\tv_permlane32_swap_b32 %0, %1\n\ts_nop 1\n\tv_max_f32 %2, %0, %1"
-               : "+v"(a), "+v"(b), "=v"(r));
-  return r;
-}
-
 template <bool PAGED, bool SHORT>
 __global__ __launch_bounds__(256, 2) void attn_fwd_kernel(AttnArgs A) {
   __shared__ __attribute__((aligned(16))) unsigned char smem[65536];
@@ -53,7 +30,6 @@
   const int wi = xcd * A.per_xcd + slot_i;
   if (slot_i >= A.per_xcd || wi >= A.total) return;
   const int head = wi / A.q_tiles, qt = wi - head * A.q_tiles;
-  const int kv_stride = A.kv_heads * HD;
   const int kvh = head / A.q_per_kv;
 
   const int qrow = qt * QT + wave * 32 + l31;
@@ -66,214 +42,31 @@
   }
   __builtin_amdgcn_s_waitcnt(0x0F70);
 
-  const int d_row = lane >> 4, d_pc = lane & 15;
-  int k_src_c[4], v_src_c[4], d_rowi[4];
-#pragma unroll
-  for (int r = 0; r < 4; ++r) {
-    const int row = (r * 4 + wave) * 4 + d_row;
-    d_rowi[r] = row;
-    k_src_c[r] = (d_pc ^ (row & 15)) * 8;
-    v_src_c[r] = ((((d_pc >> 2) ^ (row & 3)) << 2) | (d_pc & 3)) * 8;
-  }
+  const AttnLane L(smem, lane, wave);
   const unsigned short* kbase = A.k + kvh * HD;
   const unsigned short* vbase = A.v + kvh * HD;
-  const int last_key = A.kv_len - 1;
-  const unsigned lds0 = (unsigned)(unsigned long long)(attn_lds_ptr_t)smem + wave * 1024;
-  auto issue = [&](int t, int buf, auto clamp_tag) {
-    constexpr bool CLAMP = decltype(clamp_tag)::value;
-    const unsigned kb = lds0 + buf * 32768;
-#pragma unroll
-    for (int r = 0; r < 4; ++r) {
-      int key = A.kv_start + t * KT + d_rowi[r];
-      if (CLAMP) key = min(key, last_key);
-      const size_t off = (size_t)(PAGED ? A.ka.slot(key) : key) * kv_stride;
-      attn_dma16(kbase + off + k_src_c[r], kb + r * 4096);
-      attn_dma16(vbase + off + v_src_c[r], kb + 16384 + r * 4096);
-    }
-  };
-
-  f32x16 o[4];
-#pragma unroll
-  for (int d = 0; d < 4; ++d)
-#pragma unroll
-    for (int r = 0; r < 16; ++r) o[d][r] = 0.f;
-  float m_run = -INFINITY, l_run = 0.f;
-  const float c2 = A.scale_log2;
-
-  const int kswz = l31 & 15;
-  const int vi = lane & 15, vg1 = (lane >> 4) & 1;
-  const int v_rowq = vi >> 2;
-  const int v_in = (vg1 << 5) | ((vi & 3) << 3);
-
   const int nkeys = A.kv_len - A.kv_start;
+  const AttnKeys K{A.ka, A.kv_start, A.kv_len - 1, A.kv_heads * HD, nkeys, A.last_key_bias, A.scale_log2};
   const int NT = (nkeys + KT - 1) / KT;
-
-  auto tile = [&](int t, int buf, auto ragged_tag) {
-    constexpr bool RAGGED = decltype(ragged_tag)::value;
-    const unsigned char* kb = smem + buf * 32768;
-    const unsigned char* vb = kb + 16384;
-    bf16x8 kA[4], kB[4], vA[4], vB[4];
-    auto ldK = [&](bf16x8(&f)[4], int b, int kh) {
-      const unsigned char* krow = kb + (32 * b + l31) * 256;
-#pragma unroll
-      for (int k4 = 0; k4 < 4; ++k4)
-        f[k4] = *reinterpret_cast<const bf16x8*>(krow + (((2 * (4 * kh + k4) + hi) ^ kswz) << 4));
-    };
-    auto mmaK = [&](f32x16& acc, bf16x8(&f)[4], int kh) {
-#pragma unroll
-      for (int k4 = 0; k4 < 4; ++k4) acc = __builtin_amdgcn_mfma_f32_32x32x16_bf16(f[k4], qf[4 * kh + k4], acc, 0, 0, 0);
-    };
-    auto ldV = [&](bf16x8(&f)[4], int b, int s2) {
-      const unsigned char* vr0 = vb + (32 * b + 16 * s2 + 4 * hi + v_rowq) * 256 + v_in;
-      const unsigned char* vr1 = vr0 + 8 * 256;
-#pragma unroll
-      for (int d = 0; d < 4; ++d) {
-        const int ch = (d ^ v_rowq) << 6;
-        const bf16x4 t0 = __builtin_amdgcn_ds_read_tr16_b64_v4bf16((bf16x4 __attribute__((address_space(3)))*)(vr0 + ch));
-        const bf16x4 t1 = __builtin_amdgcn_ds_read_tr16_b64_v4bf16((bf16x4 __attribute__((address_space(3)))*)(vr1 + ch));
-        f[d] = __builtin_shufflevector(t0, t1, 0, 1, 2, 3, 4, 5, 6, 7);
-      }
-    };
-    auto mmaV = [&](bf16x8(&f)[4], const bf16x8& p) {
-#pragma unroll
-      for (int d = 0; d < 4; ++d) o[d] = __builtin_amdgcn_mfma_f32_32x32x16_bf16(f[d], p, o[d], 0, 0, 0);
-    };
-    auto block_max = [&](f32x16& sb) -> float {
-      float mx = __builtin_fmaxf(sb[0], sb[1]);
-      mx = max3f(mx, sb[2], m_run);
-#pragma unroll
-      for (int r = 3; r < 15; r += 2) mx = max3f(mx, sb[r], sb[r + 1]);
-      mx = max3f(mx, sb[15], mx);
-      return half_swap_max(mx);
-    };
-    auto exp_block = [&](f32x16& sb, bf16x8(&pb)[2]) -> float {
-      typedef float f32x2 __attribute__((ext_vector_type(2)));
-      const float mc = m_run * c2;
-      const f32x2 c2v = {c2, c2}, mcv = {mc, mc};
-      float a0 = 0.f, a1 = 0.f;
-#pragma unroll
-      for (int i = 0; i < 8; ++i) {
-        const f32x2 sv = {sb[2 * i], sb[2 * i + 1]};
-        const f32x2 e = sv * c2v - mcv;
-        const float p0 = __builtin_amdgcn_exp2f(e[0]), p1 = __builtin_amdgcn_exp2f(e[1]);
-        a0 += p0;
-        a1 += p1;
-        pb[i >> 2][(2 * i) & 7] = static_cast<__bf16>(p0);
-        pb[i >> 2][(2 * i + 1) & 7] = static_cast<__bf16>(p1);
-      }
-      return a0 + a1;
-    };
-    auto softmax_block = [&](f32x16& sb, int b, bf16x8(&pb)[2]) -> float {
-      if (RAGGED) {
-        const int kidx = t * KT + 32 * b + 4 * hi;
-#pragma unroll
-        for (int r = 0; r < 16; ++r) {
-          const int kk = kidx + (r & 3) + 8 * (r >> 2);
-          if (kk >= nkeys) sb[r] = -INFINITY;
-          else if (kk == nkeys - 1) sb[r] += A.last_key_bias;
-        }
-      }
-      if (t == 0 && b == 0) m_run = block_max(sb);
-      float ps = exp_block(sb, pb);
-      float alpha = 1.0f;
-      if (__any(!(ps < 1048576.f))) {
-        const float m_new = block_max(sb);
-        alpha = __builtin_amdgcn_exp2f((m_run - m_new) * c2);
-        m_run = m_new;
-        ps = exp_block(sb, pb);
-        l_run *= alpha;
-      }
-      l_run += ps;
-      return alpha;
-    };
-    auto rescale_o = [&](float alpha) {
-      asm volatile("" : "+v"(alpha));
-      if (__any(alpha != 1.0f)) {
-        asm volatile("s_nop 15\n\ts_nop 7" ::: "memory");
-#pragma unroll
-        for (int d = 0; d < 4; ++d)
-#pragma unroll
-          for (int r = 0; r < 16; ++r) asm volatile("v_mul_f32 %0, %0, %1" : "+v"(o[d][r]) : "v"(alpha));
-        asm volatile("s_nop 3" ::: "memory");
-      }
-    };
-
-    f32x16 s0, s1;
-    bf16x8 p0[2], p1[2];
-    ldK(kA, 0, 0);
-    ldK(kB, 0, 1);
-    __builtin_amdgcn_sched_barrier(0);
-#pragma unroll
-    for (int r = 0; r < 16; ++r) s0[r] = 0.f;
-    __builtin_amdgcn_s_setprio(1);
-    mmaK(s0, kA, 0);
-    ldK(kA, 1, 0);
-    __builtin_amdgcn_sched_barrier(0);
-    mmaK(s0, kB, 1);
-    ldK(kB, 1, 1);
-    __builtin_amdgcn_sched_barrier(0);
-#pragma unroll
-    for (int r = 0; r < 16; ++r) s1[r] = 0.f;
-    mmaK(s1, kA, 0);
-    ldV(vA, 0, 0);
-    mmaK(s1, kB, 1);
-    ldV(vB, 0, 1);
-    const float a0 = softmax_block(s0, 0, p0);
-#pragma unroll
-    for (int i = 0; i < 8; ++i) {
-      __builtin_amdgcn_sched_group_barrier(0x008, 1, 0);
-      __builtin_amdgcn_sched_group_barrier(0x100, 2, 0);
-      __builtin_amdgcn_sched_group_barrier(0x002, 10, 0);
-    }
-    __builtin_amdgcn_sched_barrier(0);
-    rescale_o(a0);
-    mmaV(vA, p0[0]);
-    ldV(vA, 1, 0);
-    mmaV(vB, p0[1]);
-    ldV(vB, 1, 1);
-    const float a1 = softmax_block(s1, 1, p1);
-#pragma unroll
-    for (int i = 0; i < 8; ++i) {
-      __builtin_amdgcn_sched_group_barrier(0x008, 1, 1);
-      __builtin_amdgcn_sched_group_barrier(0x100, 2, 1);
-      __builtin_amdgcn_sched_group_barrier(0x002, 10, 1);
-    }
-    __builtin_amdgcn_sched_barrier(0);
-    rescale_o(a1);
-    mmaV(vA, p1[0]);
-    mmaV(vB, p1[1]);
-    __builtin_amdgcn_s_setprio(0);
-  };
-
-  issue(0, 0, std::true_type{});
+  AttnAcc acc;
+  acc.reset();
+
+  attn_issue_tile<PAGED, true>(L, K, kbase, vbase, 0, 0);
   asm volatile("s_waitcnt vmcnt(0)" ::: "memory");
   __builtin_amdgcn_s_barrier();
   for (int t = 0; t < NT - 1; ++t) {
     const int buf = t & 1;
-    if (t + 2 < NT) issue(t + 1, buf ^ 1, std::false_type{});
-    else issue(t + 1, buf ^ 1, std::true_type{});
-    tile(t, buf, std::false_type{});
+    if (t + 2 < NT) attn_issue_tile<PAGED, false>(L, K, kbase, vbase, t + 1, buf ^ 1);
+    else attn_issue_tile<PAGED, true>(L, K, kbase, vbase, t + 1, buf ^ 1);
+    attn_tile<false>(smem, L, K, qf, acc, t, buf);
     asm volatile("s_waitcnt vmcnt(0) lgkmcnt(0)" ::: "memory");
     __builtin_amdgcn_s_barrier();
   }
-  if ((nkeys & (KT - 1)) || A.last_key_bias != 0.f) tile(NT - 1, (NT - 1) & 1, std::true_type{});
-  else tile(NT - 1, (NT - 1) & 1, std::false_type{});
-
-  const float l_tot = l_run + __shfl_xor(l_run, 32, 64);
-  const float inv = 1.0f / l_tot;
-  if (qrow < A.q_rows) {
-    unsigned short* op = A.out + (size_t)qrow * A.ldo + head * HD + 4 * hi;
-#pragma unroll
-    for (int d = 0; d < 4; ++d)
-#pragma unroll
-      for (int g = 0; g < 4; ++g) {
-        u16x4 w;
-#pragma unroll
-        for (int e = 0; e < 4; ++e) w[e] = f2bf(o[d][4 * g + e] * inv);
-        *reinterpret_cast<u16x4*>(op + 32 * d + 8 * g) = w;
-      }
-    if (A.lse != nullptr && hi == 0) A.lse[(size_t)head * A.q_rows + qrow] = m_run * A.scale + __logf(l_tot);
-  }
+  if ((nkeys & (KT - 1)) || A.last_key_bias != 0.f) attn_tile<true>(smem, L, K, qf, acc, NT - 1, (NT - 1) & 1);
+  else attn_tile<false>(smem, L, K, qf, acc, NT - 1, (NT - 1) & 1);
+
+  const float l_tot = attn_store_row(L, acc, A.out + (size_t)qrow * A.ldo + head * HD, qrow < A.q_rows);
+  if (qrow < A.q_rows && A.lse != nullptr && hi == 0) A.lse[(size_t)head * A.q_rows + qrow] = acc.m_run * A.scale + __logf(l_tot);
 }
 
 __global__ __launch_bounds__(256) void lse_merge_kernel(unsigned short* __restrict__ oa, float* __restrict__ la,
diff --git a/inferix_amd/csrc/ifx_attn_tile.h b/inferix_amd/csrc/ifx_attn_tile.h
--- /dev/null
+++ b/inferix_amd/csrc/ifx_attn_tile.h
@@ -0,0 +1,248 @@
+#pragma once
+#include <type_traits>
+
+#include "ifx_common.h"
+
+namespace ifx {
+
+constexpr int QT = 128;
+constexpr int KT = 64;
+constexpr int HD = 128;
+
+typedef __attribute__((address_space(3))) void* attn_lds_ptr_t;
+typedef const __attribute__((address_space(1))) void* attn_gbl_ptr_t;
+
+__device__ __forceinline__ void attn_dma16(const unsigned short* src, unsigned lds) {
+  asm volatile("s_mov_b32 m0, %0\n\ts_nop 0\n\tglobal_load_lds_dwordx4 %1, off" : : "s"(lds), "v"(src) : "memory");
+}
+
+__device__ __forceinline__ float max3f(float a, float b, float c) {
+  float r;
+  asm("v_max3_f32 %0, %1, %2, %3" : "=v"(r) : "v"(a), "v"(b), "v"(c));
+  return r;
+}
+__device__ __forceinline__ float half_swap_max(float x) {
+  float a = x, b = x, r;
+  asm volatile("s_nop 1\n\tv_permlane32_swap_b32 %0, %1\n\ts_nop 1\n\tv_max_f32 %2, %0, %1"
+               : "+v"(a), "+v"(b), "=v"(r));
+  return r;
+}
+
+struct AttnLane {
+  int hi, l31;
+  int k_src_c[4], v_src_c[4], d_rowi[4];
+  unsigned lds0;
+  int kswz, v_rowq, v_in;
+  __device__ __forceinline__ AttnLane(const unsigned char* smem, int lane, int wave) : hi(lane >> 5), l31(lane & 31) {
+    const int d_row = lane >> 4, d_pc = lane & 15;
+#pragma unroll
+    for (int r = 0; r < 4; ++r) {
+      const int row = (r * 4 + wave) * 4 + d_row;
+      d_rowi[r] = row;
+      k_src_c[r] = (d_pc ^ (row & 15)) * 8;
+      v_src_c[r] = ((((d_pc >> 2) ^ (row & 3)) << 2) | (d_pc & 3)) * 8;
+    }
+    lds0 = (unsigned)(unsigned long long)(attn_lds_ptr_t)smem + wave * 1024;
+    kswz = l31 & 15;
+    const int vi = lane & 15, vg1 = (lane >> 4) & 1;
+    v_rowq = vi >> 2;
+    v_in = (vg1 << 5) | ((vi & 3) << 3);
+  }
+};
+
+struct AttnKeys {
+  KvAddr ka;
+  int kv_start, last_key, kv_stride, nkeys;
+  float last_key_bias;
+  float c2;
+};
+
+template <bool PAGED, bool CLAMP>
+__device__ __forceinline__ void attn_issue_tile(const AttnLane& L, const AttnKeys& K, const unsigned short* kbase,
+                                                const unsigned short* vbase, int t, int buf) {
+  const unsigned kb = L.lds0 + buf * 32768;
+#pragma unroll
+  for (int r = 0; r < 4; ++r) {
+    int key = K.kv_start + t * KT + L.d_rowi[r];
+    if (CLAMP) key = min(key, K.last_key);
+    const size_t off = (size_t)(PAGED ? K.ka.slot(key) : key) * K.kv_stride;
+    attn_dma16(kbase + off + L.k_src_c[r], kb + r * 4096);
+    attn_dma16(vbase + off + L.v_src_c[r], kb + 16384 + r * 4096);
+  }
+}
+
+struct AttnAcc {
+  f32x16 o[4];
+  float m_run, l_run;
+  __device__ __forceinline__ void reset() {
+#pragma unroll
+    for (int d = 0; d < 4; ++d)
+#pragma unroll
+      for (int r = 0; r < 16; ++r) o[d][r] = 0.f;
+    m_run = -INFINITY;
+    l_run = 0.f;
+  }
+};
+
+template <bool RAGGED>
+__device__ __forceinline__ void attn_tile(const unsigned char* smem, const AttnLane& L, const AttnKeys& K, const bf16x8 (&qf)[8],
+                                          AttnAcc& acc, int t, int buf) {
+  const int hi = L.hi, l31 = L.l31, kswz = L.kswz, v_rowq = L.v_rowq, v_in = L.v_in, nkeys = K.nkeys;
+  const float c2 = K.c2;
+  f32x16(&o)[4] = acc.o;
+  float& m_run = acc.m_run;
+  float& l_run = acc.l_run;
+  const unsigned char* kb = smem + buf * 32768;
+  const unsigned char* vb = kb + 16384;
+  bf16x8 kA[4], kB[4], vA[4], vB[4];
+  auto ldK = [&](bf16x8(&f)[4], int b, int kh) {
+    const unsigned char* krow = kb + (32 * b + l31) * 256;
+#pragma unroll
+    for (int k4 = 0; k4 < 4; ++k4)
+      f[k4] = *reinterpret_cast<const bf16x8*>(krow + (((2 * (4 * kh + k4) + hi) ^ kswz) << 4));
+  };
+  auto mmaK = [&](f32x16& a, bf16x8(&f)[4], int kh) {
+#pragma unroll
+    for (int k4 = 0; k4 < 4; ++k4) a = __builtin_amdgcn_mfma_f32_32x32x16_bf16(f[k4], qf[4 * kh + k4], a, 0, 0, 0);
+  };
+  auto ldV = [&](bf16x8(&f)[4], int b, int s2) {
+    const unsigned char* vr0 = vb + (32 * b + 16 * s2 + 4 * hi + v_rowq) * 256 + v_in;
+    const unsigned char* vr1 = vr0 + 8 * 256;
+#pragma unroll
+    for (int d = 0; d < 4; ++d) {
+      const int ch = (d ^ v_rowq) << 6;
+      const bf16x4 t0 = __builtin_amdgcn_ds_read_tr16_b64_v4bf16((bf16x4 __attribute__((address_space(3)))*)(vr0 + ch));
+      const bf16x4 t1 = __builtin_amdgcn_ds_read_tr16_b64_v4bf16((bf16x4 __attribute__((address_space(3)))*)(vr1 + ch));
+      f[d] = __builtin_shufflevector(t0, t1, 0, 1, 2, 3, 4, 5, 6, 7);
+    }
+  };
+  auto mmaV = [&](bf16x8(&f)[4], const bf16x8& p) {
+#pragma unroll
+    for (int d = 0; d < 4; ++d) o[d] = __builtin_amdgcn_mfma_f32_32x32x16_bf16(f[d], p, o[d], 0, 0, 0);
+  };
+  auto block_max = [&](f32x16& sb) -> float {
+    float mx = __builtin_fmaxf(sb[0], sb[1]);
+    mx = max3f(mx, sb[2], m_run);
+#pragma unroll
+    for (int r = 3; r < 15; r += 2) mx = max3f(mx, sb[r], sb[r + 1]);
+    mx = max3f(mx, sb[15], mx);
+    return half_swap_max(mx);
+  };
+  auto exp_block = [&](f32x16& sb, bf16x8(&pb)[2]) -> float {
+    typedef float f32x2 __attribute__((ext_vector_type(2)));
+    const float mc = m_run * c2;
+    const f32x2 c2v = {c2, c2}, mcv = {mc, mc};
+    float a0 = 0.f, a1 = 0.f;
+#pragma unroll
+    for (int i = 0; i < 8; ++i) {
+      const f32x2 sv = {sb[2 * i], sb[2 * i + 1]};
+      const f32x2 e = sv * c2v - mcv;
+      const float p0 = __builtin_amdgcn_exp2f(e[0]), p1 = __builtin_amdgcn_exp2f(e[1]);
+      a0 += p0;
+      a1 += p1;
+      pb[i >> 2][(2 * i) & 7] = static_cast<__bf16>(p0);
+      pb[i >> 2][(2 * i + 1) & 7] = static_cast<__bf16>(p1);
+    }
+    return a0 + a1;
+  };
+  auto softmax_block = [&](f32x16& sb, int b, bf16x8(&pb)[2]) -> float {
+    if (RAGGED) {
+      const int kidx = t * KT + 32 * b + 4 * hi;
+#pragma unroll
+      for (int r = 0; r < 16; ++r) {
+        const int kk = kidx + (r & 3) + 8 * (r >> 2);
+        if (kk >= nkeys) sb[r] = -INFINITY;
+        else if (kk == nkeys - 1) sb[r] += K.last_key_bias;
+      }
+    }
+    if (t == 0 && b == 0) m_run = block_max(sb);
+    float ps = exp_block(sb, pb);
+    float alpha = 1.0f;
+    if (__any(!(ps < 1048576.f))) {
+      const float m_new = block_max(sb);
+      alpha = __builtin_amdgcn_exp2f((m_run - m_new) * c2);
+      m_run = m_new;
+      ps = exp_block(sb, pb);
+      l_run *= alpha;
+    }
+    l_run += ps;
+    return alpha;
+  };
+  auto rescale_o = [&](float alpha) {
+    asm volatile("" : "+v"(alpha));
+    if (__any(alpha != 1.0f)) {
+      asm volatile("s_nop 15\n\ts_nop 7" ::: "memory");
+#pragma unroll
+      for (int d = 0; d < 4; ++d)
+#pragma unroll
+        for (int r = 0; r < 16; ++r) asm volatile("v_mul_f32 %0, %0, %1" : "+v"(o[d][r]) : "v"(alpha));
+      asm volatile("s_nop 3" ::: "memory");
+    }
+  };
+
+  f32x16 s0, s1;
+  bf16x8 p0[2], p1[2];
+  ldK(kA, 0, 0);
+  ldK(kB, 0, 1);
+  __builtin_amdgcn_sched_barrier(0);
+#pragma unroll
+  for (int r = 0; r < 16; ++r) s0[r] = 0.f;
+  __builtin_amdgcn_s_setprio(1);
+  mmaK(s0, kA, 0);
+  ldK(kA, 1, 0);
+  __builtin_amdgcn_sched_barrier(0);
+  mmaK(s0, kB, 1);
+  ldK(kB, 1, 1);
+  __builtin_amdgcn_sched_barrier(0);
+#pragma unroll
+  for (int r = 0; r < 16; ++r) s1[r] = 0.f;
+  mmaK(s1, kA, 0);
+  ldV(vA, 0, 0);
+  mmaK(s1, kB, 1);
+  ldV(vB, 0, 1);
+  const float a0 = softmax_block(s0, 0, p0);
+#pragma unroll
+  for (int i = 0; i < 8; ++i) {
+    __builtin_amdgcn_sched_group_barrier(0x008, 1, 0);
+    __builtin_amdgcn_sched_group_barrier(0x100, 2, 0);
+    __builtin_amdgcn_sched_group_barrier(0x002, 10, 0);
+  }
+  __builtin_amdgcn_sched_barrier(0);
+  rescale_o(a0);
+  mmaV(vA, p0[0]);
+  ldV(vA, 1, 0);
+  mmaV(vB, p0[1]);
+  ldV(vB, 1, 1);
+  const float a1 = softmax_block(s1, 1, p1);
+#pragma unroll
+  for (int i = 0; i < 8; ++i) {
+    __builtin_amdgcn_sched_group_barrier(0x008, 1, 1);
+    __builtin_amdgcn_sched_group_barrier(0x100, 2, 1);
+    __builtin_amdgcn_sched_group_barrier(0x002, 10, 1);
+  }
+  __builtin_amdgcn_sched_barrier(0);
+  rescale_o(a1);
+  mmaV(vA, p1[0]);
+  mmaV(vB, p1[1]);
+  __builtin_amdgcn_s_setprio(0);
+}
+
+__device__ __forceinline__ float attn_store_row(const AttnLane& L, const AttnAcc& acc, unsigned short* op, bool valid) {
+  const float l_tot = acc.l_run + __shfl_xor(acc.l_run, 32, 64);
+  const float inv = 1.0f / l_tot;
+  if (valid) {
+    op += 4 * L.hi;
+#pragma unroll
+    for (int d = 0; d < 4; ++d)
+#pragma unroll
+      for (int g = 0; g < 4; ++g) {
+        u16x4 w;
+#pragma unroll
+        for (int e = 0; e < 4; ++e) w[e] = f2bf(acc.o[d][4 * g + e] * inv);
+        *reinterpret_cast<u16x4*>(op + 32 * d + 8 * g) = w;
+      }
+  }
+  return l_tot;
+}
+
+}
diff --git a/inferix_amd/csrc/ifx_core.hip b/inferix_amd/csrc/ifx_core.hip
--- a/inferix_amd/csrc/ifx_core.hip
+++ b/inferix_amd/csrc/ifx_core.hip
@@ -15,6 +15,7 @@
 }
 
 static int g_gemm_variant = -1, g_gemm_pp_variant = -1, g_attn_variant = -1, g_conv_variant = -1, g_spin_timeout_ms = -1, g_spin_fault = 0;
+static int g_cross_fused = -1;
 static thread_local int g_gemm_small_split = -1;
 static int opt_or_env(int& slot, const char* env, int dflt = 0) {
   if (slot < 0) {
@@ -98,6 +99,7 @@
   }
   if (key && !strcmp(key, "spin_timeout_ms") && value >= 1 && value <= 600000) { ifx::g_spin_timeout_ms = value; return IFX_OK; }
   if (key && !strcmp(key, "spin_fault") && (value == 0 || value == 1)) { ifx::g_spin_fault = value; return IFX_OK; }
+  if (key && !strcmp(key, "cross_fused") && (value == 0 || value == 1)) { ifx::g_cross_fused = value; return IFX_OK; }
   ifx::set_error("ifx_set_option: unknown key or value out of range: %s = %d", key ? key : "(null)", (int)value);
   return IFX_EINVAL;
 }
@@ -120,6 +122,7 @@
   }
   if (!strcmp(key, "spin_timeout_ms")) { *value = (int32_t)(ifx::spin_timeout_ticks() / 100000LL); return IFX_OK; }
   if (!strcmp(key, "spin_fault")) { *value = ifx::spin_fault(); return IFX_OK; }
+  if (!strcmp(key, "cross_fused")) { *value = ifx::opt_or_env(ifx::g_cross_fused, "IFX_CROSS_FUSED", 1); return IFX_OK; }
   ifx::set_error("ifx_get_option: unknown key: %s", key);
   return IFX_EINVAL;
 }
diff --git a/inferix_amd/csrc/ifx_cross.hip b/inferix_amd/csrc/ifx_cross.hip
--- /dev/null
+++ b/inferix_amd/csrc/ifx_cross.hip
@@ -0,0 +1,186 @@
+#include "ifx_attn_tile.h"
+#include "ifx_rows.h"
+
+namespace ifx {
+
+#ifndef IFX_CROSS_G
+#define IFX_CROSS_G 2
+#endif
+constexpr int kCrossG = IFX_CROSS_G;
+constexpr int kCrossMaxKeys = 256;
+
+struct CrossArgs {
+  const unsigned short* q;
+  unsigned short* out;
+  const unsigned short* w;
+  const unsigned short* k;
+  const unsigned short* v;
+  int q_rows, heads, kv_len, ldq, ldo;
+  int head_groups, per_xcd, total;
+  float last_key_bias, scale_log2, eps;
+};
+
+template <int NCH>
+constexpr int cross_row_batch() { return NCH <= 3 ? 8 : (NCH <= 6 ? 4 : 2); }
+
+template <int NCH, int G>
+__global__ __launch_bounds__(256, 1) void cross_attn_rms_kernel(CrossArgs A) {
+  __shared__ __attribute__((aligned(16))) unsigned char smem[65536 + (G - 1) * 32768];
+  const int tid = threadIdx.x, lane = tid & 63;
+  const int wave = __builtin_amdgcn_readfirstlane(tid >> 6);
+  const int hi = lane >> 5, l31 = lane & 31;
+
+  const int xcd = blockIdx.x & 7, slot_i = blockIdx.x >> 3;
+  const int wi = xcd * A.per_xcd + slot_i;
+  if (slot_i >= A.per_xcd || wi >= A.total) return;
+  const int qt = wi / A.head_groups, head0 = (wi - qt * A.head_groups) * G;
+  const int ng = min(G, A.heads - head0);
+  const int dim = A.heads * HD;
+
+  const AttnLane L(smem, lane, wave);
+  const AttnKeys K{KvAddr{nullptr, 1, 0, 0}, 0, A.kv_len - 1, dim, A.kv_len, A.last_key_bias, A.scale_log2};
+  const int NT = (A.kv_len + KT - 1) / KT;
+  const int items = ng * NT;
+  auto issue = [&](int g, int t, int slot) {
+    attn_issue_tile<false, true>(L, K, A.k + (head0 + g) * HD, A.v + (head0 + g) * HD, t, slot);
+  };
+  issue(0, 0, 0);
+  if (items > 1) issue(NT > 1 ? 0 : 1, NT > 1 ? 1 : 0, 1);
+
+  const int row0 = qt * QT + wave * 32;
+  const int qrow = row0 + l31;
+  u16x8 qraw[G][8], wv[G][8];
+  {
+    const unsigned short* qp = A.q + (size_t)min(qrow, A.q_rows - 1) * A.ldq + hi * 8;
+#pragma unroll
+    for (int g = 0; g < G; ++g) {
+      const int hc = (head0 + min(g, ng - 1)) * HD;
+#pragma unroll
+      for (int ks = 0; ks < 8; ++ks) {
+        qraw[g][ks] = *reinterpret_cast<const u16x8*>(qp + hc + ks * 16);
+        wv[g][ks] = *reinterpret_cast<const u16x8*>(A.w + hc + hi * 8 + ks * 16);
+      }
+    }
+  }
+
+  constexpr int RB = cross_row_batch<NCH>();
+  float ss_mine = 0.f;
+  auto row_sums = [&](auto full_tag) {
+    u16x8 xr[2][RB][NCH];
+    auto request = [&](int b, u16x8 (&x)[RB][NCH]) {
+#pragma unroll
+      for (int j = 0; j < RB; ++j) load_chunks<NCH>(x[j], A.q + (size_t)min(row0 + b * RB + j, A.q_rows - 1) * A.ldq, dim, lane);
+      __builtin_amdgcn_sched_barrier(0);
+    };
+    request(0, xr[0]);
+#pragma unroll
+    for (int b = 0; b < 32 / RB; ++b) {
+      if (b + 1 < 32 / RB) request(b + 1, xr[(b + 1) & 1]);
+#pragma unroll
+      for (int j = 0; j < RB; ++j) {
+        Row<NCH> row;
+        if (decltype(full_tag)::value) row.from_full(xr[b & 1][j]);
+        else row.from(xr[b & 1][j], dim, lane);
+        const float ss = wave_sum(row.sumsq());
+        if (l31 == b * RB + j) ss_mine = ss;
+      }
+      __builtin_amdgcn_sched_barrier(0);
+    }
+  };
+  if (dim == NCH * 512) row_sums(std::true_type{});
+  else row_sums(std::false_type{});
+#ifdef IFX_CROSS_LAB_NOSTATS
+  ss_mine = (float)dim;
+#endif
+  const float rs_mine = 1.0f / sqrtf(ss_mine / (float)dim + A.eps);
+
+  bf16x8 qf[8];
+  unsigned char* park = smem + 65536 + wave * 8192 + lane * 16;
+#pragma unroll
+  for (int g = 0; g < G; ++g)
+#pragma unroll
+    for (int ks = 0; ks < 8; ++ks) {
+      u16x8 o;
+#pragma unroll
+      for (int e = 0; e < 8; ++e) o[e] = f2bf(rbf(bf2f(qraw[g][ks][e]) * rs_mine) * bf2f(wv[g][ks][e]));
+      if (g == 0) qf[ks] = __builtin_bit_cast(bf16x8, o);
+      else *reinterpret_cast<u16x8*>(park + (g - 1) * 32768 + ks * 1024) = o;
+    }
+
+  const bool ragged_last = (A.kv_len & (KT - 1)) || A.last_key_bias != 0.f;
+  AttnAcc acc;
+  asm volatile("s_waitcnt vmcnt(0)" ::: "memory");
+  __builtin_amdgcn_s_barrier();
+  for (int i = 0, g = 0, t = 0; i < items; ++i) {
+    if (t == 0) {
+      if (g > 0) {
+#pragma unroll
+        for (int ks = 0; ks < 8; ++ks) qf[ks] = *reinterpret_cast<const bf16x8*>(park + (g - 1) * 32768 + ks * 1024);
+      }
+      acc.reset();
+    }
+    if (i >= 1 && i + 1 < items) {
+      if (t + 1 < NT) issue(g, t + 1, (i + 1) & 1);
+      else issue(g + 1, 0, (i + 1) & 1);
+    }
+    if (t == NT - 1 && ragged_last) attn_tile<true>(smem, L, K, qf, acc, t, i & 1);
+    else attn_tile<false>(smem, L, K, qf, acc, t, i & 1);
+    asm volatile("s_waitcnt vmcnt(0) lgkmcnt(0)" ::: "memory");
+    __builtin_amdgcn_s_barrier();
+    if (++t == NT) {
+      attn_store_row(L, acc, A.out + (size_t)qrow * A.ldo + (head0 + g) * HD, qrow < A.q_rows);
+      t = 0;
+      ++g;
+    }
+  }
+}
+
+}
+
+using namespace ifx;
+
+extern "C" int ifx_cross_attn_rms(const ifx_bf16* q, int32_t ldq, ifx_bf16* out, int32_t ldo, const ifx_bf16* w, const ifx_kv_view* kv,
+                                  int32_t q_rows, int32_t heads, int32_t kv_len, int32_t last_key_multiplicity, float eps, float scale,
+                                  void* stream) {
+  IFX_REQUIRE(q && out && w && kv && kv->k && kv->v, "ifx_cross_attn_rms: null argument");
+  IFX_REQUIRE(kv->head_dim == HD, "ifx_cross_attn_rms: head_dim %d not built (128 only)", kv->head_dim);
+  IFX_REQUIRE(heads > 0 && kv->kv_heads == heads, "ifx_cross_attn_rms: kv_heads %d != heads %d (no grouped-query form)", kv->kv_heads,
+              heads);
+  const int dim = heads * HD;
+  IFX_REQUIRE(dim <= 5120, "ifx_cross_attn_rms: heads * 128 = %d is wider than the row kernels' 5120", dim);
+  if (ldq <= 0) ldq = dim;
+  if (ldo <= 0) ldo = dim;
+  IFX_REQUIRE(ldq >= dim && ldo >= dim && ldq % 8 == 0 && ldo % 8 == 0,
+              "ifx_cross_attn_rms: row strides (%d, %d) must be >= heads * 128 and multiples of 8", ldq, ldo);
+  IFX_REQUIRE(kv->page_table == nullptr && kv->seg_split <= 0,
+              "ifx_cross_attn_rms: paged or two-segment kv view: the fused form reads a contiguous cache (use ifx_rmsnorm + ifx_attn_fwd_dedup)");
+  IFX_REQUIRE(last_key_multiplicity >= 1, "ifx_cross_attn_rms: multiplicity %d", last_key_multiplicity);
+  IFX_REQUIRE(q_rows >= 0 && kv_len >= 1 && kv_len <= kv->num_slots, "ifx_cross_attn_rms: kv_len %d out of range (capacity %d)", kv_len,
+              kv->num_slots);
+  IFX_REQUIRE(kv_len <= kCrossMaxKeys, "ifx_cross_attn_rms: kv_len %d beyond the fused form's limit of %d keys (use ifx_rmsnorm + ifx_attn_fwd_dedup)",
+              kv_len, kCrossMaxKeys);
+  if (q_rows == 0) return IFX_OK;
+  constexpr int G = kCrossG;
+  CrossArgs a;
+  a.q = q;
+  a.out = out;
+  a.w = w;
+  a.k = kv->k;
+  a.v = kv->v;
+  a.q_rows = q_rows;
+  a.heads = heads;
+  a.kv_len = kv_len;
+  a.ldq = ldq;
+  a.ldo = ldo;
+  a.head_groups = (heads + G - 1) / G;
+  a.total = ((q_rows + QT - 1) / QT) * a.head_groups;
+  a.per_xcd = (a.total + 7) / 8;
+  const float sc = scale > 0.f ? scale : 0.08838834764831845f;
+  a.scale_log2 = sc * 1.4426950408889634f;
+  a.last_key_bias = last_key_multiplicity > 1 ? logf((float)last_key_multiplicity) / sc : 0.f;
+  a.eps = eps;
+  return dispatch_norm(dim, [&](auto nch) {
+    hipLaunchKernelGGL((cross_attn_rms_kernel<decltype(nch)::value, G>), dim3(a.per_xcd * 8), dim3(256), 0, (hipStream_t)stream, a);
+    return check_launch("ifx_cross_attn_rms");
+  });
+}
diff --git a/inferix_amd/csrc/ifx_norm.hip b/inferix_amd/csrc/ifx_norm.hip
--- a/inferix_amd/csrc/ifx_norm.hip
+++ b/inferix_amd/csrc/ifx_norm.hip
@@ -189,11 +189,6 @@
   }
 }
 
-template <typename F>
-static int dispatch_norm(int dim, F&& f) {
-  return dispatch_nch<1, 2, 3, 4, 6, 8, 10>(dim, "row kernels support dim <= 5120 (got %d)", f);
-}
-
 }
 
 using namespace ifx;
diff --git a/inferix_amd/csrc/ifx_rows.h b/inferix_amd/csrc/ifx_rows.h
--- a/inferix_amd/csrc/ifx_rows.h
+++ b/inferix_amd/csrc/ifx_rows.h
@@ -24,6 +24,12 @@
 #pragma unroll
       for (int i = 0; i < 8; ++i) v[c][i] = ok ? bf2f(u[c][i]) : 0.f;
     }
+  }
+  __device__ __forceinline__ void from_full(const u16x8 (&u)[NCH]) {
+#pragma unroll
+    for (int c = 0; c < NCH; ++c)
+#pragma unroll
+      for (int i = 0; i < 8; ++i) v[c][i] = bf2f(u[c][i]);
   }
   __device__ __forceinline__ float sum() const {
     float s = 0.f;
@@ -203,6 +209,11 @@
   return IFX_EUNSUP;
 }
 
+template <typename F>
+static int dispatch_norm(int dim, F&& f) {
+  return dispatch_nch<1, 2, 3, 4, 6, 8, 10>(dim, "row kernels support dim <= 5120 (got %d)", f);
+}
+
 template <typename K, typename... A>
 static int launch_rows(const char* who, K kernel, int rows, void* stream, A... args) {
   hipLaunchKernelGGL(kernel, dim3((rows + 3) / 4), dim3(256), 0, (hipStream_t)stream, args...);
diff --git a/inferix_amd/hip_ops.py b/inferix_amd/hip_ops.py
--- a/inferix_amd/hip_ops.py
+++ b/inferix_amd/hip_ops.py
@@ -836,3 +836,37 @@
         _hip.check(_hip.load().ifx_attn_fwd_dedup(_dev(q, "q"), _dev(out, "out"), C.byref(ks), rows, heads, int(kv_len),
                                                   int(last_key_multiplicity), float(scale), _stream()), "ifx_attn_fwd_dedup")
     return out
+
+
+CROSS_FUSED_MAX_KEYS = 256
+
+
+def cross_fused_serves(kv: KvCacheView, kv_len: int, heads: int) -> bool:
+    return (kv.page_table is None and not kv.seg_split and 1 <= kv_len <= CROSS_FUSED_MAX_KEYS and kv.k.shape[1] == heads
+            and heads * 128 <= 5120)
+
+
+def cross_attention_rms(q: torch.Tensor, weight: torch.Tensor, eps: float, kv: KvCacheView, kv_len: int, last_key_multiplicity: int,
+                        out: Optional[torch.Tensor] = None, scale: float = 0.0, tag: str = "attn_cross") -> torch.Tensor:
+    heads = kv.k.shape[1]
+    d = heads * 128
+    q2 = q.view(q.shape[0], d) if q.dim() == 3 else q
+    out = torch.empty_like(q) if out is None else out
+    o2 = out.view(out.shape[0], d) if out.dim() == 3 else out
+    rows = q2.shape[0]
+    assert q2.dim() == 2 and o2.shape[0] == rows and q2.shape[1] >= d and o2.shape[1] >= d and weight.numel() == d
+    fused = _OPTIONS.get("cross_fused")
+    if fused is None:
+        fused = get_option("cross_fused")
+    if not fused:
+        assert q2.is_contiguous() and o2.is_contiguous() and q2.shape[1] == d, "cross_fused = 0 takes dense rows"
+        rmsnorm(q2, weight, eps, out=q2)
+        attention_dedup(q2.view(rows, heads, 128), kv, kv_len, last_key_multiplicity, out=o2.view(rows, heads, 128), scale=scale, tag=tag)
+        return out
+    ks = kv.struct()
+    nk = kv_len - 1 + last_key_multiplicity
+    with _timed(tag, 4.0 * rows * nk * d, 0.0), _timed(tag + "_rms", 4.0 * rows * nk * d, 4.0 * rows * d):
+        _hip.check(_hip.load().ifx_cross_attn_rms(_dev(q2, "q"), q2.stride(0), _dev(o2, "out"), o2.stride(0), _dev(weight, "weight"),
+                                                  C.byref(ks), rows, heads, int(kv_len), int(last_key_multiplicity), float(eps),
+                                                  float(scale), _stream()), "ifx_cross_attn_rms")
+    return out
diff --git a/inferix_amd/wan/causal_model.py b/inferix_amd/wan/causal_model.py
--- a/inferix_amd/wan/causal_model.py
+++ b/inferix_amd/wan/causal_model.py
@@ -376,7 +376,6 @@
         self._lin(w, "o", ab, epilogue=_hip.IFX_EPI_GATE_RES, residual=xact, mod=El, gate_slot=2,
                   rows_per_group=rows_per_group, out=xact)
         self._norm_lin(w, "cq", xact, h, dict(gamma=w["n3_w"], beta=w["n3_b"]), out=qb)
-        ops.rmsnorm(qb, w["cnq"], self.eps, out=qb)
         b = 0
         while b < len(samples):
             req = samples[b]["req"]
@@ -392,6 +391,12 @@
                 self._lin(w, "cv", cb, out=cview.v.view(self.text_len, d))
             nkeys, mult = self._cross_dedup.get(req.request_id, (self.text_len, 1)) if self.cross_dedup else (self.text_len, 1)
             qv, av = qb[b * N:(b + nb) * N].view(nb * N, H, hd), ab[b * N:(b + nb) * N].view(nb * N, H, hd)
+            if (nb == 1 and len(samples) == 1 and not explicit_any and self.cp is None and ops.cross_fused_serves(cview, nkeys, H)
+                    and ops.get_option("cross_fused")):
+                ops.cross_attention_rms(qv, w["cnq"], self.eps, cview, nkeys, mult, out=av, tag="attn_cross")
+                b += nb
+                continue
+            ops.rmsnorm(qb[b * N:(b + nb) * N], w["cnq"], self.eps, out=qb[b * N:(b + nb) * N])
             if mult > 1:
                 ops.attention_dedup(qv, cview, nkeys, mult, out=av, tag="attn_cross")
             else:
```

Result: slower. 22.15 frames/s (-1.3%).
